# QuentinFuxa/WhisperLiveKit

Hardware: AMD Instinct MI355X
Metric: audio seconds transcribed per second (1/RTF), Whisper-base EN simul_whisper AlignAtt, 0.5 s chunks (higher is better)
Workload: dtype f32; 1 GPU; base.en simul_whisper, 1 stream(s) over 1 GPU(s) (1 per GPU), 30 s 16 kHz speech-like stream, 0.5 s chunks, beam 1, frame_threshold 25, seeded random weights, synthetic vocabulary; model=base.en, streams_total=1

## Files before the change

whisperlivekit_amd/csrc/api.hip:

```cpp
#include <cmath>
#include <cstdio>
#include <cstdlib>
#include <atomic>
#include <chrono>
#include <cstring>
#include <map>
#include <memory>
#include <mutex>
#include <string>
#include <vector>

#include "../../include/wlk_hip.h"
#include "common.h"
#include "internal.h"

namespace wlk {

namespace {
struct UtilStream {
    std::mutex mu;
    hipStream_t stream = nullptr;
};
UtilStream g_util[64];
UtilStream& util_of_current_device() {
// ... 249 lines not shown
        for (int l = 0; l < L; ++l) {
            int n = 0;
            for (int h = 0; h < H; ++h)
                if (rank[(size_t)l * H + h] >= 0) heads[(size_t)l * H + n++] = h;
        }
        copy_sync(m->layer_heads, heads.data(), heads.size() * sizeof(int), hipMemcpyHostToDevice);
        m->align_pairs.assign(pairs, pairs + 2 * n_pairs);
        m->n_align = n_pairs;
        return WLK_OK;
    });
}

int wlk_model_finalize(wlk_model* m) {
    if (!m) return fail(WLK_ERR_ARG, "model is NULL");
    return guarded([&]() {
        WLK_HIP(hipSetDevice(m->device));
        const int nm = m->D.n_mels;
        std::vector<float> f((size_t)nm * kNFreq);
        copy_sync(f.data(), m->w("mel.filters"), f.size() * sizeof(float), hipMemcpyDeviceToHost);
        std::vector<int> lo(nm), hi(nm);
        for (int i = 0; i < nm; ++i) {
            int a = kNFreq, b = 0;
            for (int k = 0; k < kNFreq; ++k)
                if (f[(size_t)i * kNFreq + k] != 0.f) {
                    a = std::min(a, k);
                    b = k + 1;
                }
            if (b == 0) a = 0;
            lo[i] = a;
            hi[i] = b;
        }
        copy_sync(m->filt_lo, lo.data(), nm * sizeof(int), hipMemcpyHostToDevice);
        copy_sync(m->filt_hi, hi.data(), nm * sizeof(int), hipMemcpyHostToDevice);
        m->enc_layers.clear();
        m->dec_layers.clear();
        for (int i = 0; i < m->D.n_audio_layer; ++i) m->enc_layers.push_back(layer_weights(m, "enc", i, false));
        for (int i = 0; i < m->D.n_text_layer; ++i) m->dec_layers.push_back(layer_weights(m, "dec", i, true));
        {
            const size_t d = m->D.n_text_state, da = m->D.n_audio_state, Ld = m->D.n_text_layer;
            if (!m->xkv_all_w) m->xkv_all_w = dev_alloc<float>(Ld * 2 * d * da);
            if (!m->xkv_all_b) m->xkv_all_b = dev_alloc<float>(Ld * 2 * d);
            for (size_t i = 0; i < Ld; ++i) {
                copy_sync(m->xkv_all_w + i * 2 * d * da, m->dec_layers[i].xkvw, 2 * d * da * sizeof(float),
                                  hipMemcpyDeviceToDevice);
                copy_sync(m->xkv_all_b + i * 2 * d, m->dec_layers[i].xkvb, 2 * d * sizeof(float),
                                  hipMemcpyDeviceToDevice);
            }
        }
        {
            for (unsigned short* p : m->x3_owned) (void)hipFree(p);
            m->x3_owned.clear();
            m->xkv_all_w3 = nullptr;
            const int da = m->D.n_audio_state, T = m->D.n_audio_ctx;
            LaunchCtx c;
            c.stream = nullptr;
            hipStream_t st;
            WLK_HIP(hipStreamCreateWithFlags(&st, hipStreamNonBlocking));
            struct StreamGuard {
                hipStream_t s;
                ~StreamGuard() { (void)hipStreamDestroy(s); }
            } st_guard{st};
            c.stream = st;
            auto pack = [&](const float* w, int n_rows, int k = 0) -> unsigned short* {
                if (k == 0) k = da;
                unsigned short* p3 = dev_alloc<unsigned short>(x3_w_elems(n_rows, k));
                m->x3_owned.push_back(p3);
                launch_x3_pack_w(c, w, k, p3, n_rows, k);
                return p3;
            };
            static const bool narrow = [] { const char* e = getenv("WLK_X3_NARROW"); return !(e && e[0] == '0'); }();
            for (auto& L : m->enc_layers) {
                L.qkvw3 = gemm_x3_wide_applicable(T, 3 * da, da, da) ? pack(L.qkvw, 3 * da) : nullptr;
                L.fc1w3 = gemm_x3_wide_applicable(T, 4 * da, da, da) ? pack(L.fc1w, 4 * da) : nullptr;
                L.outw3 = narrow && gemm_x3_wide_applicable(T, da, da, da) ? pack(L.outw, da) : nullptr;
                L.fc2w3 = narrow && gemm_x3_wide_applicable(T, da, 4 * da, 4 * da) ? pack(L.fc2w, da, 4 * da) : nullptr;
            }
            const int n_xkv = m->D.n_text_layer * 2 * m->D.n_text_state;
            if (gemm_x3_wide_applicable(T, n_xkv, da, da)) m->xkv_all_w3 = pack(m->xkv_all_w, n_xkv);
            WLK_HIP(hipStreamSynchronize(st));
        }
        m->w_tok_emb = m->w("dec.tok_emb");
        m->w_dec_pos = m->w("dec.pos");
        m->w_ln_w = m->w("dec.ln.w");
        m->w_ln_b = m->w("dec.ln.b");
        m->finalized = true;
        return WLK_OK;
    });
}

int wlk_model_destroy(wlk_model* m) {
    if (!m) return WLK_OK;
    wlk_engine_destroy_for_model(m);
    (void)hipSetDevice(m->device);
    if (m->owns_arena) (void)hipFree(m->arena);
    if (m->xkv_all_w) (void)hipFree(m->xkv_all_w);
    if (m->xkv_all_b) (void)hipFree(m->xkv_all_b);
    for (unsigned short* p : m->x3_owned) (void)hipFree(p);
    (void)hipFree(m->twiddle);
    (void)hipFree(m->filt_lo);
    (void)hipFree(m->filt_hi);
    (void)hipFree(m->head_rank);
    (void)hipFree(m->layer_heads);
    (void)hipFree(m->layer_ranks);
    (void)hipFree(m->all_ranks);
    if (m->cif_w) (void)hipFree(m->cif_w);
    delete m;
    return WLK_OK;
}

int wlk_session_create(wlk_model* m, int beam, int max_audio_samples, wlk_session** out) {
    if (!m || !out) return fail(WLK_ERR_ARG, "NULL argument");
    if (!m->finalized) return fail(WLK_ERR_STATE, "model not finalized");
    if (beam < 1 || beam > 7) return fail(WLK_ERR_ARG, "beam must be in [1, 7]");
    if (max_audio_samples < kHop) return fail(WLK_ERR_ARG, "max_audio_samples too small");
    return guarded([&]() {
        WLK_HIP(hipSetDevice(m->device));
        auto s = std::make_unique<wlk_session>();
        s->m = m;
        s->beam = beam;
        s->audio_cap = max_audio_samples;
        WLK_HIP(hipStreamCreateWithFlags(&s->stream, hipStreamNonBlocking));
        if (const char* e = std::getenv("WLK_NO_GRAPH")) s->use_graph = !(e[0] == '1');
        hipStream_t st = s->stream;
        const wlk_dims& D = m->D;
        const size_t d = D.n_audio_state, T = D.n_audio_ctx, ctx = D.n_text_ctx, V = D.n_vocab;
        s->audio[0] = dev_alloc_zero<float>(s->audio_cap, st);
        s->audio[1] = dev_alloc_zero<float>(s->audio_cap, st);
        s->frame_cap = s->audio_cap / kHop + 4;
        s->logmel = dev_alloc<float>((size_t)s->frame_cap * D.n_mels);
        s->frame_max = dev_alloc<float>(s->frame_cap);
        s->logmel_alt = dev_alloc<float>((size_t)s->frame_cap * D.n_mels);
        s->frame_max_alt = dev_alloc<float>(s->frame_cap);
        if (const char* e = std::getenv("WLK_MEL_INCREMENTAL")) s->mel_incremental = !(e[0] == '0');
        s->mel_t = dev_alloc_zero<float>((size_t)(kMelFrames + 2) * D.n_mels, st);
        s->x1p = dev_alloc_zero<float>((size_t)(kMelFrames + 1) * d, st);
        s->ex = dev_alloc<float>(T * d);
        s->eh = dev_alloc<float>(T * d);
        s->eqkv = dev_alloc<float>(T * 3 * d);
        s->eatt = dev_alloc<float>(T * d);
        s->emlp = dev_alloc<float>(T * 4 * d);
        s->enc_out = dev_alloc<float>(T * d);
        {
            bool any_x3 = m->xkv_all_w3 != nullptr, qkv_x3 = false;
            bool fc2_x3 = false;
            for (const auto& L : m->enc_layers) {
                any_x3 |= L.qkvw3 || L.fc1w3 || L.outw3;
                qkv_x3 |= L.qkvw3 != nullptr;
                fc2_x3 |= L.fc2w3 != nullptr;
            }
            if (fc2_x3) s->emlp3 = dev_alloc<unsigned short>(T * 3 * 4 * d);
            const bool attn_x3 = qkv_x3 && enc_attention_x3_enabled() && d == (size_t)D.n_audio_head * 64 && T >= 64 && (2 * d) % 128 == 0;
            if (any_x3) s->eh3 = dev_alloc<unsigned short>(T * 3 * d);
            if (attn_x3) s->eqkv3 = dev_alloc_zero<unsigned short>(x3_attn_image_elems((int)T, (int)d), st);
            if (m->xkv_all_w3) s->enc_out3 = dev_alloc<unsigned short>(T * 3 * d);
        }
        s->cross_kv = dev_alloc<float>((size_t)D.n_text_layer * T * 2 * d);

        s->max_rows = beam * (int)ctx;
        const size_t R = s->max_rows;
        s->step_in = dev_alloc<int>(3 * R + 4);
        s->tokens_dev = s->step_in;
        s->dx = dev_alloc<float>(R * d);
        s->dh = dev_alloc<float>(R * d);
        s->dqkv = dev_alloc<float>(R * 3 * d);
        s->datt = dev_alloc<float>(R * d);
        s->dq = dev_alloc<float>(R * d);
        s->dmlp = dev_alloc<float>(R * 4 * d);
        const size_t cache = (size_t)D.n_text_layer * beam * ctx * d;
        s->kcache[0] = dev_alloc<float>(cache);
        s->vcache[0] = dev_alloc<float>(cache);
        s->hsel = dev_alloc<float>((size_t)2 * beam * d);
        s->logits_last = dev_alloc<float>((size_t)2 * beam * V);
        s->logits_sot = s->logits_last + (size_t)beam * V;
        s->ring_row = s->step_in + R;
        s->beam_of_row = s->step_in + 2 * R;
        s->d_offset = s->step_in + 3 * R;
        s->ring_rows = (int)ctx + kAlignWindow;
        if (m->n_align > 0) s->ring = dev_alloc<float>((size_t)m->n_align * beam * s->ring_rows * T);
        s->xsplit = dev_alloc<float>(cross_split_scratch_floats(8, D.n_text_head, (int)T));
        s->fsplit = dev_alloc<float>(flash_split_scratch_floats(s->max_rows, D.n_text_head, wlk_session::kFlashSplitsMax));
        s->z = dev_alloc<float>((size_t)beam * std::max(m->n_align, 1) * T + (size_t)beam * 128);
        s->attn_last = dev_alloc_zero<float>((size_t)beam * T, st);
        s->adj_row = dev_alloc<int>(3 * wlk_session::kAdjCap);
        s->src_rows = dev_alloc<int>(8);
        if (beam >= 2 && beam <= 7) s->anc = dev_alloc_zero<unsigned char>((size_t)beam * ctx, st);
        s->top_vals = dev_alloc<float>((size_t)beam * 18);
        s->top_ids = reinterpret_cast<int*>(s->top_vals) + (size_t)beam * 8;
        s->frames = s->top_ids + (size_t)beam * 8;
        WLK_HIP(hipMalloc(&s->topk_scratch, topk_scratch_bytes(beam)));
        s->probs = dev_alloc<float>(beam);
        WLK_HIP(hipHostMalloc(&s->pinned, wlk_session::kPinnedBytes, hipHostMallocDefault));
        WLK_HIP(hipHostMalloc(&s->dec_stage, 65536, hipHostMallocDefault));
        WLK_HIP(hipHostMalloc(&s->audio_stage, wlk_session::kPinnedBytes, hipHostMallocDefault));
        WLK_HIP(hipEventCreateWithFlags(&s->audio_stage_ev, hipEventDisableTiming));
        WLK_HIP(hipEventCreateWithFlags(&s->dec_stage_ev, hipEventDisableTiming));
        if (beam == 1) {
            void* hp = nullptr;
            WLK_HIP(hipHostMalloc(&hp, 4096, hipHostMallocMapped | hipHostMallocCoherent));
            std::memset(hp, 0, 4096);
            s->step_host = static_cast<StepBlock*>(hp);
            s->result_host = reinterpret_cast<StepResult*>(static_cast<char*>(hp) + 2048);
            void* dp = nullptr;
            WLK_HIP(hipHostGetDevicePointer(&dp, hp, 0));
            s->step_host_dev = static_cast<StepBlock*>(dp);
            s->result_host_dev = reinterpret_cast<StepResult*>(static_cast<char*>(dp) + 2048);
            s->step_dev = reinterpret_cast<StepBlock*>(dev_alloc<int>(sizeof(StepBlock) / 4));
        }
        if (m->cif_w) wlk_cif_session_prepare(s.get());
        WLK_HIP(hipStreamSynchronize(st));
        *out = s.release();
        return WLK_OK;
    });
}

int wlk_session_destroy(wlk_session* s) {
    if (!s) return WLK_OK;
    if (s->step_count && getenv("WLK_STEP_TIMING"))
        fprintf(stderr, "[wlk] one-replay steps: %llu, mean %.1f us per step (graph launch call %.1f us)\n",
                (unsigned long long)s->step_count, s->step_ns / 1e3 / s->step_count, s->step_launch_ns / 1e3 / s->step_count);
    (void)wlk_engine_detach(s);
    (void)hipSetDevice(s->m->device);
    (void)hipStreamSynchronize(s->stream);
    float* fl[] = {s->audio[0], s->audio[1], s->logmel, s->frame_max, s->logmel_alt, s->frame_max_alt, s->mel_t, s->x1p, s->ex, s->eh, s->eqkv,
                   s->eatt, s->emlp, s->enc_out, s->cross_kv, s->dx, s->dh, s->dqkv, s->datt, s->dq, s->dmlp,
                   s->kcache[0], s->kcache[1], s->vcache[0], s->vcache[1], s->hsel, s->logits_last,
                   s->ring, s->z, s->attn_last, s->qk_debug, s->xsplit, s->fsplit, s->top_vals, s->probs};
    for (float* p : fl)
        if (p) (void)hipFree(p);
    int* il[] = {s->step_in, s->adj_row, s->src_rows};
    for (int* p : il)
        if (p) (void)hipFree(p);
    for (auto& e : s->step_exec)
        if (e) (void)hipGraphExecDestroy(e);
    for (auto& e : s->bstep_exec)
        if (e) (void)hipGraphExecDestroy(e);
    if (s->anc) (void)hipFree(s->anc);
    if (s->topk_scratch) (void)hipFree(s->topk_scratch);
    if (s->pcm16_dev) (void)hipFree(s->pcm16_dev);
    if (s->eh3) (void)hipFree(s->eh3);
    if (s->eqkv3) (void)hipFree(s->eqkv3);
    if (s->enc_out3) (void)hipFree(s->enc_out3);
    if (s->emlp3) (void)hipFree(s->emlp3);
    if (s->wa_buf) (void)hipFree(s->wa_buf);
    if (s->pinned) (void)hipHostFree(s->pinned);
    if (s->dec_stage) (void)hipHostFree(s->dec_stage);
    if (s->audio_stage) (void)hipHostFree(s->audio_stage);
    if (s->rules_mask) (void)hipFree(s->rules_mask);
    if (s->pick_out) (void)hipFree(s->pick_out);
    if (s->audio_stage_ev) (void)hipEventDestroy(s->audio_stage_ev);
    if (s->dec_stage_ev) (void)hipEventDestroy(s->dec_stage_ev);
    if (s->step_host) (void)hipHostFree(s->step_host);
    if (s->step_dev) (void)hipFree(s->step_dev);
    if (s->step_align_dev) (void)hipFree(s->step_align_dev);
    wlk_cif_session_free(s);
    for (auto& e : s->fstep_exec)
        if (e) (void)hipGraphExecDestroy(e);
    for (auto& r : s->prof.recs) {
        (void)hipEventDestroy(r.a);
        (void)hipEventDestroy(r.b);
    }
    for (auto e : s->prof.pool) (void)hipEventDestroy(e);
    (void)hipStreamDestroy(s->stream);
    delete s;
    return WLK_OK;
}

int wlk_session_set_debug(wlk_session* s, int on) {
    if (!s) return fail(WLK_ERR_ARG, "session is NULL");
    return guarded([&]() {
        WLK_HIP(hipSetDevice(s->m->device));
        s->debug = on != 0;
        if (s->debug && !s->qk_debug) {
            const wlk_dims& D = s->m->D;
            s->qk_debug = dev_alloc<float>((size_t)D.n_text_layer * s->max_rows * D.n_text_head * D.n_audio_ctx);
        }
        return WLK_OK;
    });
}

static bool drain_staging() {
    static const bool on = [] {
        const char* e = getenv("WLK_DRAIN_STAGING");
        return e && e[0] == '1';
    }();
    return on;
}

int wlk_audio_append(wlk_session* s, const float* pcm_host, int n) {
    if (!s || (n > 0 && !pcm_host) || n < 0) return fail(WLK_ERR_ARG, "bad audio chunk");
    if (s->audio_len + n > s->audio_cap)
        return fail(WLK_ERR_CAPACITY, "audio buffer capacity exceeded (" + std::to_string(s->audio_len + n) + " > " +
                                          std::to_string(s->audio_cap) + " samples)");
    if (n == 0) return WLK_OK;
    return guarded([&]() {
        WLK_HIP(hipSetDevice(s->m->device));
        float* dst = s->audio[s->audio_cur] + s->audio_len;
        size_t done = 0;
        while (done < (size_t)n) {
            const size_t chunk = std::min((size_t)n - done, wlk_session::kPinnedBytes / sizeof(float));
            if (s->audio_stage_used) WLK_HIP(hipEventSynchronize(s->audio_stage_ev));
            std::memcpy(s->audio_stage, pcm_host + done, chunk * sizeof(float));
            WLK_HIP(hipMemcpyAsync(dst + done, s->audio_stage, chunk * sizeof(float), hipMemcpyHostToDevice, s->stream));
            WLK_HIP(hipEventRecord(s->audio_stage_ev, s->stream));
            s->audio_stage_used = true;
            done += chunk;
        }
        if (drain_staging()) WLK_HIP(hipStreamSynchronize(s->stream));
        s->audio_len += n;
        s->encoded = false;
        return WLK_OK;
    });
}

int wlk_audio_append_pcm16(wlk_session* s, const int16_t* pcm_host, int n) {
    if (!s || (n > 0 && !pcm_host) || n < 0) return fail(WLK_ERR_ARG, "bad audio chunk");
    if (s->audio_len + n > s->audio_cap)
        return fail(WLK_ERR_CAPACITY, "audio buffer capacity exceeded (" + std::to_string(s->audio_len + n) + " > " +
                                          std::to_string(s->audio_cap) + " samples)");
    if (n == 0) return WLK_OK;
    return guarded([&]() {
        WLK_HIP(hipSetDevice(s->m->device));
        constexpr size_t kMax = wlk_session::kPinnedBytes / sizeof(int16_t);
        if (!s->pcm16_dev) WLK_HIP(hipMalloc(reinterpret_cast<void**>(&s->pcm16_dev), kMax * sizeof(int16_t)));
        float* dst = s->audio[s->audio_cur] + s->audio_len;
        const LaunchCtx c = s->ctx();
        size_t done = 0;
        while (done < (size_t)n) {
            const size_t chunk = std::min((size_t)n - done, kMax);
            if (s->audio_stage_used) WLK_HIP(hipEventSynchronize(s->audio_stage_ev));
            std::memcpy(s->audio_stage, pcm_host + done, chunk * sizeof(int16_t));
            WLK_HIP(hipMemcpyAsync(s->pcm16_dev, s->audio_stage, chunk * sizeof(int16_t), hipMemcpyHostToDevice, s->stream));
            launch_pcm16_to_float(c, s->pcm16_dev, dst + done, (int)chunk);
            WLK_HIP(hipEventRecord(s->audio_stage_ev, s->stream));
            s->audio_stage_used = true;
            done += chunk;
        }
        if (drain_staging()) WLK_HIP(hipStreamSynchronize(s->stream));
        s->audio_len += n;
        s->encoded = false;
        return WLK_OK;
    });
}

int wlk_audio_append_zeros(wlk_session* s, int n) {
    if (!s || n < 0) return fail(WLK_ERR_ARG, "bad zero run");
    if (s->audio_len + n > s->audio_cap) return fail(WLK_ERR_CAPACITY, "audio buffer capacity exceeded");
    if (n == 0) return WLK_OK;
    return guarded([&]() {
        WLK_HIP(hipSetDevice(s->m->device));
        WLK_HIP(hipMemsetAsync(s->audio[s->audio_cur] + s->audio_len, 0, (size_t)n * sizeof(float), s->stream));
        s->audio_len += n;
        s->encoded = false;
        return WLK_OK;
    });
}

int wlk_audio_drop_front(wlk_session* s, int n) {
    if (!s || n < 0 || n > s->audio_len) return fail(WLK_ERR_ARG, "bad eviction length");
    if (n == 0) return WLK_OK;
    return guarded([&]() {
        WLK_HIP(hipSetDevice(s->m->device));
        const int keep = s->audio_len - n;
        if (keep > 0)
            WLK_HIP(hipMemcpyAsync(s->audio[s->audio_cur ^ 1], s->audio[s->audio_cur] + n, (size_t)keep * sizeof(float),
                                   hipMemcpyDeviceToDevice, s->stream));
        s->audio_cur ^= 1;
        s->audio_len = keep;
        s->encoded = false;
        const int shift = n / kHop;
        if (s->mel_incremental && n % kHop == 0 && s->mel_cached_samples > n && shift < s->mel_cached_frames) {
            const int rows = s->mel_cached_frames - shift;
            const int nm = s->m->D.n_mels;
            WLK_HIP(hipMemcpyAsync(s->logmel_alt, s->logmel + (size_t)shift * nm, (size_t)rows * nm * sizeof(float),
                                   hipMemcpyDeviceToDevice, s->stream));
            WLK_HIP(hipMemcpyAsync(s->frame_max_alt, s->frame_max + shift, (size_t)rows * sizeof(float),
                                   hipMemcpyDeviceToDevice, s->stream));
            std::swap(s->logmel, s->logmel_alt);
            std::swap(s->frame_max, s->frame_max_alt);
            s->mel_cached_samples -= n;
            s->mel_cached_frames = rows;
            s->mel_dirty_head = 2;
        } else {
            s->mel_cached_samples = 0;
        }
        return WLK_OK;
    });
}

int wlk_audio_clear(wlk_session* s) {
    if (!s) return fail(WLK_ERR_ARG, "session is NULL");
    s->audio_len = 0;
    s->encoded = false;
    s->mel_cached_samples = 0;
    return WLK_OK;
}

int wlk_audio_len(wlk_session* s, int* n) {
    if (!s || !n) return fail(WLK_ERR_ARG, "NULL argument");
    *n = s->audio_len;
    return WLK_OK;
}

static void transformer_mlp(const LaunchCtx& c, const LayerW& L, float* x, float* h, float* mlp, int rows, int d,
                            const char* t_ln, const char* t_fc1, const char* t_fc2) {
    GemmArgs g;
    g.lda = d; g.W = L.fc1w; g.bias = L.fc1b; g.C = mlp; g.ldc = 4 * d; g.M = rows; g.N = 4 * d; g.K = d;
    g.flags = kGemmGelu;
    if (gemv_applicable(rows, d)) {
        g.A = x; g.ln_gamma = L.ln2w; g.ln_beta = L.ln2b;
        launch_gemv(c, g, "dec_ln2_fc1");
    } else {
        launch_layernorm(c, x, d, L.ln2w, L.ln2b, h, d, rows, d, t_ln);
        g.A = h;
        launch_gemm(c, g, t_fc1);
    }
    GemmArgs g2;
    g2.A = mlp; g2.lda = 4 * d; g2.W = L.fc2w; g2.bias = L.fc2b; g2.C = x; g2.ldc = d; g2.M = rows; g2.N = d;
    g2.K = 4 * d; g2.flags = kGemmResidual; g2.R = x; g2.ldr = d;
    launch_linear(c, g2, t_fc2);
}

extern "C++" std::string wlk_encode_precheck(const wlk_session* s, const wlk_model* m) {
    if (!s) return "encode: session is NULL";
    if (s->m != m) return "encode: the session belongs to another model";
    const int N = s->audio_len;
    const int n_total = (N + kPadSamples) / kHop;
    int n_active = N > 0 ? (N + kNFft / 2 + kHop - 1) / kHop : 0;
    if (n_active > n_total) n_active = n_total;
    if (n_active > s->frame_cap) return "audio longer than the session's frame capacity";
    return std::string();
}

extern "C++" void wlk_encode_group(const std::vector<wlk_session*>& group, const LaunchCtx& c,
                                   std::vector<int>& content_out, bool mel_given) {
    const int B = (int)group.size();
    if (B < 1 || B > kMaxBatch) throw std::invalid_argument("encode: bad group size");
    wlk_model* m = group[0]->m;
    const wlk_dims& D = m->D;
    const int d = D.n_audio_state, T = D.n_audio_ctx;
    content_out.assign(B, 0);
    for (int i = 0; i < B; ++i) {
        wlk_session* s = group[i];
        if (s->m != m) throw std::invalid_argument("encode: sessions of different models in one group");
        if (mel_given) {
            content_out[i] = D.n_audio_ctx;
            continue;
        }
        const int N = s->audio_len;
        const int n_total = (N + kPadSamples) / kHop;
        int n_active = N > 0 ? (N + kNFft / 2 + kHop - 1) / kHop : 0;
        if (n_active > n_total) n_active = n_total;
        if (n_active > s->frame_cap) throw std::length_error("audio longer than the session's frame capacity");
        content_out[i] = (n_total - kMelFrames) / 2;
        MelArgs ma;
        ma.audio = s->audio[s->audio_cur]; ma.n_samples = N;
        ma.window = m->w("mel.window"); ma.twiddle = m->twiddle; ma.filters = m->w("mel.filters");
        ma.filt_lo = m->filt_lo; ma.filt_hi = m->filt_hi; ma.n_mels = D.n_mels;
        ma.logmel = s->logmel; ma.frame_max = s->frame_max; ma.mel_t = s->mel_t;
        ma.n_active = n_active; ma.n_total = n_total;
        if (s->mel_incremental && s->mel_cached_samples > 0 && s->mel_cached_samples <= N && s->mel_cached_frames <= n_active) {
            int first = s->mel_cached_samples >= kNFft / 2 ? (s->mel_cached_samples - kNFft / 2) / kHop + 1 : 0;
            first = std::min(first, s->mel_cached_frames);
            ma.first = first;
            ma.head = std::min(s->mel_dirty_head, first);
        }
        launch_mel(c, ma);
        s->mel_cached_samples = N;
        s->mel_cached_frames = n_active;
        s->mel_dirty_head = 0;
    }
    auto table = [&](auto in, auto out, auto res) {
        PtrTable z{};
        for (int i = 0; i < B; ++i) {
            z.in[i] = in(group[i]);
            z.out[i] = out(group[i]);
            z.res[i] = res(group[i]);
        }
        return z;
    };
    auto none = [](wlk_session*) -> const float* { return nullptr; };
    auto gemm = [&](GemmArgs g, const PtrTable& z, const char* tag) {
        const bool stackable = !gemm_takes_kwave(g.M, g.N, g.K) && (long)((g.N + 63) / 64) * ((g.M + 63) / 64) >= 64;
        if (stackable) {
            g.batch = B;
            g.z = z;
            launch_gemm(c, g, tag);
        } else {
            for (int i = 0; i < B; ++i) {
                g.A = z.in[i]; g.C = z.out[i]; g.R = z.res[i];
                launch_gemm(c, g, tag);
            }
        }
    };
    {
        GemmArgs g;
        g.lda = D.n_mels; g.W = m->w("enc.conv1.w"); g.bias = m->w("enc.conv1.b");
        g.ldc = d; g.M = kMelFrames; g.N = d; g.K = 3 * D.n_mels; g.flags = kGemmGelu;
        gemm(g, table([](wlk_session* s) { return (const float*)s->mel_t; }, [&](wlk_session* s) { return s->x1p + d; }, none),
             "enc_conv1");
    }
    {
        const float* pos = m->w("enc.pos");
        GemmArgs g;
        g.lda = 2 * d; g.W = m->w("enc.conv2.w"); g.bias = m->w("enc.conv2.b");
        g.ldc = d; g.M = T; g.N = d; g.K = 3 * d; g.flags = kGemmGelu | kGemmResidual; g.ldr = d;
        gemm(g, table([](wlk_session* s) { return (const float*)s->x1p; }, [](wlk_session* s) { return s->ex; },
                      [&](wlk_session*) { return pos; }), "enc_conv2");
    }
    const float scale = std::pow((float)kHeadDim, -0.25f);
    const PtrTable z_ex_eh = table([](wlk_session* s) { return (const float*)s->ex; }, [](wlk_session* s) { return s->eh; }, none);
    const PtrTable z_eh_qkv = table([](wlk_session* s) { return (const float*)s->eh; }, [](wlk_session* s) { return s->eqkv; }, none);
    const PtrTable z_qkv_att = table([](wlk_session* s) { return (const float*)s->eqkv; }, [](wlk_session* s) { return s->eatt; }, none);
    const PtrTable z_att_ex = table([](wlk_session* s) { return (const float*)s->eatt; }, [](wlk_session* s) { return s->ex; },
                                    [](wlk_session* s) { return (const float*)s->ex; });
    const PtrTable z_eh_mlp = table([](wlk_session* s) { return (const float*)s->eh; }, [](wlk_session* s) { return s->emlp; }, none);
    const PtrTable z_mlp_ex = table([](wlk_session* s) { return (const float*)s->emlp; }, [](wlk_session* s) { return s->ex; },
                                    [](wlk_session* s) { return (const float*)s->ex; });
    const PtrTable z_ex_eh3 = table([](wlk_session* s) { return (const float*)s->ex; },
                                    [](wlk_session* s) { return reinterpret_cast<float*>(s->eh3); }, none);
    const PtrTable z_eh3_qkv = table([](wlk_session* s) { return reinterpret_cast<const float*>(s->eh3); },
                                     [](wlk_session* s) { return s->eqkv; }, none);
    const PtrTable z_eh3_mlp = table([](wlk_session* s) { return reinterpret_cast<const float*>(s->eh3); },
                                     [](wlk_session* s) { return s->emlp; }, none);
    const PtrTable z_eh3_qkv3 = table([](wlk_session* s) { return reinterpret_cast<const float*>(s->eh3); },
                                      [](wlk_session* s) { return reinterpret_cast<float*>(s->eqkv3); }, none);
    const PtrTable z_qkv3_att = table([](wlk_session* s) { return reinterpret_cast<const float*>(s->eqkv3); },
                                      [](wlk_session* s) { return s->eatt; }, none);
    const PtrTable z_qkv3_eh3 = table([](wlk_session* s) { return reinterpret_cast<const float*>(s->eqkv3); },
                                      [](wlk_session* s) { return reinterpret_cast<float*>(s->eh3); }, none);
    const PtrTable z_eh3_ex_res = table([](wlk_session* s) { return reinterpret_cast<const float*>(s->eh3); }, [](wlk_session* s) { return s->ex; },
                                        [](wlk_session* s) { return (const float*)s->ex; });
    const PtrTable z_eh3_mlp3 = table([](wlk_session* s) { return reinterpret_cast<const float*>(s->eh3); },
                                      [](wlk_session* s) { return reinterpret_cast<float*>(s->emlp3); }, none);
    const PtrTable z_mlp3_ex_res = table([](wlk_session* s) { return reinterpret_cast<const float*>(s->emlp3); }, [](wlk_session* s) { return s->ex; },
                                         [](wlk_session* s) { return (const float*)s->ex; });
    const bool attn_x3 = enc_attention_x3_enabled() && d == D.n_audio_head * 64 && T >= 64 && (2 * d) % 128 == 0;
    auto gemm_x3 = [&](const GemmArgs& g, const unsigned short* w3, const PtrTable& z, const char* tag) {
        X3GemmArgs x;
        x.lda = g.lda; x.W3 = w3; x.bias = g.bias; x.ldc = g.ldc; x.ldr = g.ldr; x.M = g.M; x.N = g.N; x.K = g.K;
        x.flags = g.flags; x.scale = g.scale; x.scale_cols = g.scale_cols; x.scale_period = g.scale_period;
        x.batch = B;
        x.z = z;
        launch_gemm_x3(c, x, tag);
    };
    for (int i = 0; i < D.n_audio_layer; ++i) {
        const LayerW& L = m->enc_layers[i];
        GemmArgs g;
        g.lda = d; g.W = L.qkvw; g.bias = L.qkvb; g.ldc = 3 * d; g.M = T; g.N = 3 * d;
        g.K = d; g.flags = kGemmScaleCols; g.scale = scale; g.scale_cols = 2 * d;
        bool att_is_x3 = false;
        if (L.qkvw3 && attn_x3) {
            launch_layernorm_x3_batched(c, z_ex_eh3, B, d, L.ln1w, L.ln1b, d, T, d, "enc_ln1");
            X3GemmArgs x;
            x.lda = d; x.W3 = L.qkvw3; x.bias = g.bias; x.M = T; x.N = 3 * d; x.K = d; x.flags = g.flags; x.scale = g.scale;
            x.scale_cols = g.scale_cols; x.batch = B; x.z = z_eh3_qkv3;
            x.x3_out = true; x.ldc3 = 2 * d; x.vt_col0 = 2 * d; x.vt_off = x3_attn_vt_off(T, d); x.vt_ld = x3_attn_vt_ld(T);
            launch_gemm_x3(c, x, "enc_qkv_x3");
            att_is_x3 = L.outw3 != nullptr;
            launch_encoder_attention_x3(c, nullptr, 2L * d, x3_attn_vt_off(T, d), x3_attn_vt_ld(T), nullptr, d, T, d, D.n_audio_head,
                                        att_is_x3 ? &z_qkv3_eh3 : &z_qkv3_att, B, att_is_x3);
        } else {
            if (L.qkvw3) {
                launch_layernorm_x3_batched(c, z_ex_eh3, B, d, L.ln1w, L.ln1b, d, T, d, "enc_ln1");
                gemm_x3(g, L.qkvw3, z_eh3_qkv, "enc_qkv_x3");
            } else {
                launch_layernorm_batched(c, z_ex_eh, B, d, L.ln1w, L.ln1b, d, T, d, "enc_ln1");
                gemm(g, z_eh_qkv, "enc_qkv");
            }
            launch_encoder_attention_batched(c, z_qkv_att, B, T, d, D.n_audio_head);
        }
        GemmArgs o;
        o.lda = d; o.W = L.outw; o.bias = L.outb; o.ldc = d; o.M = T; o.N = d; o.K = d;
        o.flags = kGemmResidual; o.ldr = d;
        if (L.outw3) {
            if (!att_is_x3)
                for (int i = 0; i < B; ++i) launch_x3_pack(c, group[i]->eatt, d, group[i]->eh3, d, T, d);
            gemm_x3(o, L.outw3, z_eh3_ex_res, "enc_out_x3");
        } else {
            gemm(o, z_att_ex, "enc_out");
        }
        GemmArgs f1;
        f1.lda = d; f1.W = L.fc1w; f1.bias = L.fc1b; f1.ldc = 4 * d; f1.M = T; f1.N = 4 * d; f1.K = d; f1.flags = kGemmGelu;
        const bool mlp_x3 = L.fc1w3 && L.fc2w3 && (4 * d) % 128 == 0;
        if (mlp_x3) {
            launch_layernorm_x3_batched(c, z_ex_eh3, B, d, L.ln2w, L.ln2b, d, T, d, "enc_ln2");
            X3GemmArgs x;
            x.lda = d; x.W3 = L.fc1w3; x.bias = f1.bias; x.M = T; x.N = 4 * d; x.K = d; x.flags = kGemmGelu; x.batch = B; x.z = z_eh3_mlp3;
            x.x3_out = true; x.ldc3 = 4 * d; x.vt_col0 = 4 * d; x.vt_off = 0; x.vt_ld = (T + 31) / 32 * 32;
            launch_gemm_x3(c, x, "enc_fc1_x3");
        } else if (L.fc1w3) {
            launch_layernorm_x3_batched(c, z_ex_eh3, B, d, L.ln2w, L.ln2b, d, T, d, "enc_ln2");
            gemm_x3(f1, L.fc1w3, z_eh3_mlp, "enc_fc1_x3");
        } else {
            launch_layernorm_batched(c, z_ex_eh, B, d, L.ln2w, L.ln2b, d, T, d, "enc_ln2");
            gemm(f1, z_eh_mlp, "enc_fc1");
        }
        GemmArgs f2;
        f2.lda = 4 * d; f2.W = L.fc2w; f2.bias = L.fc2b; f2.ldc = d; f2.M = T; f2.N = d; f2.K = 4 * d;
        f2.flags = kGemmResidual; f2.ldr = d;
        if (L.fc2w3) {
            if (!mlp_x3)
                for (int i = 0; i < B; ++i) launch_x3_pack(c, group[i]->emlp, 4 * d, group[i]->emlp3, 4 * d, T, 4 * d);
            gemm_x3(f2, L.fc2w3, z_mlp3_ex_res, "enc_fc2_x3");
        } else {
            gemm(f2, z_mlp_ex, "enc_fc2");
        }
    }
    {
        GemmArgs g;
        g.lda = d; g.W = m->xkv_all_w; g.bias = m->xkv_all_b;
        g.ldc = (long)D.n_text_layer * 2 * d; g.M = T; g.N = D.n_text_layer * 2 * d; g.K = d;
        g.flags = kGemmScaleCols; g.scale = scale; g.scale_cols = d; g.scale_period = 2 * d;
        if (m->xkv_all_w3) {
            launch_layernorm_x3_batched(c, table([](wlk_session* s) { return (const float*)s->ex; },
                                                 [](wlk_session* s) { return reinterpret_cast<float*>(s->enc_out3); }, none),
                                        B, d, m->w("enc.ln_post.w"), m->w("enc.ln_post.b"), d, T, d, "enc_ln_post");
            gemm_x3(g, m->xkv_all_w3,
                    table([](wlk_session* s) { return reinterpret_cast<const float*>(s->enc_out3); }, [](wlk_session* s) { return s->cross_kv; }, none),
                    "dec_cross_kv_x3");
        } else {
            launch_layernorm_batched(c, table([](wlk_session* s) { return (const float*)s->ex; }, [](wlk_session* s) { return s->enc_out; }, none),
                                     B, d, m->w("enc.ln_post.w"), m->w("enc.ln_post.b"), d, T, d, "enc_ln_post");
            gemm(g, table([](wlk_session* s) { return (const float*)s->enc_out; }, [](wlk_session* s) { return s->cross_kv; }, none),
                 "dec_cross_kv");
        }
        for (int i = 0; i < B; ++i) group[i]->enc_out_is_x3 = m->xkv_all_w3 != nullptr;
    }
    if (m->cif_w) wlk_cif_enqueue(group, c, content_out);
    else
        for (int i = 0; i < B; ++i) group[i]->cif_T = -1;
    for (int i = 0; i < B; ++i) {
        wlk_session* s = group[i];
        s->encoded = true;
        s->content_len = content_out[i];
        s->self_len = 0;
        s->n_steps = 0;
    }
}

int wlk_encode(wlk_session* s, int32_t* content_mel_len) {
    if (!s) return fail(WLK_ERR_ARG, "session is NULL");
    return guarded([&]() {
        WLK_HIP(hipSetDevice(s->m->device));
        int content = 0;
        struct Busy {
            wlk_session* s;
            explicit Busy(wlk_session* ss) : s(ss) { wlk_engine_loop_enter(s); }
            ~Busy() { wlk_engine_loop_exit(s); }
        } busy(s);
        if (wlk_engine_batches_encodes(s)) {
            if (int rc = wlk_engine_encode(s, &content)) return rc;
        } else {
            std::vector<int> out;
            wlk_encode_group({s}, s->ctx(), out);
            content = out[0];
        }
        if (content_mel_len) *content_mel_len = content;
        return WLK_OK;
    });
}

int wlk_session::flash_splits() {
    static const int n = [] {
        const char* e = getenv("WLK_FLASH_SPLITS");
        const int v = e ? atoi(e) : 6;
        return v < 1 ? 1 : (v > kFlashSplitsMax ? kFlashSplitsMax : v);
    }();
    return n;
}

constexpr size_t kAncStageOffset = 65536 - 64;

static void enqueue_decode(wlk_session* s, const LaunchCtx& c, int n_rows, int n_tok, bool first, int sot_index,
                           bool step_block = false, const AlignArgs* side_align = nullptr, int side_blocks = 0, int side_zf = 0,
                           bool ancestry = false) {
    wlk_model* m = s->m;
    const wlk_dims& D = m->D;
    const int ctx_len = D.n_text_ctx;
    const int R = n_rows * n_tok;
    const int d = D.n_text_state, T = D.n_audio_ctx, H = D.n_text_head, V = D.n_vocab;
    if (!step_block)
        WLK_HIP(hipMemcpyAsync(s->step_in, s->dec_stage, (size_t)(3 * s->max_rows + 1) * sizeof(int), hipMemcpyHostToDevice,
                               s->stream));
    const bool fused = gemv_applicable(R, d) && n_tok == 1;
    if (ancestry) {
        if (!fused || step_block || !s->anc) throw std::logic_error("decode: the ancestry step needs the fused beam step");
        WLK_HIP(hipMemcpyAsync(s->src_rows, static_cast<char*>(s->dec_stage) + kAncStageOffset, 8 * sizeof(int),
                               hipMemcpyHostToDevice, s->stream));
        launch_anc_update(c, s->anc, s->src_rows, s->d_offset, n_rows, ctx_len);
    }

    if (step_block)
        launch_embed_step(c, s->step_host_dev, s->step_dev, s->tokens_dev, s->ring_row, s->beam_of_row, s->d_offset,
                          m->w_tok_emb, m->w_dec_pos, s->dx, d);
    else
        launch_embed(c, s->tokens_dev, m->w_tok_emb, m->w_dec_pos, s->dx, n_rows, n_tok, s->d_offset, d);
    const float scale = std::pow((float)kHeadDim, -0.25f);
    const size_t cache_layer = (size_t)s->beam * ctx_len * d;
    bool scores_dumped = false;
    for (int i = 0; i < D.n_text_layer; ++i) {
        const LayerW& L = m->dec_layers[i];
        float* kc = s->kcache[s->kv_cur] + i * cache_layer;
        float* vc = s->vcache[s->kv_cur] + i * cache_layer;
        GemmArgs g;
        g.W = L.qkvw; g.bias = L.qkvb; g.C = s->dqkv; g.ldc = 3 * d; g.M = R; g.N = 3 * d;
        g.K = d; g.flags = kGemmScaleCols; g.scale = scale; g.scale_cols = 2 * d; g.lda = d;
        if (fused) {
            g.A = s->dx; g.ln_gamma = L.ln1w; g.ln_beta = L.ln1b;
            g.kcache = kc; g.vcache = vc; g.kv_pos = s->d_offset; g.kv_d = d; g.kv_ctx = ctx_len;
            launch_gemv(c, g, "dec_ln1_qkv_kv");
        } else {
            launch_layernorm(c, s->dx, d, L.ln1w, L.ln1b, s->dh, d, R, d, "dec_ln1");
            g.A = s->dh;
            if (!gemv_applicable(R, d) && gemm_takes_kwave(R, 3 * d, d)) {
                g.kcache = kc; g.vcache = vc; g.kv_pos = s->d_offset; g.kv_d = d; g.kv_ctx = ctx_len; g.kv_ntok = n_tok;
                launch_gemm(c, g, "dec_qkv");
            } else {
                launch_linear(c, g, "dec_qkv");
                launch_kv_append(c, s->dqkv, kc, vc, n_rows, n_tok, s->d_offset, d, ctx_len);
            }
        }
        if (ancestry)
            launch_decoder_self_attention_anc(c, s->dqkv, kc, vc, s->anc, s->datt, n_rows, s->d_offset, d, H, ctx_len);
        else
            launch_decoder_self_attention(c, s->dqkv, kc, vc, s->datt, n_rows, n_tok, s->d_offset, d, H, ctx_len);
        GemmArgs o;
        o.A = s->datt; o.lda = d; o.W = L.outw; o.bias = L.outb; o.C = s->dx; o.ldc = d; o.M = R; o.N = d; o.K = d;
        o.flags = kGemmResidual; o.R = s->dx; o.ldr = d;
        launch_linear(c, o, "dec_out");

        GemmArgs q;
        q.lda = d; q.W = L.xqw; q.bias = L.xqb; q.C = s->dq; q.ldc = d; q.M = R; q.N = d; q.K = d;
// ... 576 lines not shown
        s->step_ns += (uint64_t)std::chrono::duration_cast<std::chrono::nanoseconds>(std::chrono::steady_clock::now() - t_enter).count();
        s->step_count += 1;
        top_logprobs2[0] = r->top_vals[0]; top_logprobs2[1] = r->top_vals[1];
        top_ids2[0] = r->top_ids[0]; top_ids2[1] = r->top_ids[1];
        *frame = r->frame;
        return WLK_OK;
    });
}

int wlk_kv_reorder(wlk_session* s, const int32_t* source_rows, int n_rows) {
    if (!s || !source_rows || n_rows != s->beam) return fail(WLK_ERR_ARG, "bad reorder request");
    if (s->anc_live)
        return fail(WLK_ERR_STATE, "wlk_kv_reorder after an ancestry beam step: the cache rows are not the hypotheses");
    bool identity = true;
    for (int i = 0; i < n_rows; ++i) {
        if (source_rows[i] < 0 || source_rows[i] >= n_rows) return fail(WLK_ERR_ARG, "source row out of range");
        identity &= source_rows[i] == i;
    }
    if (identity || s->self_len == 0) return WLK_OK;
    return guarded([&]() {
        const wlk_dims& D = s->m->D;
        WLK_HIP(hipSetDevice(s->m->device));
        const LaunchCtx c = s->ctx();
        const size_t cache = (size_t)D.n_text_layer * s->beam * D.n_text_ctx * D.n_text_state;
        if (!s->kcache[1]) {
            s->kcache[1] = dev_alloc<float>(cache);
            s->vcache[1] = dev_alloc<float>(cache);
        }
        WLK_HIP(hipStreamSynchronize(s->stream));
        std::memcpy(s->pinned, source_rows, n_rows * sizeof(int));
        WLK_HIP(hipMemcpyAsync(s->src_rows, s->pinned, n_rows * sizeof(int), hipMemcpyHostToDevice, s->stream));
        const int cur = s->kv_cur;
        launch_kv_gather(c, s->kcache[cur], s->kcache[cur ^ 1], s->src_rows, n_rows, s->self_len, D.n_text_state,
                         D.n_text_ctx, D.n_text_layer);
        launch_kv_gather(c, s->vcache[cur], s->vcache[cur ^ 1], s->src_rows, n_rows, s->self_len, D.n_text_state,
                         D.n_text_ctx, D.n_text_layer);
        s->kv_cur ^= 1;
        return WLK_OK;
    });
}

extern "C++" int wlk_beam_step(wlk_session* s, const int64_t* tokens, const int32_t* source_rows) {
    if (!s || !tokens || !source_rows) return fail(WLK_ERR_ARG, "NULL argument");
    wlk_model* m = s->m;
    const wlk_dims& D = m->D;
    const int B = s->beam;
    if (!s->anc || B < 2 || B > 7 || s->debug || s->prof_on || !s->use_graph || s->n_steps < 1 || !s->encoded ||
        !gemv_applicable(B, D.n_text_state) || D.n_text_ctx > 512 || D.n_text_state != D.n_text_head * kHeadDim ||
        (size_t)(s->max_rows * 3 + 4) * sizeof(int) > kAncStageOffset)
        return 1;
    if (s->self_len + 1 > D.n_text_ctx) return fail(WLK_ERR_CAPACITY, "text context exceeded");
    for (int b = 0; b < B; ++b) {
        if (tokens[b] < 0 || tokens[b] >= D.n_vocab) return fail(WLK_ERR_ARG, "token id out of range");
        if (source_rows[b] < 0 || source_rows[b] >= B) return fail(WLK_ERR_ARG, "source row out of range");
    }
    return guarded([&]() {
        WLK_HIP(hipSetDevice(m->device));
        const LaunchCtx c = s->ctx();
        if (s->dec_stage_used) WLK_HIP(hipEventSynchronize(s->dec_stage_ev));
        if (drain_staging()) WLK_HIP(hipStreamSynchronize(s->stream));
        int* stage = static_cast<int*>(s->dec_stage);
        const int MR = s->max_rows;
        const int slot_row = D.n_text_ctx + ((s->n_steps - 1) % kAlignWindow);
        for (int b = 0; b < B; ++b) {
            stage[b] = (int)tokens[b];
            stage[MR + b] = slot_row;
            stage[2 * MR + b] = b;
        }
        stage[3 * MR] = s->self_len;
        int* ctl = reinterpret_cast<int*>(static_cast<char*>(s->dec_stage) + kAncStageOffset);
        for (int b = 0; b < 7; ++b) ctl[b] = b < B ? source_rows[b] : 0;
        ctl[7] = s->anc_live ? 0 : 1;
        hipGraphExec_t& exec = s->bstep_exec[s->kv_cur];
        if (!exec) capture_step_graph(s->stream, exec, [&] { enqueue_decode(s, c, B, 1, false, 0, false, nullptr, 0, 0, true); });
        WLK_HIP(hipGraphLaunch(exec, s->stream));
        WLK_HIP(hipEventRecord(s->dec_stage_ev, s->stream));
        s->dec_stage_used = true;
        s->have_sot = false;
        s->anc_live = true;
        s->anc_steps += 1;
        s->self_len += 1;
        s->n_steps += 1;
        s->last_rows = B;
        s->last_ntok = 1;
        return WLK_OK;
    });
}

int wlk_diag_beam_step(wlk_session* s, const int64_t* tokens, const int32_t* source_rows, int n_rows) {
    if (!s || n_rows != s->beam) return fail(WLK_ERR_ARG, "n_rows must equal the session's beam size");
    const int rc = wlk_beam_step(s, tokens, source_rows);
    return rc == 1 ? fail(WLK_ERR_STATE, "the session does not qualify for the ancestry step") : rc;
}

int wlk_decode_ancestry(wlk_session* s, const int64_t* tokens, const int32_t* source_rows, int n_rows) {
    if (!s || !tokens || !source_rows) return fail(WLK_ERR_ARG, "NULL argument");
    if (n_rows != s->beam) return fail(WLK_ERR_ARG, "n_rows must equal the session's beam size");
    if (!s->encoded) return fail(WLK_ERR_STATE, "wlk_decode_ancestry before wlk_encode");
    if (s->n_steps == 0) return fail(WLK_ERR_STATE, "wlk_decode_ancestry before the prefill (wlk_decode with first=1)");
    const int rc = wlk_beam_step(s, tokens, source_rows);
    if (rc != 1) return rc;
    if (s->anc_live) return fail(WLK_ERR_STATE, "wlk_decode_ancestry: the session stopped qualifying for the ancestry step inside an infer");
    if (int rc2 = wlk_kv_reorder(s, source_rows, n_rows)) return rc2;
    return wlk_decode(s, tokens, n_rows, 1, 0, 0);
}

int wlk_session_beam_stats(wlk_session* s, uint64_t* ancestry_steps) {
    if (!s || !ancestry_steps) return fail(WLK_ERR_ARG, "NULL argument");
    *ancestry_steps = s->anc_steps;
    return WLK_OK;
}

int wlk_sync(wlk_session* s) {
    if (!s) return fail(WLK_ERR_ARG, "session is NULL");
    return guarded([&]() {
        WLK_HIP(hipSetDevice(s->m->device));
        WLK_HIP(hipStreamSynchronize(s->stream));
        return WLK_OK;
    });
}

static int copy_out(wlk_session* s, const float* dev, uint64_t n, float* host, uint64_t cap, uint64_t* n_written) {
    if (n_written) *n_written = n;
    if (n > cap) return fail(WLK_ERR_CAPACITY, "export buffer too small: need " + std::to_string(n) + " floats");
    WLK_HIP(hipStreamSynchronize(s->stream));
    copy_sync(host, dev, n * sizeof(float), hipMemcpyDeviceToHost);
    return WLK_OK;
}

int wlk_export(wlk_session* s, const char* what, float* host, uint64_t capacity, uint64_t* n_written) {
    if (!s || !what || !host) return fail(WLK_ERR_ARG, "NULL argument");
    return guarded([&]() {
        const wlk_dims& D = s->m->D;
        WLK_HIP(hipSetDevice(s->m->device));
        const std::string w(what);
        const uint64_t T = D.n_audio_ctx, d = D.n_text_state;
        if (w == "mel") {
            const uint64_t n = (uint64_t)D.n_mels * kMelFrames;
            if (n_written) *n_written = n;
            if (n > capacity) return fail(WLK_ERR_CAPACITY, "export buffer too small");
            std::vector<float> tm(n);
            WLK_HIP(hipStreamSynchronize(s->stream));
            copy_sync(tm.data(), s->mel_t + D.n_mels, n * sizeof(float), hipMemcpyDeviceToHost);
            for (int t = 0; t < kMelFrames; ++t)
                for (int mm = 0; mm < D.n_mels; ++mm) host[(size_t)mm * kMelFrames + t] = tm[(size_t)t * D.n_mels + mm];
            return WLK_OK;
        }
        if (w == "enc") {
            if (s->enc_out_is_x3) {
                launch_x3_unpack(s->ctx(), s->enc_out3, d, s->enc_out, d, (int)T, (int)d);
            }
            return copy_out(s, s->enc_out, T * d, host, capacity, n_written);
        }
        if (w == "logits_last") return copy_out(s, s->logits_last, (uint64_t)s->beam * D.n_vocab, host, capacity, n_written);
        if (w == "logits_sot") return copy_out(s, s->logits_sot, (uint64_t)s->beam * D.n_vocab, host, capacity, n_written);
        if (w == "attn_last") return copy_out(s, s->attn_last, (uint64_t)s->beam * T, host, capacity, n_written);
        if (w == "dec_x") return copy_out(s, s->dx, (uint64_t)s->last_rows * s->last_ntok * d, host, capacity, n_written);
        const auto colon = w.find(':');
        if (colon != std::string::npos) {
            const std::string kind = w.substr(0, colon);
            const int idx = std::atoi(w.c_str() + colon + 1);
            if (kind == "cross_qk") {
                if (!s->qk_debug) return fail(WLK_ERR_STATE, "cross_qk export needs a debug session");
                if (idx < 0 || idx >= D.n_text_layer) return fail(WLK_ERR_ARG, "layer out of range");
                const uint64_t rows = (uint64_t)s->last_rows * s->last_ntok;
                return copy_out(s, s->qk_debug + (size_t)idx * s->max_rows * D.n_text_head * T,
                                rows * D.n_text_head * T, host, capacity, n_written);
            }
            if (kind == "self_k" || kind == "self_v") {
                if (idx < 0 || idx >= D.n_text_layer) return fail(WLK_ERR_ARG, "layer out of range");
                const float* base = (kind == "self_k" ? s->kcache : s->vcache)[s->kv_cur] +
                                    (size_t)idx * s->beam * D.n_text_ctx * d;
                const uint64_t n = (uint64_t)s->beam * s->self_len * d;
                if (n_written) *n_written = n;
                if (n > capacity) return fail(WLK_ERR_CAPACITY, "export buffer too small");
                WLK_HIP(hipStreamSynchronize(s->stream));
                for (int b = 0; b < s->beam; ++b)
                    copy_sync(host + (size_t)b * s->self_len * d, base + (size_t)b * D.n_text_ctx * d,
                                      (size_t)s->self_len * d * sizeof(float), hipMemcpyDeviceToHost);
                return WLK_OK;
            }
            if (kind == "xattn_w") {
                if (idx < 0 || idx >= s->m->n_align) return fail(WLK_ERR_ARG, "alignment rank out of range");
                const int pre = s->n_steps <= kAlignWindow ? s->prefill_rows : 0;
                const int ns = std::min(s->n_steps - 1, kAlignWindow);
                const uint64_t n = (uint64_t)(pre + ns) * T;
                if (n_written) *n_written = n;
                if (n > capacity) return fail(WLK_ERR_CAPACITY, "export buffer too small");
                const float* base = s->ring + (size_t)idx * s->beam * s->ring_rows * T;
                WLK_HIP(hipStreamSynchronize(s->stream));
                if (pre) copy_sync(host, base, (size_t)pre * T * sizeof(float), hipMemcpyDeviceToHost);
                if (ns)
                    copy_sync(host + (size_t)pre * T, base + (size_t)D.n_text_ctx * T, (size_t)ns * T * sizeof(float),
                                      hipMemcpyDeviceToHost);
                return WLK_OK;
            }
        }
        return fail(WLK_ERR_ARG, "unknown export '" + w + "'");
    });
}


int wlk_melspec_create(int device, int n_fft, int win_length, int hop, int n_mels, const float* filters,
                       const float* window, float preemph, float log_guard, int max_samples, wlk_melspec** out) {
    if (!filters || !window || !out) return fail(WLK_ERR_ARG, "NULL argument");
    if (n_fft < 16 || n_fft > 512 || win_length < 1 || win_length > n_fft || hop < 1 || n_mels < 1 || n_mels > 256 ||
        max_samples < n_fft)
        return fail(WLK_ERR_ARG, "unsupported mel-spectrogram configuration");
    return guarded([&]() {
        WLK_HIP(hipSetDevice(device));
        auto m = std::make_unique<wlk_melspec>();
        m->device = device; m->n_fft = n_fft; m->win_length = win_length; m->hop = hop; m->n_mels = n_mels;
        m->preemph = preemph; m->log_guard = log_guard; m->cap = max_samples;
        const int nf = n_fft / 2 + 1;
        WLK_HIP(hipStreamCreateWithFlags(&m->stream, hipStreamNonBlocking));
        m->window = dev_alloc<float>(win_length);
        m->filters = dev_alloc<float>((size_t)n_mels * nf);
        m->twiddle = dev_alloc<double>(n_fft);
        m->lo = dev_alloc<int>(n_mels);
        m->hi = dev_alloc<int>(n_mels);
        m->audio = dev_alloc<float>(max_samples);
        m->out = dev_alloc<float>((size_t)(max_samples / hop + 2) * n_mels);
        std::vector<double> tw(n_fft);
        for (int i = 0; i < n_fft; ++i) tw[i] = std::cos(2.0 * M_PI * (double)i / (double)n_fft);
        std::vector<int> lo(n_mels), hi(n_mels);
        for (int i = 0; i < n_mels; ++i) {
            int a = nf, b = 0;
            for (int k = 0; k < nf; ++k)
                if (filters[(size_t)i * nf + k] != 0.f) { a = std::min(a, k); b = k + 1; }
            if (b == 0) a = 0;
            lo[i] = a; hi[i] = b;
        }
        copy_sync(m->window, window, win_length * sizeof(float), hipMemcpyHostToDevice);
        copy_sync(m->filters, filters, (size_t)n_mels * nf * sizeof(float), hipMemcpyHostToDevice);
        copy_sync(m->twiddle, tw.data(), n_fft * sizeof(double), hipMemcpyHostToDevice);
        copy_sync(m->lo, lo.data(), n_mels * sizeof(int), hipMemcpyHostToDevice);
        copy_sync(m->hi, hi.data(), n_mels * sizeof(int), hipMemcpyHostToDevice);
        *out = m.release();
        return WLK_OK;
    });
}

int wlk_melspec_run(wlk_melspec* m, const float* pcm_host, int n, float* out_host, int capacity_frames, int* n_frames) {
    if (!m || !pcm_host || !out_host || !n_frames) return fail(WLK_ERR_ARG, "NULL argument");
    if (n < 1 || n > m->cap) return fail(WLK_ERR_CAPACITY, "chunk does not fit the extractor's buffer");
    return guarded([&]() {
        std::lock_guard<std::mutex> lock(m->mu);
        WLK_HIP(hipSetDevice(m->device));
        const int frames = n / m->hop + 1;
        *n_frames = frames;
        if (frames > capacity_frames) return fail(WLK_ERR_CAPACITY, "output buffer too small");
        WLK_HIP(hipMemcpyAsync(m->audio, pcm_host, (size_t)n * sizeof(float), hipMemcpyHostToDevice, m->stream));
        MelSpecArgs a;
        a.audio = m->audio; a.n_samples = n; a.window = m->window; a.twiddle = m->twiddle; a.filters = m->filters;
        a.filt_lo = m->lo; a.filt_hi = m->hi; a.out = m->out; a.n_fft = m->n_fft; a.win_length = m->win_length;
        a.hop = m->hop; a.n_mels = m->n_mels; a.preemph = m->preemph; a.log_guard = m->log_guard;
        LaunchCtx c{m->stream, nullptr};
        launch_melspec(c, a, frames);
        WLK_HIP(hipMemcpyAsync(out_host, m->out, (size_t)frames * m->n_mels * sizeof(float), hipMemcpyDeviceToHost, m->stream));
        WLK_HIP(hipStreamSynchronize(m->stream));
        return WLK_OK;
    });
}

int wlk_melspec_destroy(wlk_melspec* m) {
    if (!m) return WLK_OK;
    (void)hipSetDevice(m->device);
    float* fl[] = {m->window, m->filters, m->audio, m->out};
    for (float* p : fl)
        if (p) (void)hipFree(p);
    if (m->twiddle) (void)hipFree(m->twiddle);
    if (m->lo) (void)hipFree(m->lo);
    if (m->hi) (void)hipFree(m->hi);
    if (m->stream) (void)hipStreamDestroy(m->stream);
    delete m;
    return WLK_OK;
}

int wlk_prof_begin(wlk_session* s) {
    if (!s) return fail(WLK_ERR_ARG, "session is NULL");
    for (auto& r : s->prof.recs) {
        s->prof.pool.push_back(r.a);
        s->prof.pool.push_back(r.b);
    }
    s->prof.recs.clear();
    s->prof_on = true;
    return WLK_OK;
}

int wlk_session_step_stats(wlk_session* s, uint64_t* steps, uint64_t* wall_ns, uint64_t* launch_ns) {
    if (!s || !steps || !wall_ns || !launch_ns) return fail(WLK_ERR_ARG, "NULL argument");
    *steps = s->step_count;
    *wall_ns = s->step_ns;
    *launch_ns = s->step_launch_ns;
    return WLK_OK;
}

int wlk_prof_end(wlk_session* s, int cap, const char** names, float* total_ms, int32_t* launches, double* flops,
                 double* bytes, int32_t* n_out) {
    if (!s || !n_out) return fail(WLK_ERR_ARG, "NULL argument");
    return guarded([&]() {
        WLK_HIP(hipSetDevice(s->m->device));
        WLK_HIP(hipStreamSynchronize(s->stream));
        s->prof_on = false;
        std::vector<const char*> order;
        std::map<std::string, std::pair<double, int>> acc;
// ... 34 lines not shown
```

whisperlivekit_amd/csrc/common.h:

```cpp
#pragma once
#include <hip/hip_runtime.h>

#include <cstdint>
#include <stdexcept>
#include <mutex>
#include <string>

namespace wlk {

constexpr int kNFft = 400;
constexpr int kHop = 160;
constexpr int kNFreq = 201;
constexpr int kMelFrames = 3000;
constexpr int kPadSamples = 480000;
constexpr int kHeadDim = 64;
constexpr int kAlignWindow = 16;

struct HipError : std::runtime_error {
    using std::runtime_error::runtime_error;
};

inline void hip_check(hipError_t e, const char* what, const char* file, int line) {
    if (e != hipSuccess) {
        throw HipError(std::string(what) + " failed: " + hipGetErrorString(e) + " (" + file + ":" +
                       std::to_string(line) + ")");
    }
}
#define WLK_HIP(expr) ::wlk::hip_check((expr), #expr, __FILE__, __LINE__)

void set_last_error(const std::string& msg);

struct Profiler;
void copy_sync(void* dst, const void* src, size_t bytes, hipMemcpyKind kind);
void memset_sync(void* dst, int value, size_t bytes);

struct LaunchCtx {
    hipStream_t stream = nullptr;
    Profiler* prof = nullptr;
};
void prof_before(const LaunchCtx& ctx, const char* name, double flops, double bytes);
void prof_after(const LaunchCtx& ctx);

struct KernelScope {
    const LaunchCtx& ctx;
    KernelScope(const LaunchCtx& c, const char* name, double flops = 0.0, double bytes = 0.0) : ctx(c) {
        if (ctx.prof) prof_before(ctx, name, flops, bytes);
    }
    ~KernelScope() {
        if (ctx.prof) prof_after(ctx);
    }
};

template <typename F>
void capture_step_graph(hipStream_t stream, hipGraphExec_t& exec, F&& enqueue) {
    if (exec) throw std::logic_error("capture_step_graph: the executable graph is already recorded");
    hipGraph_t graph = nullptr;
    WLK_HIP(hipStreamBeginCapture(stream, hipStreamCaptureModeThreadLocal));
    try {
        enqueue();
    } catch (...) {
        (void)hipStreamEndCapture(stream, &graph);
        if (graph) (void)hipGraphDestroy(graph);
        throw;
    }
    hipError_t e = hipStreamEndCapture(stream, &graph);
    if (e == hipSuccess) e = hipGraphInstantiate(&exec, graph, nullptr, nullptr, 0);
    if (graph) (void)hipGraphDestroy(graph);
    if (e != hipSuccess) exec = nullptr;
    hip_check(e, "recording a step graph", __FILE__, __LINE__);
}

struct StepRow {
    float* kcache;
    float* vcache;
    const float* cross_kv;
    float* ring;
    int token;
    int offset;
    int ring_row;
    int prefill_rows, n_single, newest_row, content_len;
    int pad;
};

constexpr int kStepMaxAdj = 160;
struct StepBlock {
    StepRow row;
    int n_adj;
    unsigned seq;
    int pad[2];
    int adj_row[kStepMaxAdj];
    int adj_ids[kStepMaxAdj];
    float adj_deltas[kStepMaxAdj];
};
struct StepResult {
    float top_vals[2];
    int top_ids[2];
    int frame;
    unsigned flag_topk, flag_align;
    int pad;
};
struct StepHostOut {
    StepResult* result = nullptr;
    const int* n_adj = nullptr;
    const unsigned* seq = nullptr;
};
constexpr int kEngineFusedAdj = 1024;
struct EngineBlock {
    int n_adj;
    unsigned seq;
    int pad[2];
    StepRow rows[8];
    int adj_row[kEngineFusedAdj];
    int adj_ids[kEngineFusedAdj];
    float adj_deltas[kEngineFusedAdj];
};
void launch_embed_rows_step(const LaunchCtx& ctx, const EngineBlock* host_block, EngineBlock* dev_block, const float* tok_emb,
                            const float* pos_emb, float* x, int n_rows, int d);
void launch_embed_step(const LaunchCtx& ctx, const StepBlock* host_block, StepBlock* dev_block, int* tokens_dev,
                       int* ring_row, int* beam_of_row, int* d_offset, const float* tok_emb, const float* pos_emb, float* x,
                       int d);

constexpr int kMaxBatch = 8;
struct PtrTable {
    const float* in[kMaxBatch];
    float* out[kMaxBatch];
    const float* res[kMaxBatch];
};
template <typename T>
__device__ __forceinline__ T table_at(T const (&t)[kMaxBatch], unsigned z) {
    T v = t[0];
#pragma unroll
    for (int i = 1; i < kMaxBatch; ++i) v = (z == (unsigned)i) ? t[i] : v;
    return v;
}

enum GemmFlags : int {
    kGemmGelu = 1,
    kGemmResidual = 2,
    kGemmScaleCols = 4,
    kGemmRelu = 8,
    kGemmSwish = 16,
};
struct AlignArgs;
struct GemmArgs {
    const float* A = nullptr;
    long lda = 0;
    const float* W = nullptr;
    const float* bias = nullptr;
    float* C = nullptr;
    long ldc = 0;
    const float* R = nullptr;
    long ldr = 0;
    int M = 0, N = 0, K = 0;
    int flags = 0;
    float scale = 1.f;
    int scale_cols = 0;
    int scale_period = 0;
    int batch = 0;
    long long* dbg_clock = nullptr;
    const float* ln_gamma = nullptr;
    const float* ln_beta = nullptr;
    float* kcache = nullptr;
    float* vcache = nullptr;
    const int* kv_pos = nullptr;
    int kv_d = 0, kv_ctx = 0;
    int kv_ntok = 1;
    const StepRow* kv_rows = nullptr;
    long kv_layer_off = 0;
    const float* mg_pm = nullptr;
    const float* mg_pl = nullptr;
    const float* mg_po = nullptr;
    const float* mg_scores = nullptr;
    const int* mg_head_rank = nullptr;
    const int* mg_side_heads = nullptr;
    float* mg_ring = nullptr;
    const int* mg_ring_row = nullptr;
    const int* mg_beam_of_row = nullptr;
    int mg_heads = 0, mg_T = 0, mg_ring_rows = 0, mg_n_beam = 1, mg_side_blocks = 0;
    PtrTable z;
    const AlignArgs* side_align = nullptr;
    int side_blocks = 0, side_zf = 0;
    bool force_kwave = false;
    int force_kernel = 0;
    bool gemm_plain_loop = false;
};
#define WLK_PIN_S(x) asm volatile("" ::"s"(x))
#define WLK_PIN_GEMM_ARGS(g)                                                                                                \
    do {                                                                                                                    \
        asm volatile("" ::"s"((g).A), "s"((g).lda), "s"((g).W), "s"((g).bias), "s"((g).C), "s"((g).ldc), "s"((g).R),        \
                     "s"((g).ldr), "s"((g).M), "s"((g).N), "s"((g).K), "s"((g).flags), "s"((g).scale), "s"((g).scale_cols), \
                     "s"((g).scale_period), "s"((g).batch), "s"((g).dbg_clock));                                            \
        __builtin_amdgcn_sched_barrier(0);     \
    } while (0)
void launch_gemm(const LaunchCtx& ctx, const GemmArgs& g, const char* tag);
void launch_gemm_kp(const LaunchCtx& ctx, const GemmArgs& g, const char* tag);
bool gemm_kp_takes_kpipe(int M, int N, int K);
bool gemm_takes_kwave(int M, int N, int K);
bool gemm_takes_ksplit(int M, int N, int K);
void launch_gemv(const LaunchCtx& ctx, const GemmArgs& g, const char* tag);
inline int gemv_row_bucket(int M) { return M <= 1 ? 1 : M <= 2 ? 2 : M <= 4 ? 4 : 8; }
inline bool gemv_applicable(int M, int K) {
    return M <= 8 && (long)gemv_row_bucket(M) * K * 4 <= 64 * 1024 && K % 4 == 0;
}
struct GemvPlan {
    enum Kernel { kRefused, kStaged, kSingleRow, kSingleRowMergeLds };
    Kernel kernel = kRefused;
    int width = 0;
    int rpw = 0;
    bool ln = false, mg = false, full = false;
    const char* refusal = nullptr;
};
GemvPlan gemv_plan(const GemmArgs& g);
bool gemv1_folds_merge(int K);
void refresh_env_switches();
inline void launch_linear(const LaunchCtx& ctx, const GemmArgs& g, const char* tag) {
    if (gemv_applicable(g.M, g.K)) launch_gemv(ctx, g, tag);
    else launch_gemm(ctx, g, tag);
}

struct X3GemmArgs {
    const unsigned short* A3 = nullptr;
    long lda = 0;
    const unsigned short* W3 = nullptr;
    const float* bias = nullptr;
    float* C = nullptr;
    long ldc = 0;
    const float* R = nullptr;
    long ldr = 0;
    int M = 0, N = 0, K = 0;
    int flags = 0;
    float scale = 1.f;
    int scale_cols = 0;
    int scale_period = 0;
    int batch = 0;
    int walk_banded = 0;
    int walk_colmajor = 0;
    int walk_slots = 0;
    unsigned short* C3 = nullptr;
    long ldc3 = 0;
    int vt_col0 = 0;
    long vt_off = 0;
    long vt_ld = 0;
    bool x3_out = false;
    PtrTable z;
};
bool gemm_x3_wide_applicable(int M, int N, int K, long lda);
void launch_gemm_x3(const LaunchCtx& ctx, const X3GemmArgs& g, const char* tag);
void x3_gemm_check(const X3GemmArgs& g);
struct X3GemmPlan {
    int bm = 96;
    int tiles_m = 0, tiles_n = 0;
    int banded = 0, colmajor = 0, persist = 1;
    int slots = 0;
    int blocks = 0;
};
X3GemmPlan x3_gemm_plan(int M, int N, int batch, int cus);
size_t x3_w_elems(int n, int k);
void launch_x3_pack_w(const LaunchCtx& ctx, const float* src, long ld_src, unsigned short* dst, int n, int k);
void launch_x3_pack(const LaunchCtx& ctx, const float* src, long ld_src, unsigned short* dst, long ld_dst, int rows, int cols);
void x3_pack_check(long ld_src, long ld_dst, int cols);
void launch_x3_unpack(const LaunchCtx& ctx, const unsigned short* src, long ld_src, float* dst, long ld_dst, int rows, int cols);

inline long x3_attn_vt_ld(int T) { return ((long)T + 31) / 32 * 32; }
inline long x3_attn_vt_off(int T, int d) { return (long)T * 3 * 2 * d; }
inline size_t x3_attn_image_elems(int T, int d) { return (size_t)x3_attn_vt_off(T, d) + (size_t)d * 3 * x3_attn_vt_ld(T); }
bool enc_attention_x3_enabled();
void launch_encoder_attention_x3(const LaunchCtx& ctx, const unsigned short* qk3, long ldqk, long vt_off, long vt_ld, float* out,
                                 long ldo, int T, int d, int n_head, const PtrTable* z, int batch, bool x3_out = false);
void enc_attention_x3_check(long ldqk, long vt_ld, long ldo, int T, int d, int n_head, bool x3_out);
void launch_x3_pack_qkv(const LaunchCtx& ctx, const float* qkv, unsigned short* out, int T, int d, long vt_off, long vt_ld);

void layernorm_check(int d, long ldx, long ldy3, bool x3, int batch);
void launch_layernorm(const LaunchCtx& ctx, const float* x, long ldx, const float* gamma, const float* beta,
                      float* y, long ldy, int rows, int d, const char* tag);
void launch_layernorm_batched(const LaunchCtx& ctx, const PtrTable& z, int batch, long ldx, const float* gamma,
                              const float* beta, long ldy, int rows, int d, const char* tag);
void launch_layernorm_x3(const LaunchCtx& ctx, const float* x, long ldx, const float* gamma, const float* beta,
                         unsigned short* y3, long ldy3, int rows, int d, const char* tag);
void launch_layernorm_x3_batched(const LaunchCtx& ctx, const PtrTable& z, int batch, long ldx, const float* gamma,
                                 const float* beta, long ldy3, int rows, int d, const char* tag);

struct MelArgs {
    const float* audio;
    int n_samples;
    const float* window;
    const double* twiddle;
    const float* filters;
    const int* filt_lo;
    const int* filt_hi;
    int n_mels;
    float* logmel;
    float* frame_max;
    float* mel_t;
    int n_active;
    int n_total;
    int head = 0;
    int first = 0;
    int n_padded = 0x7fffffff;
};
void launch_mel(const LaunchCtx& ctx, const MelArgs& a);
void launch_mel_full(const LaunchCtx& ctx, const MelArgs& a, float* max_scratch, float* out);
void launch_pcm16_to_float(const LaunchCtx& ctx, const short* in, float* out, int n);

struct MelSpecArgs {
    const float* audio;
    int n_samples;
    const float* window;
    const double* twiddle;
    const float* filters;
    const int* filt_lo;
    const int* filt_hi;
    float* out;
    int n_fft, win_length, hop, n_mels;
    float preemph, log_guard;
};
void launch_melspec(const LaunchCtx& ctx, const MelSpecArgs& a, int n_frames);
}
struct wlk_melspec {
    int device = 0, n_fft = 0, win_length = 0, hop = 0, n_mels = 0, cap = 0;
    float preemph = 0.f, log_guard = 0.f;
    float *window = nullptr, *filters = nullptr, *audio = nullptr, *out = nullptr;
    double* twiddle = nullptr;
    int *lo = nullptr, *hi = nullptr;
    hipStream_t stream = nullptr;
    std::mutex mu;
};
namespace wlk {

struct FlashArgs {
    const float* q = nullptr; long ldq = 0;
    const float* k = nullptr; const float* v = nullptr; long ldkv = 0;
    float* out = nullptr; long ldo = 0;
    int Tq = 0, Tk = 0, n_head = 0;
    int batch = 0;
    long z_k_off = 0, z_v_off = 0;
    int k_splits = 1;
    int ring_rows = 0;
    const StepRow* tile_rows = nullptr;
    long tile_kv_off = 0, tile_v_off = 0;
    const int* head_rank = nullptr;
    float* ring = nullptr;
    const int* ring_row = nullptr;
    const int* beam_of_row = nullptr;
    int n_beam = 1;
    float* part_o = nullptr;
    float* part_m = nullptr;
    float* part_l = nullptr;
    PtrTable z;
};
#define WLK_PIN_FLASH_ARGS(a)                                                                                              \
    do {                                                                                                                   \
        asm volatile("" ::"s"((a).q), "s"((a).ldq), "s"((a).k), "s"((a).v), "s"((a).ldkv), "s"((a).out), "s"((a).ldo),      \
                     "s"((a).Tq), "s"((a).Tk), "s"((a).n_head), "s"((a).batch), "s"((a).z_k_off), "s"((a).z_v_off),         \
                     "s"((a).k_splits), "s"((a).ring_rows), "s"((a).tile_rows));                                            \
        __builtin_amdgcn_sched_barrier(0);                                                                                 \
    } while (0)
size_t flash_split_scratch_floats(int rows, int n_head, int k_splits);
void launch_encoder_attention(const LaunchCtx& ctx, const float* qkv, float* out, int T, int d, int n_head);
void launch_encoder_attention_batched(const LaunchCtx& ctx, const PtrTable& z, int batch, int T, int d, int n_head);
void launch_prefill_cross_attention(const LaunchCtx& ctx, const FlashArgs& a);
void launch_ring_softmax(const LaunchCtx& ctx, float* ring, const int* ring_row, const int* beam_of_row,
                         const int* ranks_dev, int n_ranks, int rows, int ring_rows, int n_beam, int T);

void launch_embed(const LaunchCtx& ctx, const int* tokens, const float* tok_emb, const float* pos_emb,
                  float* x, int n_rows, int n_tok, const int* offset_dev, int d);
void launch_embed_rows(const LaunchCtx& ctx, const StepRow* rows, const float* tok_emb, const float* pos_emb, float* x,
                       int n_rows, int d);
void launch_decoder_self_attention_rows(const LaunchCtx& ctx, const float* qkv, const StepRow* rows, long layer_off,
                                        float* out, int n_rows, int d, int n_head, int ctx_len);
void launch_kv_append(const LaunchCtx& ctx, const float* qkv, float* kc, float* vc, int n_rows, int n_tok,
                      const int* offset_dev, int d, int ctx_len);
void launch_kv_append_rows(const LaunchCtx& ctx, const float* qkv, const StepRow* rows, long layer_off, int n_rows, int d);
void launch_decoder_self_attention_anc(const LaunchCtx& ctx, const float* qkv, const float* kc, const float* vc,
                                       const unsigned char* anc, float* out, int n_rows, const int* offset, int d,
                                       int n_head, int ctx_len);
void launch_anc_update(const LaunchCtx& ctx, unsigned char* anc, const int* ctl, const int* offset, int n_rows, int ctx_len);
void launch_anc_update_block(const LaunchCtx& ctx, unsigned char* anc, const int* block, int n_rows, int ctx_len);
void launch_decoder_self_attention(const LaunchCtx& ctx, const float* qkv, const float* kc, const float* vc,
                                   float* out, int n_rows, int n_tok, const int* offset_dev, int d, int n_head,
                                   int ctx_len);
struct CrossAttnArgs {
    const float* q;
    const float* k;
    const float* v;
    long ldkv;
    float* out;
    int rows, d, n_head, T;
    const int* head_rank;
    float* ring;
    const int* ring_row;
    const int* beam_of_row;
    int ring_rows, n_beam;
    float* qk_debug;
    const StepRow* step_rows = nullptr;
    long kv_off = 0;
    const float* xq_x = nullptr;
    const float* xq_w = nullptr;
    const float* xq_b = nullptr;
    const float* xq_gamma = nullptr;
    const float* xq_beta = nullptr;
    float xq_scale = 1.f;
};
void launch_decoder_cross_attention(const LaunchCtx& ctx, const CrossAttnArgs& a);
bool cross_split_folds_query(int d);
void launch_decoder_cross_attention_split(const LaunchCtx& ctx, const CrossAttnArgs& a, float* scores, float* pm,
                                          float* pl, float* po, bool merge = true);
constexpr int kCrossSplitWays = 8;
size_t cross_split_scratch_floats(int rows, int n_head, int T);
void launch_kv_gather(const LaunchCtx& ctx, const float* src, float* dst, const int* source_rows, int n_rows,
                      int len, int d, int ctx_len, int n_layer);

inline int sf_sub_len(int n) { return (n - 1) / 2 + 1; }
void launch_sf_scale_copy(const LaunchCtx& ctx, const float* src, float* dst, long n, float scale);
constexpr int kSfMaxSegments = 8;
struct SfSegments {
    int n = 0;
    int start[kSfMaxSegments] = {0}, len[kSfMaxSegments] = {0};
};
struct SfConvSegs {
    int n = 0, in_total = 0, out_total = 0;
    int in_start[kSfMaxSegments] = {0}, in_len[kSfMaxSegments] = {0}, out_start[kSfMaxSegments] = {0};
};
SfConvSegs sf_conv_segs_next(const SfConvSegs& prev);
void launch_sf_conv0(const LaunchCtx& ctx, const float* in, const float* w, const float* b, float* out, const SfConvSegs& sg, int F,
                     int C);
void launch_sf_dwconv2d(const LaunchCtx& ctx, const float* in, const float* w, const float* b, float* out, const SfConvSegs& sg,
                        int Fi, int C);
void launch_sf_assemble(const LaunchCtx& ctx, const float* ctx_rows, const float* chunk_rows, float* x, const SfSegments& rows,
                        const SfSegments& chunks, int d, float scale);
struct SfAttnArgs {
    const float* q = nullptr; const float* k = nullptr; const float* v = nullptr;
    long ldq = 0, ldk = 0, ldv = 0;
    float* out = nullptr; long ldo = 0;
    int T = 0, n_head = 0, dh = 0;
    float scale = 1.f;
    const float* pos = nullptr; long ldp = 0; int pos_row0 = 0;
    const float* bias_u = nullptr; const float* bias_v = nullptr;
    int n_seg = 0;
    int seg_start[kSfMaxSegments] = {0}, seg_T[kSfMaxSegments] = {0};
};
constexpr int kSfMaxFrames = 512;
void launch_sf_attention(const LaunchCtx& ctx, const SfAttnArgs& a, int form = 0);
void launch_sf_glu_dwconv(const LaunchCtx& ctx, const float* in, const float* w, const float* b, const float* bn_mean,
                          const float* bn_invstd, const float* bn_w, const float* bn_b, float* out, const SfSegments& rows, int d,
                          int taps);
void launch_sf_head(const LaunchCtx& ctx, const float* x, const float* w1t, const float* b1, const float* w2,
                    const float* b2, float* out, int T, int d, int n_spk);
void launch_sf_transpose(const LaunchCtx& ctx, const float* src, float* dst, int rows, int cols);

constexpr int kSfStateMaxKeys = 4096;
constexpr int kSfStateMaxRows = 1024;
struct SfStateParams {
// ... 71 lines not shown
```

whisperlivekit_amd/csrc/gemm_f32.hip:

```cpp
#include <algorithm>
#include <atomic>
#include <cstdlib>
#include <type_traits>

#include "common.h"
#include "wave_ops.h"
#include "align_body.h"

namespace wlk {

typedef float f32x16 __attribute__((ext_vector_type(16)));
typedef float f32x4 __attribute__((ext_vector_type(4)));
typedef unsigned int u32x4 __attribute__((ext_vector_type(4)));

constexpr int BK = 32, LDS_LD = BK + 4;

__device__ __forceinline__ float gelu_erf(float x) {
    return 0.5f * x * (1.0f + erff(x * 0.70710678118654752440f));
}

template <int NA, int NW>
struct Stage {
    float4 a[NA], w[NW];
};

template <int BM, int BN>
__global__ __launch_bounds__(64 * (BM / 32) * (BN / 32)) void gemm_nt_f32_kernel(GemmArgs g) {
    WLK_PIN_GEMM_ARGS(g);
    constexpr int NT = 64 * (BM / 32) * (BN / 32);
    constexpr int NA = BM * 8 / NT, NW = BN * 8 / NT;
    __shared__ __attribute__((aligned(16))) float As[2][BM * LDS_LD];
    __shared__ __attribute__((aligned(16))) float Ws[2][BN * LDS_LD];

    const int tid = threadIdx.x;
    const int lane = tid & 63;
    const int wave = tid >> 6;
    const int wr = wave / (BN / 32), wc = wave % (BN / 32);
    const bool batched = g.batch > 0;
    const float* const gA = batched ? table_at(g.z.in, blockIdx.y) : g.A;
    float* const gC = batched ? table_at(g.z.out, blockIdx.y) : g.C;
    const float* const gR = batched ? table_at(g.z.res, blockIdx.y) : g.R;
    const int tiles_m = (g.M + BM - 1) / BM, tiles_n = (g.N + BN - 1) / BN;
    int tile_m, tile_n;
    if (tiles_m >= 8) {
        const int band_m = (tiles_m + 3) / 4, band_n = (tiles_n + 1) / 2;
        const int xcd = blockIdx.x & 7, slot = blockIdx.x >> 3;
        tile_m = (xcd >> 1) * band_m + slot / band_n;
        tile_n = (xcd & 1) * band_n + slot % band_n;
        if (slot >= band_m * band_n || tile_m >= tiles_m || tile_n >= tiles_n) return;
    } else {
        tile_m = blockIdx.x / tiles_n;
        tile_n = blockIdx.x - tile_m * tiles_n;
        if (tile_m >= tiles_m) return;
    }
    const int m0 = tile_m * BM;
    const int n0 = tile_n * BN;

    constexpr unsigned kOob = 0x80000000u;
    const __amdgpu_buffer_rsrc_t rsrc_a = __builtin_amdgcn_make_buffer_rsrc(
        const_cast<float*>(gA), 0, (int)((((long)g.M - 1) * g.lda + g.K) * 4), 0x00020000);
    const __amdgpu_buffer_rsrc_t rsrc_w = __builtin_amdgcn_make_buffer_rsrc(
        const_cast<float*>(g.W), 0, (int)((long)g.N * g.K * 4), 0x00020000);
    unsigned a_byte[NA], w_byte[NW];
    int a_lds[NA], w_lds[NW], a_c[NA], w_c[NW];
#pragma unroll
    for (int i = 0; i < NA; ++i) {
        const int idx = tid + NT * i, row = idx >> 3, c4 = idx & 7;
        a_byte[i] = (m0 + row) < g.M ? (unsigned)(((long)(m0 + row) * g.lda + c4 * 4) * 4) : kOob;
        a_lds[i] = row * LDS_LD + c4 * 4;
        a_c[i] = c4 * 4;
    }
#pragma unroll
    for (int i = 0; i < NW; ++i) {
        const int idx = tid + NT * i, row = idx >> 3, c4 = idx & 7;
        w_byte[i] = (n0 + row) < g.N ? (unsigned)(((long)(n0 + row) * g.K + c4 * 4) * 4) : kOob;
        w_lds[i] = row * LDS_LD + c4 * 4;
        w_c[i] = c4 * 4;
    }
    const int nk = (g.K + BK - 1) / BK;

    auto fetch = [&](Stage<NA, NW>& st, int kt) {
        const int k0 = kt * BK;
#pragma unroll
        for (int i = 0; i < NA; ++i) {
            const unsigned off = (k0 + a_c[i]) < g.K ? a_byte[i] + (unsigned)k0 * 4u : kOob;
            const u32x4 v = __builtin_amdgcn_raw_buffer_load_b128(rsrc_a, (int)off, 0, 0);
            st.a[i] = make_float4(__uint_as_float(v.x), __uint_as_float(v.y), __uint_as_float(v.z), __uint_as_float(v.w));
        }
#pragma unroll
        for (int i = 0; i < NW; ++i) {
            const unsigned off = (k0 + w_c[i]) < g.K ? w_byte[i] + (unsigned)k0 * 4u : kOob;
            const u32x4 v = __builtin_amdgcn_raw_buffer_load_b128(rsrc_w, (int)off, 0, 0);
            st.w[i] = make_float4(__uint_as_float(v.x), __uint_as_float(v.y), __uint_as_float(v.z), __uint_as_float(v.w));
        }
    };
    auto stash = [&](const Stage<NA, NW>& st, int buf) {
#pragma unroll
        for (int i = 0; i < NA; ++i) *reinterpret_cast<float4*>(&As[buf][a_lds[i]]) = st.a[i];
#pragma unroll
        for (int i = 0; i < NW; ++i) *reinterpret_cast<float4*>(&Ws[buf][w_lds[i]]) = st.w[i];
    };

    f32x16 acc;
#pragma unroll
    for (int i = 0; i < 16; ++i) acc[i] = 0.f;
    const int a_off = (wr * 32 + (lane & 31)) * LDS_LD + (lane >> 5) * 4;
    const int w_off = (wc * 32 + (lane & 31)) * LDS_LD + (lane >> 5) * 4;
    Stage<NA, NW> s0, s1;
    fetch(s0, 0);
    fetch(s1, 1);
    stash(s0, 0);
    __syncthreads();
    const int nk2 = (nk + 1) & ~1;
    {
#define WLK_MFMA(a, b) acc = __builtin_amdgcn_mfma_f32_32x32x2f32(a, b, acc, 0, 0, 0)
#define WLK_SB() __builtin_amdgcn_sched_barrier(0)
        auto rd_a = [&](int buf, int grp) { return *reinterpret_cast<const float4*>(&As[buf][a_off + grp * 8]); };
        auto rd_w = [&](int buf, int grp) { return *reinterpret_cast<const float4*>(&Ws[buf][w_off + grp * 8]); };
        float4 fa0 = rd_a(0, 0), fb0 = rd_w(0, 0), fa1 = rd_a(0, 1), fb1 = rd_w(0, 1), fa2, fb2, fa3, fb3;
        auto tile = [&](int buf, const Stage<NA, NW>& nxt) {
            WLK_MFMA(fa0.x, fb0.x); WLK_SB();
            fa2 = rd_a(buf, 2); fb2 = rd_w(buf, 2); WLK_SB();
            WLK_MFMA(fa0.y, fb0.y); WLK_MFMA(fa0.z, fb0.z); WLK_MFMA(fa0.w, fb0.w);
            WLK_MFMA(fa1.x, fb1.x); WLK_SB();
            fa3 = rd_a(buf, 3); fb3 = rd_w(buf, 3); WLK_SB();
            WLK_MFMA(fa1.y, fb1.y); WLK_MFMA(fa1.z, fb1.z); WLK_MFMA(fa1.w, fb1.w); WLK_SB();
            stash(nxt, buf ^ 1);
            __syncthreads();
            WLK_MFMA(fa2.x, fb2.x); WLK_SB();
            fa0 = rd_a(buf ^ 1, 0); fb0 = rd_w(buf ^ 1, 0); WLK_SB();
            WLK_MFMA(fa2.y, fb2.y); WLK_MFMA(fa2.z, fb2.z); WLK_MFMA(fa2.w, fb2.w);
            WLK_MFMA(fa3.x, fb3.x); WLK_SB();
            fa1 = rd_a(buf ^ 1, 1); fb1 = rd_w(buf ^ 1, 1); WLK_SB();
            WLK_MFMA(fa3.y, fb3.y); WLK_MFMA(fa3.z, fb3.z); WLK_MFMA(fa3.w, fb3.w); WLK_SB();
        };
        for (int kt = 0; kt < nk2; kt += 2) {
            fetch(s0, kt + 2);
            WLK_SB();
            tile(0, s1);
            fetch(s1, kt + 3);
            WLK_SB();
            tile(1, s0);
        }
#undef WLK_MFMA
#undef WLK_SB
    }

    const int col = n0 + wc * 32 + (lane & 31);
    if (col < g.N) {
        const float b = g.bias ? g.bias[col] : 0.f;
        const bool do_scale = (g.flags & kGemmScaleCols) && (g.scale_period ? col % g.scale_period : col) < g.scale_cols;
        const int row_base = m0 + wr * 32 + 4 * (lane >> 5);
        float res[16];
        if (g.flags & kGemmResidual) {
#pragma unroll
            for (int r = 0; r < 16; ++r) {
                const int row = row_base + (r & 3) + 8 * (r >> 2);
                res[r] = gR[(long)min(row, g.M - 1) * g.ldr + col];
            }
        } else {
#pragma unroll
            for (int r = 0; r < 16; ++r) res[r] = 0.f;
        }
        const bool gelu = (g.flags & kGemmGelu) != 0;
        const bool relu = (g.flags & kGemmRelu) != 0, swish = (g.flags & kGemmSwish) != 0;
#pragma unroll
        for (int r = 0; r < 16; ++r) {
            const int row = row_base + (r & 3) + 8 * (r >> 2);
            float v = acc[r] + b;
            if (do_scale) v *= g.scale;
            if (gelu) v = gelu_erf(v);
            if (relu) v = fmaxf(v, 0.f);
            if (swish) v = v / (1.0f + expf(-v));
            v += res[r];
            if (row < g.M) gC[(long)row * g.ldc + col] = v;
        }
    }
}

template <bool KP, int NBUF = 2>
__global__ __launch_bounds__(256) void gemm_nt_f32_kwave_kernel(GemmArgs g) {
    WLK_PIN_GEMM_ARGS(g);
    constexpr int KW = 4, SLAB = BK * KW, SUB = 32 * LDS_LD;
    __shared__ __attribute__((aligned(16))) float As[NBUF][KW * SUB];
    __shared__ __attribute__((aligned(16))) float Ws[NBUF][KW * SUB];
    const int tid = threadIdx.x, lane = tid & 63, wave = tid >> 6;
    const int tiles_n = (g.N + 31) / 32;
    const int tile_m = blockIdx.x / tiles_n, tile_n = blockIdx.x - tile_m * tiles_n;
    const int m0 = tile_m * 32, n0 = tile_n * 32;

    constexpr unsigned kOob = 0x80000000u;
    const __amdgpu_buffer_rsrc_t rsrc_a = __builtin_amdgcn_make_buffer_rsrc(
        const_cast<float*>(g.A), 0, (int)((((long)g.M - 1) * g.lda + g.K) * 4), 0x00020000);
    const __amdgpu_buffer_rsrc_t rsrc_w = __builtin_amdgcn_make_buffer_rsrc(
        const_cast<float*>(g.W), 0, (int)((long)g.N * g.K * 4), 0x00020000);
    unsigned a_byte[4], w_byte[4];
    int lds_at[4];
    const int c4 = tid & 31, kcol = c4 * 4;
#pragma unroll
    for (int i = 0; i < 4; ++i) {
        const int row = (tid >> 5) + 8 * i;
        a_byte[i] = (m0 + row) < g.M ? (unsigned)(((long)(m0 + row) * g.lda + kcol) * 4) : kOob;
        w_byte[i] = (n0 + row) < g.N ? (unsigned)(((long)(n0 + row) * g.K + kcol) * 4) : kOob;
        lds_at[i] = (c4 >> 3) * SUB + row * LDS_LD + (c4 & 7) * 4;
    }
    struct Slab {
        float4 a[4], w[4];
    };
    auto fetch = [&](Slab& st, int ks) {
// ... 267 lines not shown
        const int col = n0 + 32 * j + (lane & 31);
        eo.bias[j] = g.bias && col < g.N ? g.bias[col] : 0.f;
        eo.mul[j] = scaled && (g.scale_period ? col % g.scale_period : col) < g.scale_cols ? g.scale : 1.0f;
    }
#pragma unroll
    for (int q = 0; q < TM * TN; ++q) {
        const int i = q / TN, j = q % TN;
        const int col = min(n0 + 32 * j + (lane & 31), g.N - 1);
        const int row0 = m0 + 32 * i + 8 * wave + 4 * (lane >> 5);
#pragma unroll
        for (int e = 0; e < 4; ++e) eo.res[q][e] = has_res ? gR[(long)min(row0 + e, g.M - 1) * g.ldr + col] : 0.f;
    }
}

template <int TM, int TN, int LDS_FLOATS>
__device__ __forceinline__ void ksplit_fold_store(const GemmArgs& g, f32x16 (&acc)[TM][TN], const EpilogueOperands<TM, TN>& eo,
                                                  float* lds, int wave, int lane, int m0, int n0, float* gC) {
    constexpr int NT = TM * TN;
    constexpr int RES_FLOATS = NT * 1024, COL_FLOATS = 512;
    constexpr int P_FIT = (LDS_FLOATS - RES_FLOATS - COL_FLOATS) / 4096;
    static_assert(P_FIT >= 1, "no room for the fold");
    constexpr int P = P_FIT < NT ? P_FIT : NT;
    constexpr int PASSES = (NT + P - 1) / P;
    float* resbuf = lds;
    float* colbuf = lds + RES_FLOATS;
    float* red = colbuf + COL_FLOATS;
    const bool gelu = (g.flags & kGemmGelu) != 0, relu = (g.flags & kGemmRelu) != 0, swish = (g.flags & kGemmSwish) != 0;
    static_for<NT>([&](auto Q) {
        constexpr int q = decltype(Q)::value;
        *reinterpret_cast<float4*>(resbuf + (q * 4 + wave) * 256 + lane * 4) =
            make_float4(eo.res[q][0], eo.res[q][1], eo.res[q][2], eo.res[q][3]);
    });
    if (wave == 0 && lane < 32) {
        static_for<TN>([&](auto J) {
            constexpr int j = decltype(J)::value;
            colbuf[j * 32 + lane] = eo.bias[j];
            colbuf[128 + j * 32 + lane] = eo.mul[j];
        });
    }
    static_for<PASSES>([&](auto PP) {
        constexpr int pass = decltype(PP)::value, q_lo = pass * P, q_hi = (q_lo + P < NT ? q_lo + P : NT);
        if constexpr (pass > 0) lds_barrier();
        static_for<q_hi - q_lo>([&](auto T) {
            constexpr int t = decltype(T)::value, q = q_lo + t, i = q / TN, j = q % TN;
            float* dst = red + (t * 4 + wave) * 1024 + lane * 4;
            static_for<4>([&](auto V) {
                constexpr int v = decltype(V)::value;
                *reinterpret_cast<float4*>(dst + v * 256) =
                    make_float4(acc[i][j][4 * v], acc[i][j][4 * v + 1], acc[i][j][4 * v + 2], acc[i][j][4 * v + 3]);
            });
        });
        lds_barrier();
#pragma unroll 1
        for (int q = q_lo; q < q_hi; ++q) {
            const float* p = red + ((q - q_lo) * 4) * 1024 + wave * 256 + lane * 4;
            float4 s4 = *reinterpret_cast<const float4*>(p);
#pragma unroll
            for (int w = 1; w < 4; ++w) {
                const float4 t4 = *reinterpret_cast<const float4*>(p + w * 1024);
                s4.x += t4.x; s4.y += t4.y; s4.z += t4.z; s4.w += t4.w;
            }
            const float4 r4 = *reinterpret_cast<const float4*>(resbuf + (q * 4 + wave) * 256 + lane * 4);
            const int i = q / TN, j = q - i * TN;
            const float b = colbuf[j * 32 + (lane & 31)], mul = colbuf[128 + j * 32 + (lane & 31)];
            const int col = n0 + 32 * j + (lane & 31);
            const int row0 = m0 + 32 * i + 8 * wave + 4 * (lane >> 5);
            if (col < g.N) {
                const float res[4] = {r4.x, r4.y, r4.z, r4.w};
                float v[4] = {(s4.x + b) * mul, (s4.y + b) * mul, (s4.z + b) * mul, (s4.w + b) * mul};
                if (gelu) {
#pragma unroll
                    for (int e = 0; e < 4; ++e) v[e] = gelu_erf(v[e]);
                }
                if (relu) {
#pragma unroll
                    for (int e = 0; e < 4; ++e) v[e] = fmaxf(v[e], 0.f);
                }
                if (swish) {
#pragma unroll
                    for (int e = 0; e < 4; ++e) v[e] = v[e] / (1.0f + expf(-v[e]));
                }
                float* out = gC + (long)row0 * g.ldc + col;
#pragma unroll
                for (int e = 0; e < 4; ++e)
                    if (row0 + e < g.M) out[(long)e * g.ldc] = v[e] + res[e];
            }
        }
    });
}

typedef float f32x4v __attribute__((ext_vector_type(4)));
template <int TM, int TN>
struct KPipeCfg {
    static constexpr int BM = 32 * TM, BN = 32 * TN, KS = 32, NB = 4;
    static constexpr int A_PIECES = BM / 8, W_PIECES = BN / 8;
    static constexpr int PIECES_PER_WAVE = (A_PIECES + W_PIECES) / 4;
    static constexpr int SLAB_FLOATS = (BM + BN) * KS;
    static constexpr int RED_FLOATS = TM * TN * 1024 + 512 + 2 * 4096;
    static constexpr int LDS_FLOATS = (NB * SLAB_FLOATS > RED_FLOATS ? NB * SLAB_FLOATS : RED_FLOATS);
    static constexpr size_t LDS_BYTES = (size_t)LDS_FLOATS * sizeof(float);
};

template <int N>
__device__ __forceinline__ void wait_vmcnt() {
    static_assert(N >= 0 && N < 64, "vmcnt range");
    if constexpr (N == 0) asm volatile("s_waitcnt vmcnt(0)" ::: "memory");
#define WLK_VM(n) else if constexpr (N == n) asm volatile("s_waitcnt vmcnt(" #n ")" ::: "memory");
    WLK_VM(6) WLK_VM(8) WLK_VM(10) WLK_VM(12) WLK_VM(14)
#undef WLK_VM
    else static_assert(N < 0, "add the vmcnt literal");
}

template <int N>
__device__ __forceinline__ void wait_lgkm_tied(f32x4v* f) {
    static_assert(N >= 3 && N <= 7, "operand list");
    if constexpr (N == 3) asm volatile("s_waitcnt lgkmcnt(0)" : "+v"(f[0]), "+v"(f[1]), "+v"(f[2]));
    else if constexpr (N == 4) asm volatile("s_waitcnt lgkmcnt(0)" : "+v"(f[0]), "+v"(f[1]), "+v"(f[2]), "+v"(f[3]));
    else if constexpr (N == 5) asm volatile("s_waitcnt lgkmcnt(0)" : "+v"(f[0]), "+v"(f[1]), "+v"(f[2]), "+v"(f[3]), "+v"(f[4]));
    else if constexpr (N == 6) asm volatile("s_waitcnt lgkmcnt(0)" : "+v"(f[0]), "+v"(f[1]), "+v"(f[2]), "+v"(f[3]), "+v"(f[4]), "+v"(f[5]));
    else
        asm volatile("s_waitcnt lgkmcnt(0)" : "+v"(f[0]), "+v"(f[1]), "+v"(f[2]), "+v"(f[3]), "+v"(f[4]), "+v"(f[5]), "+v"(f[6]));
}

template <int TM, int TN>
__global__ __launch_bounds__(256) void gemm_nt_f32_kpipe_kernel(GemmArgs g) {
    WLK_PIN_GEMM_ARGS(g);
    using Cfg = KPipeCfg<TM, TN>;
    constexpr int BM = Cfg::BM, BN = Cfg::BN, NP = Cfg::PIECES_PER_WAVE, KS = Cfg::KS, NB = Cfg::NB;
    constexpr int DT = NB - 1;
    constexpr int NF = TM + TN;
    static_assert(NF <= 7, "fragment operand list");
    extern __shared__ __attribute__((aligned(1024))) float lds[];
    const long long t_start = g.dbg_clock ? (long long)__builtin_readcyclecounter() : 0;
    const int lane = threadIdx.x & 63;
    const int wave = __builtin_amdgcn_readfirstlane(threadIdx.x >> 6);
    const bool batched = g.batch > 0;
    const float* const gA = batched ? table_at(g.z.in, blockIdx.y) : g.A;
    float* const gC = batched ? table_at(g.z.out, blockIdx.y) : g.C;
    const float* const gR = batched ? table_at(g.z.res, blockIdx.y) : g.R;
    const int tiles_m = (g.M + BM - 1) / BM, tiles_n = (g.N + BN - 1) / BN;
    int tile_m, tile_n;
    if (tiles_m >= 8) {
        const int band_m = (tiles_m + 3) / 4, band_n = (tiles_n + 1) / 2;
        const int xcd = blockIdx.x & 7, slot = blockIdx.x >> 3;
        tile_m = (xcd >> 1) * band_m + slot / band_n;
        tile_n = (xcd & 1) * band_n + slot % band_n;
        if (slot >= band_m * band_n || tile_m >= tiles_m || tile_n >= tiles_n) return;
    } else {
        tile_m = blockIdx.x / tiles_n;
        tile_n = blockIdx.x - tile_m * tiles_n;
        if (tile_m >= tiles_m) return;
    }
    const int m0 = tile_m * BM, n0 = tile_n * BN;

    const float* src[NP];
#pragma unroll
    for (int i = 0; i < NP; ++i) {
        const int j = wave + 4 * i;
        const bool is_a = j < Cfg::A_PIECES;
        const int jj = is_a ? j : j - Cfg::A_PIECES;
        const int row_local = jj * 8 + (lane >> 3);
        const int chunk = (lane & 7) ^ ((row_local >> 1) & 7);
        if (is_a) src[i] = gA + (long)min(m0 + row_local, g.M - 1) * g.lda + chunk * 4;
        else src[i] = g.W + (long)min(n0 + row_local, g.N - 1) * g.K + chunk * 4;
    }
    const int nslab = g.K / KS;
    auto issue_piece = [&](auto I, int slab, int slot) {
        constexpr int i = decltype(I)::value;
        const int j = wave + 4 * i;
        __builtin_amdgcn_global_load_lds((const __attribute__((address_space(1))) void*)(src[i] + (long)min(slab, nslab - 1) * KS),
                                         (__attribute__((address_space(3))) void*)(lds + slot * Cfg::SLAB_FLOATS + j * 256), 16, 0, 0);
    };

    const unsigned lds_base = (unsigned)(size_t)(__attribute__((address_space(3))) float*)lds;
    const int c0 = 2 * wave + (lane >> 5);
    unsigned f_addr[NF];
#pragma unroll
    for (int t = 0; t < TM; ++t) {
        const int r = 32 * t + (lane & 31);
        f_addr[t] = lds_base + (unsigned)(((r >> 3) * 64 + (r & 7) * 8 + (c0 ^ ((r >> 1) & 7))) * 16);
    }
#pragma unroll
    for (int t = 0; t < TN; ++t) {
        const int r = 32 * t + (lane & 31);
        f_addr[TM + t] = lds_base + (unsigned)(Cfg::A_PIECES * 1024 + ((r >> 3) * 64 + (r & 7) * 8 + (c0 ^ ((r >> 1) & 7))) * 16);
    }
    auto read_frags = [&](f32x4v (&f)[NF], int slab) {
        const unsigned off = (unsigned)(slab % NB) * (unsigned)(Cfg::SLAB_FLOATS * 4);
#pragma unroll
        for (int t = 0; t < NF; ++t) asm volatile("ds_read_b128 %0, %1" : "=v"(f[t]) : "v"(f_addr[t] + off));
    };

    f32x16 acc[TM][TN];
#pragma unroll
    for (int i = 0; i < TM; ++i)
#pragma unroll
        for (int j = 0; j < TN; ++j)
#pragma unroll
            for (int r = 0; r < 16; ++r) acc[i][j][r] = 0.f;

    constexpr int NMF = 4 * TM * TN;
    constexpr int HEAD = NMF / 2;
    constexpr int GAP = HEAD / NP >= 1 ? HEAD / NP : 1;
    static_assert(NP <= HEAD, "more DMA pieces than head MFMAs");

    EpilogueOperands<TM, TN> eo;
    ksplit_fetch_epilogue<TM, TN>(g, eo, wave, lane, m0, n0, gR);
    static_for<DT>([&](auto S) {
        constexpr int sl = decltype(S)::value;
        static_for<NP>([&](auto I) { issue_piece(I, sl, sl % NB); });
    });
    wait_vmcnt<(DT - 1) * NP>();
    __builtin_amdgcn_s_barrier();
    f32x4v f0[NF], f1[NF];
    read_frags(f0, 0);
    wait_lgkm_tied<NF>(f0);

    auto trip = [&](f32x4v (&f)[NF], f32x4v (&fn)[NF], int tt) {
        auto mfma_at = [&](auto X) {
            constexpr int x = decltype(X)::value;
            constexpr int c = x / (TM * TN), q = x % (TM * TN), i = q / TN, j = q % TN;
            acc[i][j] = __builtin_amdgcn_mfma_f32_32x32x2f32(f[i][c], f[TM + j][c], acc[i][j], 0, 0, 0);
        };
        static_for<HEAD>([&](auto X) {
            constexpr int x = decltype(X)::value;
            mfma_at(X);
            if constexpr (x % GAP == GAP - 1 && x / GAP < NP) {
                const int slab = tt + DT;
                issue_piece(std::integral_constant<int, x / GAP>{}, slab, slab % NB);
            }
        });
        __builtin_amdgcn_sched_barrier(0);
        wait_vmcnt<(DT - 1) * NP>();
        __builtin_amdgcn_s_barrier();
        read_frags(fn, tt + 1);
        __builtin_amdgcn_sched_barrier(0);
        static_for<NMF - HEAD>([&](auto X) { mfma_at(std::integral_constant<int, HEAD + decltype(X)::value>{}); });
        __builtin_amdgcn_sched_barrier(0);
        wait_lgkm_tied<NF>(fn);
    };
    const long long t_loop = g.dbg_clock ? (long long)__builtin_readcyclecounter() : 0;
    const int ntrip = nslab;
    int tt = 0;
    for (; tt + 1 < ntrip; tt += 2) {
        trip(f0, f1, tt);
        trip(f1, f0, tt + 1);
    }
    if (tt < ntrip) trip(f0, f1, tt);
    wait_vmcnt<0>();
    __syncthreads();
    const long long t_fold = g.dbg_clock ? (long long)__builtin_readcyclecounter() : 0;

    ksplit_fold_store<TM, TN, Cfg::LDS_FLOATS>(g, acc, eo, lds, wave, lane, m0, n0, gC);
    if (g.dbg_clock && threadIdx.x == 0) {
        long long* d = g.dbg_clock + 4 * ((long)blockIdx.y * gridDim.x + blockIdx.x);
        d[0] = t_start; d[1] = t_loop; d[2] = t_fold; d[3] = (long long)__builtin_readcyclecounter();
    }
}

template <int TM, int TN>
static void launch_kpipe(const LaunchCtx& ctx, const GemmArgs& g) {
    using Cfg = KPipeCfg<TM, TN>;
    static_assert(Cfg::LDS_BYTES <= 160 * 1024, "ring does not fit the 160 KiB LDS");
    static std::atomic<uint64_t> configured{0};
    int dev = 0;
    WLK_HIP(hipGetDevice(&dev));
    if (!(configured.load(std::memory_order_acquire) >> (dev & 63) & 1)) {
        WLK_HIP(hipFuncSetAttribute(reinterpret_cast<const void*>(&gemm_nt_f32_kpipe_kernel<TM, TN>),
                                    hipFuncAttributeMaxDynamicSharedMemorySize, (int)Cfg::LDS_BYTES));
        configured.fetch_or(1ull << (dev & 63), std::memory_order_release);
    }
    const int tiles_m = (g.M + Cfg::BM - 1) / Cfg::BM, tiles_n = (g.N + Cfg::BN - 1) / Cfg::BN;
    const int blocks = tiles_m >= 8 ? 8 * ((tiles_m + 3) / 4) * ((tiles_n + 1) / 2) : tiles_m * tiles_n;
    hipLaunchKernelGGL((gemm_nt_f32_kpipe_kernel<TM, TN>), dim3(blocks, std::max(g.batch, 1)), dim3(256), Cfg::LDS_BYTES,
                       ctx.stream, g);
}

static bool dispatch_kpipe(const LaunchCtx& ctx, const GemmArgs& g, int tm, int tn) {
#define WLK_KP(a, b) if (tm == a && tn == b) { launch_kpipe<a, b>(ctx, g); return true; }
    WLK_KP(3, 4) WLK_KP(3, 3) WLK_KP(3, 2) WLK_KP(3, 1) WLK_KP(2, 4) WLK_KP(2, 2) WLK_KP(2, 1) WLK_KP(4, 2)
#undef WLK_KP
    return false;
}

struct KSplitTile { int tm, tn; };
static KSplitTile ksplit_tile(int M, int N, int K, bool forced = false) {
    if (K % 64 != 0 || K < 256 || M < 512) return {0, 0};
    if (!forced && (N > 1536 || K < 512)) return {0, 0};
    static const KSplitTile cand[] = {{3, 4}, {3, 3}, {3, 2}, {3, 1}, {2, 4}, {2, 2}, {2, 1}, {4, 2}};
    KSplitTile best{0, 0};
    double best_cost = 0.0;
    for (const KSplitTile& c : cand) {
        const long tiles = (long)((M + 32 * c.tm - 1) / (32 * c.tm)) * ((N + 32 * c.tn - 1) / (32 * c.tn));
        const double cost = ((tiles + 255) / 256) * (c.tm * c.tn * (K / 8.0) + 48.0 + 2.0 * (c.tm + c.tn) * (K / 64.0));
        if (best.tm == 0 || cost < best_cost) { best = c; best_cost = cost; }
    }
    return best;
}

static long kwave_max_tiles() {
    static const long v = [] {
        const char* e = getenv("WLK_KWAVE_MAX_TILES");
        return e ? atol(e) : 416L;
    }();
    return v;
}

bool gemm_takes_kwave(int M, int N, int K) {
    const long tiles32 = (long)((N + 31) / 32) * ((M + 31) / 32);
    return K >= 256 && tiles32 <= kwave_max_tiles();
}

bool gemm_takes_ksplit(int M, int N, int K) { return ksplit_tile(M, N, K).tm != 0; }

void x3_refresh_env_switches();
void refresh_env_switches() { x3_refresh_env_switches(); }

void launch_gemm(const LaunchCtx& ctx, const GemmArgs& g, const char* tag) {
    if (g.M <= 0 || g.N <= 0) return;
    if (g.K % 4 != 0 || g.lda % 4 != 0) throw std::invalid_argument("gemm: K and lda must be multiples of 4");
    if ((((long)g.M - 1) * g.lda + g.K) * 4 >= (1L << 31) || (long)g.N * g.K * 4 >= (1L << 31))
        throw std::invalid_argument("gemm: operand larger than 2 GiB");
    if (g.ln_gamma) throw std::invalid_argument("gemm: only the GEMV kernels (rows <= 8) take the LayerNorm; launch it separately");
    const double nb = std::max(g.batch, 1);
    KernelScope ks(ctx, tag, nb * 2.0 * g.M * g.N * g.K,
                   4.0 * (nb * (double)g.M * g.K + (double)g.N * g.K + nb * (double)g.M * g.N));
    if (g.batch > kMaxBatch) throw std::invalid_argument("gemm: batch too large");
    const bool want_kwave = g.force_kwave || g.force_kernel == 2;
    const KSplitTile kt = (want_kwave || g.kcache || g.force_kernel == 3) ? KSplitTile{0, 0} : ksplit_tile(g.M, g.N, g.K, g.force_kernel == 4);
    if (g.force_kernel == 4 && !kt.tm) throw std::invalid_argument("gemm: the k-pipe kernel does not take this shape");
    if (kt.tm) {
        if (!dispatch_kpipe(ctx, g, kt.tm, kt.tn)) throw std::logic_error("gemm: k-pipe tile without an instantiation");
        WLK_HIP(hipGetLastError());
        return;
    }
    if (g.batch > 0 && (gemm_takes_kwave(g.M, g.N, g.K) || want_kwave || (long)((g.N + 63) / 64) * ((g.M + 63) / 64) < 64))
        throw std::invalid_argument("gemm: batched launches are only available on the tiled paths");
    const long tiles64 = (long)((g.N + 63) / 64) * ((g.M + 63) / 64);
    const int tiles_n = (g.N + 63) / 64;
    const long tiles32 = (long)((g.N + 31) / 32) * ((g.M + 31) / 32);
    if (g.kcache && !(gemm_takes_kwave(g.M, g.N, g.K) || want_kwave))
        throw std::invalid_argument("gemm: fused KV-cache append is only available on the k-wave path");
    if ((gemm_takes_kwave(g.M, g.N, g.K) && g.force_kernel != 3) || (want_kwave && g.K >= 256)) {
        if (g.M <= 128 && g.force_kernel != 2) {
            const long tiles16 = (long)((g.N + 15) / 16) * ((g.M + 15) / 16);
            hipLaunchKernelGGL(gemm_nt_f32_kwave16_kernel<>, dim3((unsigned)tiles16), dim3(256), 0, ctx.stream, g);
        } else {
            hipLaunchKernelGGL(gemm_nt_f32_kwave_kernel<false>, dim3((unsigned)tiles32), dim3(256), 0, ctx.stream, g);
        }
    } else if (tiles64 >= 64) {
        const int tiles_m = (g.M + 63) / 64;
        const int blocks = tiles_m >= 8 ? 8 * ((tiles_m + 3) / 4) * ((tiles_n + 1) / 2) : tiles_m * tiles_n;
        hipLaunchKernelGGL((gemm_nt_f32_kernel<64, 64>), dim3(blocks, std::max(g.batch, 1)), dim3(256), 0, ctx.stream, g);
    } else {
        const int tiles_m = (g.M + 31) / 32;
        const int blocks = tiles_m >= 8 ? 8 * ((tiles_m + 3) / 4) * ((tiles_n + 1) / 2) : tiles_m * tiles_n;
        hipLaunchKernelGGL((gemm_nt_f32_kernel<32, 64>), dim3(blocks), dim3(128), 0, ctx.stream, g);
    }
    WLK_HIP(hipGetLastError());
}

static bool kp16_rule(int M, int N, int K, long tiles16) {
    if (N <= 512 && K <= 1024) return true;
    if (K > 1024) return M <= 320;
    if (N == 1024) return M <= 320;
    return tiles16 <= 1300;
}
static KSplitTile kp_tile(int M, int N, int K) {
    const int band = M < 900 ? 0 : M < 1800 ? 1 : M < 2800 ? 2 : 3;
    struct Row { int n, k; int t[4][2]; };
    static const Row rows[] = {
        {2048, 512, {{3, 2}, {2, 1}, {2, 2}, {2, 1}}},
        {512, 2048, {{2, 1}, {3, 1}, {3, 2}, {2, 4}}},
        {1536, 512, {{3, 2}, {2, 2}, {2, 2}, {2, 2}}},
        {512, 512, {{2, 1}, {3, 1}, {3, 2}, {2, 4}}},
        {1024, 512, {{3, 1}, {3, 2}, {2, 1}, {2, 1}}},
        {192, 768, {{2, 1}, {2, 1}, {2, 1}, {3, 1}}},
        {192, 512, {{2, 1}, {2, 1}, {2, 1}, {3, 1}}},
    };
    for (const Row& r : rows)
        if (r.n == N && r.k == K) return KSplitTile{r.t[band][0], r.t[band][1]};
    if (N == 256 && K == 256) return M < 4000 ? KSplitTile{2, 1} : M < 9000 ? KSplitTile{2, 2} : KSplitTile{2, 1};
    return ksplit_tile(M, N, K, true);
}
static bool kp_takes_16(int M, int N, int K, int force) {
    if (force == 6) return true;
    if (force == 7 || force == 8) return false;
    const long tiles16 = (long)((N + 15) / 16) * ((M + 15) / 16);
    return kp16_rule(M, N, K, tiles16);
}
bool gemm_kp_takes_kpipe(int M, int N, int K) { return K % 128 == 0 && K >= 256 && M >= 512 && ksplit_tile(M, N, K, true).tm != 0; }
void launch_gemm_kp(const LaunchCtx& ctx, const GemmArgs& g, const char* tag) {
    if (g.M <= 0 || g.N <= 0) return;
    if (g.K % 4 != 0 || g.lda % 4 != 0) throw std::invalid_argument("gemm: K and lda must be multiples of 4");
    if (g.batch > 0 || g.kcache) throw std::invalid_argument("gemm (kp family): plain projections only");
    if (g.ln_gamma) throw std::invalid_argument("gemm (kp family): the LayerNorm is a launch of its own");
    const bool short_k_kwave = g.K % 32 == 0 && g.K >= 128 && g.K < 256;
    if (!short_k_kwave && (g.K % 128 != 0 || g.K < 256)) {
        GemmArgs p = g;
        p.force_kernel = 3;
        launch_gemm(ctx, p, tag);
        return;
    }
    if ((((long)g.M - 1) * g.lda + g.K) * 4 >= (1L << 31) || (long)g.N * g.K * 4 >= (1L << 31))
        throw std::invalid_argument("gemm: operand larger than 2 GiB");
    KernelScope ks(ctx, tag, 2.0 * g.M * g.N * g.K, 4.0 * ((double)g.M * g.K + (double)g.N * g.K + (double)g.M * g.N));
    if (!short_k_kwave && gemm_kp_takes_kpipe(g.M, g.N, g.K)) {
        KSplitTile kt = kp_tile(g.M, g.N, g.K);
        if (g.force_kernel >= 500) kt = KSplitTile{(g.force_kernel - 500) / 10, (g.force_kernel - 500) % 10};
        if (!dispatch_kpipe(ctx, g, kt.tm, kt.tn)) throw std::logic_error("gemm: k-pipe tile without an instantiation");
    } else if ((!short_k_kwave || g.M < 512) && kp_takes_16(g.M, g.N, g.K, g.force_kernel)) {
        const long tiles16 = (long)((g.N + 15) / 16) * ((g.M + 15) / 16);
        hipLaunchKernelGGL((gemm_nt_f32_kwave16_kernel<true>), dim3((unsigned)tiles16), dim3(256), 0, ctx.stream, g);
    } else {
        const long tiles32 = (long)((g.N + 31) / 32) * ((g.M + 31) / 32);
        const bool one_buf = g.force_kernel == 8 || (g.force_kernel != 7 && tiles32 > 512);
        if (one_buf) hipLaunchKernelGGL((gemm_nt_f32_kwave_kernel<true, 1>), dim3((unsigned)tiles32), dim3(256), 0, ctx.stream, g);
        else hipLaunchKernelGGL(gemm_nt_f32_kwave_kernel<true>, dim3((unsigned)tiles32), dim3(256), 0, ctx.stream, g);
    }
    WLK_HIP(hipGetLastError());
}

template <int MR, int RPW>
__global__ __launch_bounds__(256) void gemv_f32_kernel(GemmArgs g) {
    WLK_PIN_GEMM_ARGS(g);
    extern __shared__ __attribute__((aligned(16))) float xs[];
    const int side = g.side_blocks;
    if ((int)blockIdx.x < side) {
        const AlignArgs a = *g.side_align;
        const int fblock = (int)blockIdx.x % g.side_zf, rest = (int)blockIdx.x / g.side_zf;
        align_zscore_body(a, fblock, rest % a.n_align, rest / a.n_align);
        return;
    }
    const int blk = (int)blockIdx.x - side, n_blk = (int)gridDim.x - side;
    const int tid = threadIdx.x;
    const int lane = tid & 63;
    const int wave = tid >> 6;
    const int K4 = g.K >> 2;
    const int n_groups = (g.N + RPW - 1) / RPW;
    const int grp0 = blk * 4 + wave;
    float4 wpre[RPW];
#pragma unroll
    for (int r = 0; r < RPW; ++r) {
        const int n = min(grp0 * RPW + r, g.N - 1);
        const bool ok = grp0 < n_groups && lane < K4;
        const float4 t = *reinterpret_cast<const float4*>(g.W + (long)(ok ? n : 0) * g.K + (ok ? lane : 0) * 4);
        wpre[r] = t;
    }
    constexpr int kLnKeep = 8;
    [[maybe_unused]] float gq[kLnKeep], bq[kLnKeep];
    {
        const float* gp = g.ln_gamma ? g.ln_gamma : g.W;
        const float* bp = g.ln_gamma ? g.ln_beta : g.W;
#pragma unroll
        for (int i = 0; i < kLnKeep; ++i) {
            const int c = lane + 64 * i;
            gq[i] = gp[c < g.K ? c : 0];
            bq[i] = bp[c < g.K ? c : 0];
        }
    }
    const int ep_r = lane / MR, ep_m = lane - ep_r * MR;
    const int ep_n0 = min(grp0 * RPW + (ep_r < RPW ? ep_r : 0), g.N - 1);
    const int ep_mm = ep_m < g.M ? ep_m : 0;
    const float bias0 = (g.bias ? g.bias + ep_n0 : g.W)[0];
    const float res0 = ((g.flags & kGemmResidual) ? g.R + (long)ep_mm * g.ldr + ep_n0 : g.W)[0];
    static_assert(sizeof(StepRow) == 64, "the dummy StepRow read below stays inside the first weight row");
    const StepRow kv_row0 = (g.kv_rows ? g.kv_rows + ep_mm : reinterpret_cast<const StepRow*>(g.W))[0];
    const int kv_pos0 = (g.kcache ? g.kv_pos : reinterpret_cast<const int*>(g.W))[0];
    for (int i = tid; i < MR * K4; i += 256) {
        const int m = i / K4, c = i - m * K4;
        float4 v = make_float4(0.f, 0.f, 0.f, 0.f);
        if (m < g.M) v = *reinterpret_cast<const float4*>(g.A + (long)m * g.lda + c * 4);
        reinterpret_cast<float4*>(xs)[i] = v;
    }
    __syncthreads();
    if (g.ln_gamma) {
        for (int m = wave; m < g.M; m += 4) {
            float* xr = xs + m * g.K;
            float sum = 0.f;
            for (int c = lane; c < g.K; c += 64) sum += xr[c];
            sum = wave_sum(sum);
            const float mean = sum / (float)g.K;
            float sq = 0.f;
            for (int c = lane; c < g.K; c += 64) {
                const float t = xr[c] - mean;
                sq += t * t;
            }
            sq = wave_sum(sq);
            const float rstd = 1.0f / sqrtf(sq / (float)g.K + 1e-5f);
#pragma unroll
            for (int i = 0; i < kLnKeep; ++i) {
                const int c = lane + 64 * i;
                if (c < g.K) xr[c] = (xr[c] - mean) * rstd * gq[i] + bq[i];
            }
            for (int c = lane + 64 * kLnKeep; c < g.K; c += 64) xr[c] = (xr[c] - mean) * rstd * g.ln_gamma[c] + g.ln_beta[c];
        }
// ... 548 lines not shown
```

whisperlivekit_amd/csrc/gemm_x3.hip:

```cpp
#include <atomic>
#include <cstdint>
#include <cstdlib>
#include <type_traits>

#include "common.h"
#include "x3.h"

namespace wlk {

typedef float xf32x16 __attribute__((ext_vector_type(16)));
typedef float xf32x4 __attribute__((ext_vector_type(4)));

__device__ __attribute__((noinline)) float x3_gelu_erf(float x) { return 0.5f * x * (1.0f + erff(x * 0.70710678118654752440f)); }

template <int N, int I = 0, typename F>
__device__ __forceinline__ void x3_static_for(F&& f) {
    if constexpr (I < N) {
        f(std::integral_constant<int, I>{});
        x3_static_for<N, I + 1>(f);
    }
}

__global__ __launch_bounds__(256) void x3_pack_kernel(const float* __restrict__ src, long ld_src, unsigned short* __restrict__ dst,
                                                      long ld_dst, int rows, int cols) {
    const int chunks = cols >> 3;
    const long idx = (long)blockIdx.x * 256 + threadIdx.x;
    if (idx >= (long)rows * chunks) return;
    const int row = (int)(idx / chunks), q = (int)(idx - (long)row * chunks);
    const float4 a = *reinterpret_cast<const float4*>(src + (long)row * ld_src + q * 8);
    const float4 b = *reinterpret_cast<const float4*>(src + (long)row * ld_src + q * 8 + 4);
    const float v[8] = {a.x, a.y, a.z, a.w, b.x, b.y, b.z, b.w};
    x3_store_chunk(dst + (long)row * 3 * ld_dst + (long)q * 24, v);
}

void x3_pack_check(long ld_src, long ld_dst, int cols) {
    if (cols % 8 != 0 || ld_src % 4 != 0 || ld_dst % 8 != 0) throw std::invalid_argument("x3 pack: columns must be whole chunks of 8");
}

void launch_x3_pack(const LaunchCtx& ctx, const float* src, long ld_src, unsigned short* dst, long ld_dst, int rows, int cols) {
    x3_pack_check(ld_src, ld_dst, cols);
    const long n = (long)rows * (cols / 8);
    if (n <= 0) return;
    KernelScope ks(ctx, "x3_pack");
    hipLaunchKernelGGL(x3_pack_kernel, dim3((unsigned)((n + 255) / 256)), dim3(256), 0, ctx.stream, src, ld_src, dst, ld_dst, rows, cols);
    WLK_HIP(hipGetLastError());
}

__global__ __launch_bounds__(256) void x3_unpack_kernel(const unsigned short* __restrict__ src, long ld_src, float* __restrict__ dst,
                                                        long ld_dst, int rows, int cols) {
    const long idx = (long)blockIdx.x * 256 + threadIdx.x;
    if (idx >= (long)rows * cols) return;
    const int row = (int)(idx / cols), k = (int)(idx - (long)row * cols);
    const unsigned short* u = src + (long)row * 3 * ld_src + (long)(k >> 3) * 24 + (k & 7);
    const float h = __uint_as_float((unsigned)u[0] << 16), m = __uint_as_float((unsigned)u[8] << 16), l = __uint_as_float((unsigned)u[16] << 16);
    dst[(long)row * ld_dst + k] = (h + m) + l;
}

void launch_x3_unpack(const LaunchCtx& ctx, const unsigned short* src, long ld_src, float* dst, long ld_dst, int rows, int cols) {
    const long n = (long)rows * cols;
    if (n <= 0) return;
    KernelScope ks(ctx, "x3_unpack");
    hipLaunchKernelGGL(x3_unpack_kernel, dim3((unsigned)((n + 255) / 256)), dim3(256), 0, ctx.stream, src, ld_src, dst, ld_dst, rows, cols);
    WLK_HIP(hipGetLastError());
}

size_t x3_w_elems(int n, int k) { return (size_t)((n + 31) / 32 * 32) * 3 * (size_t)k; }

__global__ __launch_bounds__(256) void x3_pack_w_kernel(const float* __restrict__ src, long ld_src, unsigned short* __restrict__ dst,
                                                        int n, int k) {
    const int nslab = k >> 5;
    const long idx = (long)blockIdx.x * 256 + threadIdx.x;
    const long total = (long)((n + 31) / 32) * nslab * 2 * 64;
    if (idx >= total) return;
    const int l = (int)(idx & 63), s2 = (int)((idx >> 6) & 1);
    const long bt = idx >> 7;
    const int t = (int)(bt % nslab), nb = (int)(bt / nslab);
    const int row = 32 * nb + (l & 31), k0 = 32 * t + 16 * s2 + 8 * (l >> 5);
    float v[8];
#pragma unroll
    for (int e = 0; e < 8; ++e) v[e] = row < n ? src[(long)row * ld_src + k0 + e] : 0.f;
    unsigned h[4], m[4], lo[4];
#pragma unroll
    for (int i = 0; i < 4; ++i) {
        const X3Triple x = x3_split(v[2 * i]), y = x3_split(v[2 * i + 1]);
        h[i] = x3_bits(x.h) | (x3_bits(y.h) << 16);
        m[i] = x3_bits(x.m) | (x3_bits(y.m) << 16);
        lo[i] = x3_bits(x.l) | (x3_bits(y.l) << 16);
    }
    x3_u32x4* d = reinterpret_cast<x3_u32x4*>(reinterpret_cast<char*>(dst) + (((long)nb * nslab + t) * 2 + s2) * 3072 + 16 * l);
    d[0] = x3_u32x4{h[0], h[1], h[2], h[3]};
    d[64] = x3_u32x4{m[0], m[1], m[2], m[3]};
    d[128] = x3_u32x4{lo[0], lo[1], lo[2], lo[3]};
}

void launch_x3_pack_w(const LaunchCtx& ctx, const float* src, long ld_src, unsigned short* dst, int n, int k) {
    if (k % 32 != 0 || n <= 0) throw std::invalid_argument("x3 weight pack: K must be a multiple of 32");
    const long total = (long)((n + 31) / 32) * (k / 32) * 128;
    KernelScope ks(ctx, "x3_pack_w");
    hipLaunchKernelGGL(x3_pack_w_kernel, dim3((unsigned)((total + 255) / 256)), dim3(256), 0, ctx.stream, src, ld_src, dst, n, k);
    WLK_HIP(hipGetLastError());
}

namespace {
constexpr int XW_BM = 96, XW_BN = 128;
constexpr int XW_ROW_BYTES = 192;
constexpr int XW_SLAB_BYTES = XW_BM * XW_ROW_BYTES;
constexpr int XW_LOADERS = 3;
constexpr int XW_NB = 5;
constexpr int XW_DT = XW_NB - 1;
constexpr int XW_WSLAB_BYTES = 6 * 1024;
constexpr int XW_STAGE_PITCH = XW_BN + 4;
constexpr int XW_STAGE_OFF = XW_NB * XW_SLAB_BYTES;
constexpr int XW_WPITCH = 36;
constexpr size_t XW_LDS_BYTES = (size_t)XW_STAGE_OFF + (size_t)4 * XW_BM * XW_WPITCH * 4;
static_assert((size_t)4 * XW_BM * XW_WPITCH >= (size_t)XW_BM * XW_STAGE_PITCH, "the staging region holds either transpose");
}

namespace {
constexpr int XK_CW = 8;
constexpr int XK_WAVES = XK_CW + XW_LOADERS;
constexpr int XK_THREADS = XK_WAVES * 64;
template <int NRB>
__device__ __forceinline__ void xk_read(xf32x4 (&f)[NRB], unsigned addr) {
    asm volatile("ds_read_b128 %0, %1" : "=v"(f[0]) : "v"(addr));
    asm volatile("ds_read_b128 %0, %1 offset:6144" : "=v"(f[1]) : "v"(addr));
    if constexpr (NRB == 3) asm volatile("ds_read_b128 %0, %1 offset:12288" : "=v"(f[2]) : "v"(addr));
}
static_assert(32 * XW_ROW_BYTES == 6144, "row-block stride of the fragment reads");
template <int NRB>
__device__ __forceinline__ void xk_wait(xf32x4 (&a)[NRB], xf32x4 (&b)[NRB], xf32x4 (&c)[NRB]) {
    asm volatile("s_waitcnt lgkmcnt(0)" : "+v"(a[0]), "+v"(a[1]), "+v"(b[0]), "+v"(b[1]), "+v"(c[0]), "+v"(c[1]));
    if constexpr (NRB == 3) asm volatile("" : "+v"(a[2]), "+v"(b[2]), "+v"(c[2]));
}
template <int NPW>
__device__ __forceinline__ void xk_wait_landed() {
    static_assert(NPW == 6 || NPW == 4, "update the vmcnt literals");
    if constexpr (NPW == 6) asm volatile("s_waitcnt vmcnt(18)" ::: "memory");
    else asm volatile("s_waitcnt vmcnt(12)" ::: "memory");
}
static_assert(XW_DT - 1 == 3, "xk_wait_landed's literals are 3 slabs of NPW pieces");
}

template <int BM>
__global__ __launch_bounds__(XK_THREADS) void gemm_x3_wide2_kernel(X3GemmArgs g) {
    constexpr int NRB = BM / 32;
    constexpr int SLAB_BYTES = BM * XW_ROW_BYTES;
    constexpr int NPW = SLAB_BYTES / 1024 / XW_LOADERS;
    constexpr int STAGE_OFF = XW_NB * SLAB_BYTES;
    static_assert(NPW * XW_LOADERS * 1024 == SLAB_BYTES, "a slab is a whole number of 1 KiB pieces per loader");
    asm volatile("" ::"s"(g.A3), "s"(g.lda), "s"(g.W3), "s"(g.bias), "s"(g.C), "s"(g.ldc), "s"(g.R), "s"(g.ldr), "s"(g.M),
                 "s"(g.N), "s"(g.K), "s"(g.flags), "s"(g.scale), "s"(g.scale_cols), "s"(g.scale_period), "s"(g.batch));
    __builtin_amdgcn_sched_barrier(0);
    extern __shared__ __attribute__((aligned(1024))) unsigned char lds[];
    const int lane = threadIdx.x & 63;
    const int wave = __builtin_amdgcn_readfirstlane(threadIdx.x >> 6);
    const bool batched = g.batch > 0;
    const int tiles_m = (g.M + BM - 1) / BM, tiles_n = (g.N + XW_BN - 1) / XW_BN;
    const bool banded = g.walk_banded != 0;
    const int band_m = banded ? (tiles_m + 3) / 4 : tiles_m, band_n = banded ? (tiles_n + 1) / 2 : tiles_n;
    const int per_session = band_m * band_n;
    const int xcd = banded ? (int)(blockIdx.x & 7) : 0;
    const int first = banded ? (int)(blockIdx.x >> 3) : (int)blockIdx.x;
    const int stride = banded ? (int)(gridDim.x >> 3) : (int)gridDim.x;
    const int limit = g.walk_slots;
    const int band_m0 = banded ? (xcd >> 1) * band_m : 0, band_n0 = banded ? (xcd & 1) * band_n : 0;
    auto decode = [&](int slot, int& tm, int& tn, int& b) -> bool {
        b = slot / per_session;
        const int r = slot - b * per_session;
        int rm, cn;
        if (g.walk_colmajor) {
            cn = r / band_m;
            rm = r - cn * band_m;
        } else {
            rm = r / band_n;
            cn = r - rm * band_n;
        }
        tm = band_m0 + rm;
        tn = band_n0 + cn;
        return tm < tiles_m && tn < tiles_n;
    };
    auto advance = [&](int slot) {
        int tm, tn, b;
        while (slot < limit && !decode(slot, tm, tn, b)) slot += stride;
        return slot;
    };
    const int slot0 = advance(first);
    if (slot0 >= limit) return;
    const int nslab = g.K / 32;
    const bool x3_out = g.x3_out;

    auto shared_epilogue = [&](int m0, int n0, int bz) {
        float* const gC = batched ? table_at(g.z.out, (unsigned)bz) : g.C;
        const float* const gR = batched ? table_at(g.z.res, (unsigned)bz) : g.R;
        const float* const stage = reinterpret_cast<const float*>(lds + STAGE_OFF);
        const int colq = lane & 7, rsub = lane >> 3;
        constexpr int ITEMS = 4 * (BM / 8);
        auto bias_of_item = [&](int k) -> xf32x4 {
            const int c = min(n0 + 32 * (min(k, ITEMS - 1) / (BM / 8)) + 4 * colq, g.N - 4);
            return g.bias ? *reinterpret_cast<const xf32x4*>(g.bias + c) : xf32x4{0.f, 0.f, 0.f, 0.f};
        };
        xf32x4 bq = bias_of_item(wave);
        asm volatile("s_waitcnt lgkmcnt(0)" ::: "memory");
        __builtin_amdgcn_s_barrier();
        const bool gelu = (g.flags & kGemmGelu) != 0, has_res = (g.flags & kGemmResidual) != 0;
#pragma unroll 1
        for (int k = wave; k < ITEMS; k += XK_WAVES) {
            const xf32x4 bq_next = bias_of_item(k + XK_WAVES);
            const int wp = k / (BM / 8), it = k - wp * (BM / 8);
            const int row_t = 8 * it + rsub, row = m0 + row_t;
            const int col = n0 + 32 * wp + 4 * colq;
            xf32x4 v = *reinterpret_cast<const xf32x4*>(stage + (wp * BM + row_t) * XW_WPITCH + 4 * colq);
            const xf32x4 res = has_res ? *reinterpret_cast<const xf32x4*>(gR + (long)min(row, g.M - 1) * g.ldr + min(col, g.N - 4))
                                       : xf32x4{0.f, 0.f, 0.f, 0.f};
#pragma unroll
            for (int e = 0; e < 4; ++e) {
                v[e] += bq[e];
                if ((g.flags & kGemmScaleCols) && (g.scale_period ? (col + e) % g.scale_period : col + e) < g.scale_cols) v[e] *= g.scale;
                if (gelu) v[e] = x3_gelu_erf(v[e]);
                v[e] += res[e];
            }
            if (row < g.M && col < g.N) *reinterpret_cast<xf32x4*>(gC + (long)row * g.ldc + col) = v;
            bq = bq_next;
        }
    };

    if (wave >= XK_CW) {
        const int lw = wave - XK_CW;
        const char* src[NPW];
        int row_of[NPW], unit_of[NPW];
#pragma unroll
        for (int i = 0; i < NPW; ++i) {
            const int byte = 1024 * (lw + XW_LOADERS * i) + 16 * lane;
            row_of[i] = byte / XW_ROW_BYTES;
            unit_of[i] = (((byte - row_of[i] * XW_ROW_BYTES) >> 4) ^ ((row_of[i] >> 2) & 3)) * 16;
        }
        auto set_src = [&](int slot) {
            int tm, tn, b;
            decode(slot, tm, tn, b);
            const int m0 = tm * BM;
            const char* const gA = reinterpret_cast<const char*>(batched ? reinterpret_cast<const unsigned short*>(table_at(g.z.in, (unsigned)b)) : g.A3);
#pragma unroll
            for (int i = 0; i < NPW; ++i) src[i] = gA + (long)min(m0 + row_of[i], g.M - 1) * g.lda * 6 + unit_of[i];
        };
        int issue_slot = slot0, s_next = 0, ring = 0;
        bool more = true;
        set_src(issue_slot);
        auto issue_one = [&]() {
            const long adv = (long)s_next * XW_ROW_BYTES;
            unsigned char* const dst = lds + ring * SLAB_BYTES + lw * 1024;
            x3_static_for<NPW>([&](auto I) {
                constexpr int i = decltype(I)::value;
                __builtin_amdgcn_global_load_lds((const __attribute__((address_space(1))) void*)(src[i] + adv),
                                                 (__attribute__((address_space(3))) void*)(dst + i * XW_LOADERS * 1024), 16, 0, 0);
            });
            ring = ring == XW_NB - 1 ? 0 : ring + 1;
            if (more && ++s_next == nslab) {
                const int ns = advance(issue_slot + stride);
                if (ns < limit) {
                    issue_slot = ns;
                    set_src(ns);
                    s_next = 0;
                } else {
                    more = false;
                    s_next = nslab - 1;
                }
            }
        };
#pragma unroll
        for (int i = 0; i < XW_DT; ++i) issue_one();
        xk_wait_landed<NPW>();
        __builtin_amdgcn_s_barrier();
        for (int slot = slot0; slot < limit; slot = advance(slot + stride)) {
            for (int tt = 0; tt < nslab; ++tt) {
                issue_one();
                xk_wait_landed<NPW>();
                __builtin_amdgcn_s_barrier();
            }
            __builtin_amdgcn_s_barrier();
            if (x3_out) {
                __builtin_amdgcn_s_barrier();
                __builtin_amdgcn_s_barrier();
            } else {
                int tm, tn, bz;
                decode(slot, tm, tn, bz);
                shared_epilogue(tm * BM, tn * XW_BN, bz);
            }
        }
        asm volatile("s_waitcnt vmcnt(0)" ::: "memory");
        __builtin_amdgcn_s_barrier();
        return;
    }

    const int cb = wave & 3, half = wave >> 2;
    const unsigned lds_base = (unsigned)(size_t)(__attribute__((address_space(3))) unsigned char*)lds;
    const int r = lane & 31, hi = lane >> 5, swz = (r >> 2) & 3;
    unsigned fa[3];
#pragma unroll
    for (int p = 0; p < 3; ++p) fa[p] = lds_base + (unsigned)(r * XW_ROW_BYTES) + (unsigned)((((2 * half + hi) * 3 + p) ^ swz) * 16);
    xf32x16 acc[NRB];
    auto mfma3 = [&](const xf32x4& w, const xf32x4 (&f)[NRB]) {
#pragma unroll
        for (int i = 0; i < NRB; ++i)
            acc[i] = __builtin_amdgcn_mfma_f32_32x32x16_bf16(__builtin_bit_cast(bf16x8, w), __builtin_bit_cast(bf16x8, f[i]), acc[i], 0, 0, 0);
    };
    const int n_blocks = (g.N + 31) / 32;
    typedef const __attribute__((address_space(1))) xf32x4* wptr_t;
    auto w_base = [&](int slot) -> const char* {
        int tm, tn, bz;
        decode(slot, tm, tn, bz);
        return reinterpret_cast<const char*>(g.W3) + (long)min(4 * tn + cb, n_blocks - 1) * nslab * XW_WSLAB_BYTES + half * (XW_WSLAB_BYTES / 2) + 16 * lane;
    };
    const int col_in_tile = 32 * cb + 4 * hi;
    auto load_bias = [&](int slot, xf32x4 (&b)[4]) {
        int tm, tn, bz;
        decode(slot, tm, tn, bz);
        if (x3_out && half == 0) {
#pragma unroll
            for (int j = 0; j < 4; ++j) {
                const int c = min(tn * XW_BN + col_in_tile + 8 * j, g.N - 4);
                b[j] = g.bias ? *reinterpret_cast<const xf32x4*>(g.bias + c) : xf32x4{0.f, 0.f, 0.f, 0.f};
            }
        }
    };
    xf32x4 wa[3], wb[3];
#pragma unroll
    for (int x = 0; x < 3; ++x) wb[x] = xf32x4{0.f, 0.f, 0.f, 0.f};
    const char* w_cur = w_base(slot0);
#pragma unroll
    for (int x = 0; x < 3; ++x) wa[x] = *(wptr_t)(w_cur + 1024 * x);
    xf32x4 bias_next[4];
#pragma unroll
    for (int j = 0; j < 4; ++j) bias_next[j] = xf32x4{0.f, 0.f, 0.f, 0.f};
// ... 258 lines not shown
```

whisperlivekit_amd/csrc/internal.h:

```cpp
#pragma once
#include <algorithm>
#include <map>
#include <memory>
#include <chrono>
#include <cstdlib>
#include <thread>
#include <mutex>
#include <stdexcept>
#include <string>
#include <vector>

#include "../../include/wlk_hip.h"
#include "common.h"

namespace wlk {

const std::string& get_last_error();

template <typename F>
inline int guarded(F&& f) {
    try {
        return f();
    } catch (const HipError& e) {
        set_last_error(e.what());
// ... 4 lines not shown
    } catch (const std::invalid_argument& e) {
        set_last_error(e.what());
        return WLK_ERR_ARG;
    } catch (const std::exception& e) {
        set_last_error(e.what());
        return WLK_ERR_STATE;
    }
}
inline int fail(int code, const std::string& msg) {
    set_last_error(msg);
    return code;
}


struct Profiler {
    struct Rec {
        const char* name;
        hipEvent_t a, b;
        double flops, bytes;
    };
    std::vector<Rec> recs;
    std::vector<hipEvent_t> pool;
    hipEvent_t pending = nullptr;
    const char* pending_name = nullptr;
    double pending_flops = 0.0, pending_bytes = 0.0;
    hipEvent_t get() {
        if (!pool.empty()) {
            hipEvent_t e = pool.back();
            pool.pop_back();
            return e;
        }
        hipEvent_t e;
        WLK_HIP(hipEventCreate(&e));
        return e;
    }
};

struct TensorSlot {
    std::string name;
    uint64_t offset, numel;
};


struct LayerW {
    const float *ln1w, *ln1b, *qkvw, *qkvb, *outw, *outb, *ln2w, *ln2b, *fc1w, *fc1b, *fc2w, *fc2b;
    const float *lnxw = nullptr, *lnxb = nullptr, *xqw = nullptr, *xqb = nullptr, *xkvw = nullptr, *xkvb = nullptr,
                *xoutw = nullptr, *xoutb = nullptr;
    const unsigned short *qkvw3 = nullptr, *fc1w3 = nullptr;
    const unsigned short *outw3 = nullptr, *fc2w3 = nullptr;
};

template <typename T>
inline T* dev_alloc(size_t n) {
    T* p = nullptr;
    WLK_HIP(hipMalloc(reinterpret_cast<void**>(&p), n * sizeof(T)));
    return p;
}
template <typename T>
inline T* dev_alloc_zero(size_t n, hipStream_t s) {
    T* p = dev_alloc<T>(n);
    WLK_HIP(hipMemsetAsync(p, 0, n * sizeof(T), s));
    return p;
}

}

struct wlk_engine;
struct wlk_session;
struct wlk_model;

struct wlk_prefill_ws {
    int cap_rows = 0;
    int cap_session_rows = 0;
    float *dx = nullptr, *dh = nullptr, *dqkv = nullptr, *datt = nullptr, *dq = nullptr, *dmlp = nullptr, *hsel = nullptr,
          *logits = nullptr, *part = nullptr;
    wlk::StepRow *rows_dev = nullptr, *tiles_dev = nullptr;
    int *ring_row_dev = nullptr, *zeros_dev = nullptr;
    char* pinned = nullptr;
    size_t pinned_bytes = 0;
};
struct wlk_prefill_item {
    wlk_session* s = nullptr;
    const int64_t* tokens = nullptr;
    int n_tok = 0, sot_index = 0;
    int rc = 0;
    std::string err;
};

struct wlk_model {
    wlk_dims D{};
    int device = 0;
    float* arena = nullptr;
    bool owns_arena = false;
    uint64_t arena_floats = 0;
    std::vector<wlk::TensorSlot> slots;
    std::map<std::string, const wlk::TensorSlot*> by_name;
    double* twiddle = nullptr;
    float* xkv_all_w = nullptr;
    float* xkv_all_b = nullptr;
    unsigned short* xkv_all_w3 = nullptr;
    std::vector<unsigned short*> x3_owned;
    int* filt_lo = nullptr;
    int* filt_hi = nullptr;
    int* head_rank = nullptr;
    int* layer_ranks = nullptr;
    int* layer_heads = nullptr;
    int* all_ranks = nullptr;
    std::vector<int> layer_rank_count;
    std::vector<int> align_pairs;
    int n_align = 0;
    bool finalized = false;
    std::vector<wlk::LayerW> enc_layers, dec_layers;
    const float *w_tok_emb = nullptr, *w_dec_pos = nullptr, *w_ln_w = nullptr, *w_ln_b = nullptr;
    wlk_engine* engine = nullptr;
    std::mutex engine_mu;
    float* cif_w = nullptr;
    float cif_b = 0.f;

    const float* w(const std::string& name) const {
        auto it = by_name.find(name);
        if (it == by_name.end()) throw std::invalid_argument("unknown tensor " + name);
        return arena + it->second->offset;
    }
};


struct wlk_session {
    wlk_model* m = nullptr;
    int beam = 1;
    int audio_cap = 0;
    hipStream_t stream = nullptr;
    wlk::Profiler prof;
    bool prof_on = false;
    bool debug = false;
    bool use_graph = true;
    hipGraphExec_t step_exec[2] = {nullptr, nullptr};
    short* pcm16_dev = nullptr;

    float* audio[2] = {nullptr, nullptr};
    int audio_cur = 0;
    int audio_len = 0;

    float *logmel = nullptr, *frame_max = nullptr, *mel_t = nullptr;
    float *logmel_alt = nullptr, *frame_max_alt = nullptr;
    int mel_cached_samples = 0, mel_cached_frames = 0, mel_dirty_head = 0;
    bool mel_incremental = true;
    int frame_cap = 0;
    float *x1p = nullptr, *ex = nullptr, *eh = nullptr, *eqkv = nullptr, *eatt = nullptr, *emlp = nullptr,
          *enc_out = nullptr, *cross_kv = nullptr;
    unsigned short *eh3 = nullptr, *enc_out3 = nullptr;
    unsigned short* emlp3 = nullptr;
    bool enc_out_is_x3 = false;
    unsigned short* eqkv3 = nullptr;
    bool encoded = false;
    int content_len = 0;

    int max_rows = 0;
    int* tokens_dev = nullptr;
    float *dx = nullptr, *dh = nullptr, *dqkv = nullptr, *datt = nullptr, *dq = nullptr, *dmlp = nullptr;
    float* kcache[2] = {nullptr, nullptr};
    float* vcache[2] = {nullptr, nullptr};
    int kv_cur = 0;
    int self_len = 0;
    int n_steps = 0;
    int prefill_rows = 0;
    int last_rows = 0, last_ntok = 0;
    float *hsel = nullptr, *logits_last = nullptr, *logits_sot = nullptr;
    bool have_sot = false;
    int* step_in = nullptr;
    int *ring_row = nullptr, *beam_of_row = nullptr, *d_offset = nullptr;
    float* ring = nullptr;
    int ring_rows = 0;
    float *z = nullptr, *attn_last = nullptr;
    float* qk_debug = nullptr;
    float* xsplit = nullptr;
    float* fsplit = nullptr;
    static constexpr int kFlashSplitsMax = 16;
    static int flash_splits();

    int *adj_row = nullptr, *src_rows = nullptr;
    float* top_vals = nullptr;
    void* topk_scratch = nullptr;
    int *top_ids = nullptr, *frames = nullptr;
    float* probs = nullptr;
    static constexpr int kAdjCap = 4096;
    void* pinned = nullptr;
    static constexpr size_t kPinnedBytes = 1 << 20;
    void* dec_stage = nullptr;
    hipEvent_t dec_stage_ev = nullptr;
    bool dec_stage_used = false;
    void* audio_stage = nullptr;
    hipEvent_t audio_stage_ev = nullptr;
    unsigned char* rules_mask = nullptr;
    int* pick_out = nullptr;
    bool audio_stage_used = false;
    wlk::StepBlock *step_host = nullptr, *step_host_dev = nullptr, *step_dev = nullptr;
    wlk::StepResult *result_host = nullptr, *result_host_dev = nullptr;
    hipGraphExec_t fstep_exec[2] = {nullptr, nullptr};
    wlk::AlignArgs* step_align_dev = nullptr;
    unsigned step_seq = 0;
    uint64_t step_ns = 0, step_launch_ns = 0, step_count = 0;

    unsigned char* anc = nullptr;
    hipGraphExec_t bstep_exec[2] = {nullptr, nullptr};
    bool anc_live = false;
    uint64_t anc_steps = 0;

    wlk::LaunchCtx ctx() { return wlk::LaunchCtx{stream, prof_on ? &prof : nullptr}; }
    bool align_raw_scores = false;
    float* wa_buf = nullptr;
    size_t wa_cap = 0;
    wlk_engine* engine = nullptr;
    float* cif_alpha = nullptr;
    wlk_cif_out *cif_host = nullptr, *cif_host_dev = nullptr;
    unsigned cif_seq = 0;
    int cif_T = -1;
    hipStream_t cif_stream = nullptr;
};


inline wlk::StepRow next_step_row(const wlk_session* s, int token, int content_len) {
    const int ctx_len = s->m->D.n_text_ctx;
    const int after = s->n_steps + 1;
    wlk::StepRow r;
    r.kcache = s->kcache[s->kv_cur];
    r.vcache = s->vcache[s->kv_cur];
    r.cross_kv = s->cross_kv;
    r.ring = s->ring;
    r.token = token;
    r.offset = s->self_len;
    r.ring_row = ctx_len + ((s->n_steps - 1) % wlk::kAlignWindow);
    r.prefill_rows = after <= wlk::kAlignWindow ? s->prefill_rows : 0;
    r.n_single = std::min(after - 1, wlk::kAlignWindow);
    r.newest_row = ctx_len + ((after - 2) % wlk::kAlignWindow);
    r.content_len = content_len;
    r.pad = 0;
    return r;
}

inline void wlk_wait_step_flags(hipStream_t stream, const wlk::StepResult* res, int n, unsigned seq) {
    static const long spin_us = [] {
        const char* e = getenv("WLK_STEP_SPIN_US");
        return e ? atol(e) : 400L;
    }();
    const auto t_start = std::chrono::steady_clock::now();
    auto all_set = [&]() {
        for (int i = 0; i < n; ++i)
            if (__atomic_load_n(&res[i].flag_topk, __ATOMIC_ACQUIRE) != seq || __atomic_load_n(&res[i].flag_align, __ATOMIC_ACQUIRE) != seq)
                return false;
        return true;
    };
    bool spinning = true;
    for (unsigned looks = 0;; ++looks) {
        if (all_set()) return;
        if ((looks & 0x3ff) == 0x3ff) {
            const hipError_t q = hipStreamQuery(stream);
            if (q == hipSuccess) {
                if (all_set()) return;
                throw std::runtime_error("graph step: the replay finished without delivering its result");
            }
            if (q != hipErrorNotReady) WLK_HIP(q);
        }
        if (spinning) {
            __builtin_ia32_pause();
            if ((looks & 0x3f) == 0x3f &&
                std::chrono::steady_clock::now() - t_start > std::chrono::microseconds(spin_us))
                spinning = false;
            continue;
        }
        const auto waited = std::chrono::steady_clock::now() - t_start;
        if (waited > std::chrono::seconds(30)) throw std::runtime_error("graph step: no result after 30 s");
        if (waited > std::chrono::milliseconds(2)) std::this_thread::sleep_for(std::chrono::microseconds(50));
        else std::this_thread::yield();
    }
}

int wlk_step_select(wlk_session* s, int64_t token, const int32_t* adj_ids, const float* adj_deltas, int n_adj,
                    int content_mel_len, float* top_logprobs2, int32_t* top_ids2, int32_t* frame);
int wlk_beam_step(wlk_session* s, const int64_t* tokens, const int32_t* source_rows);
int wlk_select_first(wlk_session* s, int no_speech_token, const int32_t* adj_row, const int32_t* adj_ids,
                     const float* adj_deltas, int n_adj, int k, int content_mel_len, float* no_speech_host,
                     float* top_logprobs_host, int32_t* top_ids_host, int32_t* frames_host);
void wlk_encode_group(const std::vector<wlk_session*>& group, const wlk::LaunchCtx& c, std::vector<int>& content_out,
                      bool mel_given = false);
std::string wlk_encode_precheck(const wlk_session* s, const wlk_model* m);

std::string wlk_prefill_precheck(const wlk_prefill_item& it, const wlk_prefill_ws& ws);
void wlk_prefill_group(const std::vector<wlk_prefill_item*>& items, const wlk::LaunchCtx& c, wlk_prefill_ws& ws);
void wlk_prefill_ws_alloc(const wlk_model* m, wlk_prefill_ws& ws, int max_sessions, int session_rows);
void wlk_prefill_ws_free(wlk_prefill_ws& ws);

void wlk_cif_session_prepare(wlk_session* s);
void wlk_cif_session_free(wlk_session* s);
void wlk_cif_enqueue(const std::vector<wlk_session*>& group, const wlk::LaunchCtx& c, const std::vector<int>& content);

int wlk_engine_prefill(wlk_session* s, const int64_t* tokens, int n_tok, int sot_index);
bool wlk_engine_batches_encodes(const wlk_session* s);
int wlk_engine_encode(wlk_session* s, int* content_mel_len);
namespace wlk { struct DecodeJob; }
void wlk_engine_destroy_for_model(wlk_model* m);
bool wlk_engine_wants(const wlk_session* s);
void wlk_engine_loop_enter(wlk_session* s);
void wlk_engine_loop_exit(wlk_session* s);
int wlk_engine_run_job(wlk_session* s, wlk::DecodeJob* job);
```

whisperlivekit_amd/csrc/layernorm.hip:

```cpp
#include "common.h"
#include "wave_ops.h"
#include "x3.h"

namespace wlk {

constexpr int kLnMaxPerLane = 24;

template <int NPL>
__global__ __launch_bounds__(256) void layernorm_kernel(const float* __restrict__ x, long ldx,
                                                        const float* __restrict__ gamma,
                                                        const float* __restrict__ beta, float* __restrict__ y,
                                                        long ldy, int rows, int d, PtrTable z, int batch) {
    const int lane = threadIdx.x & 63;
    const int row = blockIdx.x * 4 + (threadIdx.x >> 6);
    if (row >= rows) return;
    if (x == nullptr) {
        x = table_at(z.in, blockIdx.y);
        y = table_at(z.out, blockIdx.y);
    }
    const float* xr = x + (long)row * ldx;
    float v[NPL], g[NPL], b[NPL];
#pragma unroll
    for (int i = 0; i < NPL; ++i) {
        const int c = lane + 64 * i;
        const int cc = c < d ? c : 0;
        v[i] = xr[cc];
        g[i] = gamma[cc];
        b[i] = beta[cc];
    }
#pragma unroll
    for (int i = 0; i < NPL; ++i) { pin_loaded(g[i]); pin_loaded(b[i]); }
    __builtin_amdgcn_sched_barrier(0);
    float sum = 0.f;
#pragma unroll
    for (int i = 0; i < NPL; ++i) {
        v[i] = (lane + 64 * i) < d ? v[i] : 0.f;
        sum += v[i];
    }
    sum = wave_sum(sum);
    const float mean = sum / (float)d;
    float sq = 0.f;
#pragma unroll
    for (int i = 0; i < NPL; ++i) {
        const int c = lane + 64 * i;
        const float t = c < d ? v[i] - mean : 0.f;
        sq += t * t;
    }
    sq = wave_sum(sq);
    const float rstd = 1.0f / sqrtf(sq / (float)d + 1e-5f);
    float* yr = y + (long)row * ldy;
#pragma unroll
    for (int i = 0; i < NPL; ++i) {
        const int c = lane + 64 * i;
        if (c < d) yr[c] = (v[i] - mean) * rstd * g[i] + b[i];
    }
}

template <int NPL>
__global__ __launch_bounds__(256) void layernorm_x3_kernel(const float* __restrict__ x, long ldx,
                                                           const float* __restrict__ gamma,
                                                           const float* __restrict__ beta, unsigned short* __restrict__ y3,
                                                           long ldy3, int rows, int d, PtrTable z) {
    constexpr int NCH = (NPL + 7) / 8;
    const int lane = threadIdx.x & 63;
    const int row = blockIdx.x * 4 + (threadIdx.x >> 6);
    if (row >= rows) return;
    if (x == nullptr) {
        x = table_at(z.in, blockIdx.y);
        y3 = reinterpret_cast<unsigned short*>(table_at(z.out, blockIdx.y));
    }
    const float* xr = x + (long)row * ldx;
    const int n_chunks = d >> 3;
    float v[NPL];
    float4 xc[NCH][2], gc[NCH][2], bc[NCH][2];
#pragma unroll
    for (int i = 0; i < NPL; ++i) {
        const int c = lane + 64 * i;
        v[i] = xr[c < d ? c : 0];
    }
#pragma unroll
    for (int j = 0; j < NCH; ++j) {
        const int q = lane + 64 * j;
        const int at = (q < n_chunks ? q : 0) * 8;
        xc[j][0] = *reinterpret_cast<const float4*>(xr + at);
        xc[j][1] = *reinterpret_cast<const float4*>(xr + at + 4);
        gc[j][0] = *reinterpret_cast<const float4*>(gamma + at);
        gc[j][1] = *reinterpret_cast<const float4*>(gamma + at + 4);
        bc[j][0] = *reinterpret_cast<const float4*>(beta + at);
        bc[j][1] = *reinterpret_cast<const float4*>(beta + at + 4);
    }
#pragma unroll
    for (int j = 0; j < NCH; ++j) {
        pin_loaded(xc[j][0]); pin_loaded(xc[j][1]);
        pin_loaded(gc[j][0]); pin_loaded(gc[j][1]);
        pin_loaded(bc[j][0]); pin_loaded(bc[j][1]);
    }
    __builtin_amdgcn_sched_barrier(0);
    float sum = 0.f;
#pragma unroll
    for (int i = 0; i < NPL; ++i) {
        v[i] = (lane + 64 * i) < d ? v[i] : 0.f;
        sum += v[i];
    }
    sum = wave_sum(sum);
    const float mean = sum / (float)d;
    float sq = 0.f;
#pragma unroll
    for (int i = 0; i < NPL; ++i) {
        const float t = (lane + 64 * i) < d ? v[i] - mean : 0.f;
        sq += t * t;
    }
    sq = wave_sum(sq);
    const float rstd = 1.0f / sqrtf(sq / (float)d + 1e-5f);
    unsigned short* yr = y3 + (long)row * 3 * ldy3;
#pragma unroll
    for (int j = 0; j < NCH; ++j) {
        const int q = lane + 64 * j;
        const float o[8] = {(xc[j][0].x - mean) * rstd * gc[j][0].x + bc[j][0].x, (xc[j][0].y - mean) * rstd * gc[j][0].y + bc[j][0].y,
                            (xc[j][0].z - mean) * rstd * gc[j][0].z + bc[j][0].z, (xc[j][0].w - mean) * rstd * gc[j][0].w + bc[j][0].w,
                            (xc[j][1].x - mean) * rstd * gc[j][1].x + bc[j][1].x, (xc[j][1].y - mean) * rstd * gc[j][1].y + bc[j][1].y,
                            (xc[j][1].z - mean) * rstd * gc[j][1].z + bc[j][1].z, (xc[j][1].w - mean) * rstd * gc[j][1].w + bc[j][1].w};
        if (q < n_chunks) x3_store_chunk(yr + (long)q * 24, o);
    }
}

template <typename... Args>
static void launch_ln_x3_by_width(int d, dim3 grid, hipStream_t stream, Args... args) {
    const int npl = (d + 63) / 64;
    if (npl <= 8) hipLaunchKernelGGL(layernorm_x3_kernel<8>, grid, dim3(256), 0, stream, args...);
    else if (npl <= 12) hipLaunchKernelGGL(layernorm_x3_kernel<12>, grid, dim3(256), 0, stream, args...);
    else if (npl <= 16) hipLaunchKernelGGL(layernorm_x3_kernel<16>, grid, dim3(256), 0, stream, args...);
    else if (npl <= 20) hipLaunchKernelGGL(layernorm_x3_kernel<20>, grid, dim3(256), 0, stream, args...);
    else hipLaunchKernelGGL(layernorm_x3_kernel<kLnMaxPerLane>, grid, dim3(256), 0, stream, args...);
}

template <typename... Args>
static void launch_ln_by_width(int d, dim3 grid, hipStream_t stream, Args... args) {
    const int npl = (d + 63) / 64;
    if (npl <= 8) hipLaunchKernelGGL(layernorm_kernel<8>, grid, dim3(256), 0, stream, args...);
    else if (npl <= 12) hipLaunchKernelGGL(layernorm_kernel<12>, grid, dim3(256), 0, stream, args...);
    else if (npl <= 16) hipLaunchKernelGGL(layernorm_kernel<16>, grid, dim3(256), 0, stream, args...);
    else if (npl <= 20) hipLaunchKernelGGL(layernorm_kernel<20>, grid, dim3(256), 0, stream, args...);
    else hipLaunchKernelGGL(layernorm_kernel<kLnMaxPerLane>, grid, dim3(256), 0, stream, args...);
}

void layernorm_check(int d, long ldx, long ldy3, bool x3, int batch) {
    if (d > 64 * kLnMaxPerLane || batch > kMaxBatch) throw std::invalid_argument("layernorm: d or batch too large");
    if (x3 && (d % 8 != 0 || ldx % 4 != 0 || ldy3 % 8 != 0)) throw std::invalid_argument("layernorm (x3): unsupported width");
}

void launch_layernorm(const LaunchCtx& ctx, const float* x, long ldx, const float* gamma, const float* beta,
                      float* y, long ldy, int rows, int d, const char* tag) {
    if (rows <= 0) return;
    layernorm_check(d, ldx, 0, false, 0);
    KernelScope ks(ctx, tag);
    launch_ln_by_width(d, dim3((rows + 3) / 4), ctx.stream, x, ldx, gamma, beta, y, ldy, rows, d, PtrTable{}, 0);
    WLK_HIP(hipGetLastError());
}

void launch_layernorm_batched(const LaunchCtx& ctx, const PtrTable& z, int batch, long ldx, const float* gamma,
                              const float* beta, long ldy, int rows, int d, const char* tag) {
    if (rows <= 0 || batch <= 0) return;
    layernorm_check(d, ldx, 0, false, batch);
    KernelScope ks(ctx, tag);
    launch_ln_by_width(d, dim3((rows + 3) / 4, batch), ctx.stream, (const float*)nullptr, ldx, gamma, beta, (float*)nullptr,
                       ldy, rows, d, z, batch);
    WLK_HIP(hipGetLastError());
}


void launch_layernorm_x3(const LaunchCtx& ctx, const float* x, long ldx, const float* gamma, const float* beta,
                         unsigned short* y3, long ldy3, int rows, int d, const char* tag) {
    if (rows <= 0) return;
    layernorm_check(d, ldx, ldy3, true, 0);
    KernelScope ks(ctx, tag);
    launch_ln_x3_by_width(d, dim3((rows + 3) / 4), ctx.stream, x, ldx, gamma, beta, y3, ldy3, rows, d, PtrTable{});
    WLK_HIP(hipGetLastError());
}

void launch_layernorm_x3_batched(const LaunchCtx& ctx, const PtrTable& z, int batch, long ldx, const float* gamma,
                                 const float* beta, long ldy3, int rows, int d, const char* tag) {
    if (rows <= 0 || batch <= 0) return;
    layernorm_check(d, ldx, ldy3, true, batch);
    KernelScope ks(ctx, tag);
    launch_ln_x3_by_width(d, dim3((rows + 3) / 4, batch), ctx.stream, (const float*)nullptr, ldx, gamma, beta,
                          (unsigned short*)nullptr, ldy3, rows, d, z);
    WLK_HIP(hipGetLastError());
}

}
```

whisperlivekit_amd/csrc/mel.hip:

```cpp
#include "common.h"

namespace wlk {

__global__ __launch_bounds__(256) void mel_frame_kernel(MelArgs a) {
    __shared__ double tw[kNFft];
    __shared__ float xw[kNFft];
    __shared__ float power[kNFreq + 3];
    __shared__ float red[256];

    const int t = (int)blockIdx.x < a.head ? (int)blockIdx.x : a.first + ((int)blockIdx.x - a.head);
    const int tid = threadIdx.x;
    for (int n = tid; n < kNFft; n += 256) {
        tw[n] = a.twiddle[n];
        int j = kHop * t - kNFft / 2 + n;
        if (j < 0) j = -j;
        if (j >= a.n_padded) j = 2 * (a.n_padded - 1) - j;
        const float s = j < a.n_samples ? a.audio[j] : 0.f;
        xw[n] = s * a.window[n];
    }
    __syncthreads();

    if (tid < kNFreq) {
        double re = 0.0, im = 0.0;
        int idx = 0;
#pragma unroll 8
        for (int n = 0; n < kNFft; ++n) {
            const double x = (double)xw[n];
            int sidx = idx + 300;
            if (sidx >= kNFft) sidx -= kNFft;
            re = fma(x, tw[idx], re);
            im = fma(-x, tw[sidx], im);
            idx += tid;
            if (idx >= kNFft) idx -= kNFft;
        }
        const float mag = hypotf((float)re, (float)im);
        power[tid] = mag * mag;
    }
    __syncthreads();

    float lm = -INFINITY;
    if (tid < a.n_mels) {
        const float* f = a.filters + (long)tid * kNFreq;
        float acc = 0.f;
        const int lo = a.filt_lo[tid], hi = a.filt_hi[tid];
        for (int k = lo; k < hi; ++k) acc = fmaf(f[k], power[k], acc);
        lm = log10f(fmaxf(acc, 1e-10f));
        a.logmel[(long)t * a.n_mels + tid] = lm;
    }
    red[tid] = lm;
    __syncthreads();
    for (int s = 128; s >= 1; s >>= 1) {
        if (tid < s) red[tid] = fmaxf(red[tid], red[tid + s]);
        __syncthreads();
    }
    if (tid == 0) a.frame_max[t] = red[0];
}

__global__ __launch_bounds__(256) void mel_finish_kernel(MelArgs a) {
    __shared__ float red[256];
    const int tid = threadIdx.x;
    float m = a.n_total > a.n_active ? -10.0f : -INFINITY;
    for (int i = tid; i < a.n_active; i += 256) m = fmaxf(m, a.frame_max[i]);
    red[tid] = m;
    __syncthreads();
    for (int s = 128; s >= 1; s >>= 1) {
        if (tid < s) red[tid] = fmaxf(red[tid], red[tid + s]);
        __syncthreads();
    }
    const float floor_v = red[0] - 8.0f;
    const long total = (long)kMelFrames * a.n_mels;
    for (long i = (long)blockIdx.x * 256 + tid; i < total; i += (long)gridDim.x * 256) {
        const int t = (int)(i / a.n_mels);
        const float v = t < a.n_active ? a.logmel[i] : -10.0f;
        a.mel_t[i + a.n_mels] = (fmaxf(v, floor_v) + 4.0f) / 4.0f;
    }
}

void launch_mel(const LaunchCtx& ctx, const MelArgs& a) {
    const int n_frames = a.head + (a.n_active - a.first);
    if (n_frames > 0) {
        KernelScope ks(ctx, "mel_frames");
        hipLaunchKernelGGL(mel_frame_kernel, dim3(n_frames), dim3(256), 0, ctx.stream, a);
        WLK_HIP(hipGetLastError());
    }
    {
        KernelScope ks(ctx, "mel_finish");
        hipLaunchKernelGGL(mel_finish_kernel, dim3(240), dim3(256), 0, ctx.stream, a);
        WLK_HIP(hipGetLastError());
    }
}

__global__ __launch_bounds__(256) void mel_full_max_kernel(const float* __restrict__ frame_max, int n_active, int n_total,
                                                           float* __restrict__ out) {
    __shared__ float red[256];
    const int tid = threadIdx.x;
    float m = n_total > n_active ? -10.0f : -INFINITY;
    for (int i = tid; i < n_active; i += 256) m = fmaxf(m, frame_max[i]);
    red[tid] = m;
    __syncthreads();
    for (int s = 128; s >= 1; s >>= 1) {
        if (tid < s) red[tid] = fmaxf(red[tid], red[tid + s]);
        __syncthreads();
    }
    if (tid == 0) out[0] = red[0];
}

__global__ __launch_bounds__(256) void mel_full_finish_kernel(const float* __restrict__ logmel, const float* __restrict__ gmax,
                                                              int n_mels, int n_active, int n_total, float* __restrict__ out) {
    __shared__ float tile[64 * 129];
    const int t0 = blockIdx.x * 64, tid = threadIdx.x;
    const float floor_v = gmax[0] - 8.0f;
    const int ld = n_mels + 1;
    for (int i = tid; i < 64 * n_mels; i += 256) {
        const int r = i / n_mels, c = i - r * n_mels, t = t0 + r;
        tile[r * ld + c] = t < n_active ? logmel[(long)t * n_mels + c] : -10.0f;
    }
    __syncthreads();
    for (int i = tid; i < 64 * n_mels; i += 256) {
        const int c = i >> 6, r = i & 63, t = t0 + r;
        if (t < n_total) out[(long)c * n_total + t] = (fmaxf(tile[r * ld + c], floor_v) + 4.0f) / 4.0f;
    }
}

void launch_mel_full(const LaunchCtx& ctx, const MelArgs& a, float* max_scratch, float* out) {
    if (a.n_mels > 128) throw std::invalid_argument("log-mel: more than 128 mel bins");
    if (a.n_active > 0) {
        KernelScope ks(ctx, "mel_frames");
        hipLaunchKernelGGL(mel_frame_kernel, dim3(a.n_active), dim3(256), 0, ctx.stream, a);
        WLK_HIP(hipGetLastError());
    }
    if (a.n_total > 0) {
        KernelScope ks(ctx, "mel_finish");
        hipLaunchKernelGGL(mel_full_max_kernel, dim3(1), dim3(256), 0, ctx.stream, a.frame_max, a.n_active, a.n_total, max_scratch);
        hipLaunchKernelGGL(mel_full_finish_kernel, dim3((a.n_total + 63) / 64), dim3(256), 0, ctx.stream, a.logmel, max_scratch,
                           a.n_mels, a.n_active, a.n_total, out);
        WLK_HIP(hipGetLastError());
    }
}

__global__ void pcm16_to_float_kernel(const short* __restrict__ in, float* __restrict__ out, int n) {
    const int i = blockIdx.x * blockDim.x + threadIdx.x;
    if (i < n) out[i] = (float)in[i] * (1.0f / 32768.0f);
}

void launch_pcm16_to_float(const LaunchCtx& ctx, const short* in, float* out, int n) {
    if (n <= 0) return;
    KernelScope ks(ctx, "pcm16_to_float", 0.0, 6.0 * n);
    hipLaunchKernelGGL(pcm16_to_float_kernel, dim3((n + 255) / 256), dim3(256), 0, ctx.stream, in, out, n);
    WLK_HIP(hipGetLastError());
}

}
```

Measured before the change: 206.0 audio_s/s.

## Recompute only the changed encoder stem rows across incremental chunks

Keeps the conv stem output and the layer-0 q|k|v image between calls. When new audio only appends frames and the global mel max is unchanged, a device-side row band limits the mel finish, conv1, conv2, layer-0 LN1 and q|k|v GEMMs to the affected rows. The band is written on the GPU by the mel kernel, so no host sync is needed. It saves stem and first-projection work for streaming chunks, at the cost of extra buffers and a correctness dependence on the band bounds. Later layers and attention still run over all rows.

```diff
diff --git a/whisperlivekit_amd/csrc/api.hip b/whisperlivekit_amd/csrc/api.hip
--- a/whisperlivekit_amd/csrc/api.hip
+++ b/whisperlivekit_amd/csrc/api.hip
@@ -425,6 +425,13 @@
             const bool attn_x3 = qkv_x3 && enc_attention_x3_enabled() && d == (size_t)D.n_audio_head * 64 && T >= 64 && (2 * d) % 128 == 0;
             if (any_x3) s->eh3 = dev_alloc<unsigned short>(T * 3 * d);
             if (attn_x3) s->eqkv3 = dev_alloc_zero<unsigned short>(x3_attn_image_elems((int)T, (int)d), st);
+            if (attn_x3 && !m->enc_layers.empty() && m->enc_layers[0].qkvw3 && 2 * T == (size_t)kMelFrames) {
+                s->x0 = dev_alloc<float>(T * d);
+                s->eqkv3_l0 = dev_alloc_zero<unsigned short>(x3_attn_image_elems((int)T, (int)d), st);
+                s->enc_max = dev_alloc_zero<float>(2, st);
+                s->enc_band = dev_alloc_zero<int>(kEncBandInts, st);
+                if (const char* e = std::getenv("WLK_ENC_REUSE")) s->enc_reuse_on = !(e[0] == '0');
+            }
             if (m->xkv_all_w3) s->enc_out3 = dev_alloc<unsigned short>(T * 3 * d);
         }
         s->cross_kv = dev_alloc<float>((size_t)D.n_text_layer * T * 2 * d);
@@ -512,6 +519,10 @@
     if (s->pcm16_dev) (void)hipFree(s->pcm16_dev);
     if (s->eh3) (void)hipFree(s->eh3);
     if (s->eqkv3) (void)hipFree(s->eqkv3);
+    if (s->x0) (void)hipFree(s->x0);
+    if (s->eqkv3_l0) (void)hipFree(s->eqkv3_l0);
+    if (s->enc_max) (void)hipFree(s->enc_max);
+    if (s->enc_band) (void)hipFree(s->enc_band);
     if (s->enc_out3) (void)hipFree(s->enc_out3);
     if (s->emlp3) (void)hipFree(s->emlp3);
     if (s->wa_buf) (void)hipFree(s->wa_buf);
@@ -640,6 +651,7 @@
         s->audio_cur ^= 1;
         s->audio_len = keep;
         s->encoded = false;
+        s->enc_reuse_valid = false;
         const int shift = n / kHop;
         if (s->mel_incremental && n % kHop == 0 && s->mel_cached_samples > n && shift < s->mel_cached_frames) {
             const int rows = s->mel_cached_frames - shift;
@@ -665,6 +677,7 @@
     s->audio_len = 0;
     s->encoded = false;
     s->mel_cached_samples = 0;
+    s->enc_reuse_valid = false;
     return WLK_OK;
 }
 
@@ -715,6 +728,8 @@
     for (int i = 0; i < B; ++i) {
         wlk_session* s = group[i];
         if (s->m != m) throw std::invalid_argument("encode: sessions of different models in one group");
+        const bool was_valid = s->enc_reuse_valid;
+        s->enc_reuse_valid = false;
         if (mel_given) {
             content_out[i] = D.n_audio_ctx;
             continue;
@@ -731,16 +746,38 @@
         ma.filt_lo = m->filt_lo; ma.filt_hi = m->filt_hi; ma.n_mels = D.n_mels;
         ma.logmel = s->logmel; ma.frame_max = s->frame_max; ma.mel_t = s->mel_t;
         ma.n_active = n_active; ma.n_total = n_total;
+        bool incremental = false;
         if (s->mel_incremental && s->mel_cached_samples > 0 && s->mel_cached_samples <= N && s->mel_cached_frames <= n_active) {
             int first = s->mel_cached_samples >= kNFft / 2 ? (s->mel_cached_samples - kNFft / 2) / kHop + 1 : 0;
             first = std::min(first, s->mel_cached_frames);
             ma.first = first;
             ma.head = std::min(s->mel_dirty_head, first);
+            incremental = true;
+        }
+        if (s->enc_band) {
+            ma.band = s->enc_band;
+            ma.band_T = T;
+            ma.prev_max = s->enc_max + s->enc_max_cur;
+            ma.new_max = s->enc_max + (s->enc_max_cur ^ 1);
+            s->enc_max_cur ^= 1;
+            ma.reuse = B == 1 && s->enc_reuse_on && was_valid && incremental && s->mel_dirty_head == 0;
+            const int f_hi = std::min(n_active, kMelFrames), f_lo = std::min(ma.first, f_hi);
+            if (ma.reuse && f_hi > f_lo) {
+                int* bc = ma.band_cand;
+                bc[kBandMel] = f_lo; bc[kBandMel + 1] = f_hi;
+                bc[kBandConv1] = std::max(f_lo - 1, 0); bc[kBandConv1 + 1] = std::min(f_hi + 1, kMelFrames);
+                bc[kBandConv2] = bc[kBandConv1] / 2; bc[kBandConv2 + 1] = std::min(bc[kBandConv1 + 1] / 2 + 1, T);
+                bc[kBandQkv] = bc[kBandConv2]; bc[kBandQkv + 1] = bc[kBandConv2 + 1];
+                const int lo = bc[kBandQkv], hi = bc[kBandQkv + 1];
+                bc[kBandLn1] = std::min(lo / 96 * 96, lo / 64 * 64);
+                bc[kBandLn1 + 1] = std::min(std::max((hi + 95) / 96 * 96, (hi + 63) / 64 * 64), T);
+            }
         }
         launch_mel(c, ma);
         s->mel_cached_samples = N;
         s->mel_cached_frames = n_active;
         s->mel_dirty_head = 0;
+        s->enc_reuse_valid = s->enc_band != nullptr;
     }
     auto table = [&](auto in, auto out, auto res) {
         PtrTable z{};
@@ -752,8 +789,16 @@
         return z;
     };
     auto none = [](wlk_session*) -> const float* { return nullptr; };
+    bool stem_keep = enc_attention_x3_enabled() && d == D.n_audio_head * 64 && T >= 64 && (2 * d) % 128 == 0 &&
+                     !m->enc_layers.empty() && m->enc_layers[0].qkvw3;
+    for (int i = 0; i < B; ++i) stem_keep = stem_keep && group[i]->x0 != nullptr;
+    const int* const band = stem_keep && B == 1 && !mel_given ? group[0]->enc_band : nullptr;
+    if (!stem_keep)
+        for (int i = 0; i < B; ++i) group[i]->enc_reuse_valid = false;
     auto gemm = [&](GemmArgs g, const PtrTable& z, const char* tag) {
         const bool stackable = !gemm_takes_kwave(g.M, g.N, g.K) && (long)((g.N + 63) / 64) * ((g.M + 63) / 64) >= 64;
+        if (gemm_takes_kwave(g.M, g.N, g.K) && !gemm_takes_ksplit(g.M, g.N, g.K))
+            g.row_band = nullptr;
         if (stackable) {
             g.batch = B;
             g.z = z;
@@ -769,6 +814,7 @@
         GemmArgs g;
         g.lda = D.n_mels; g.W = m->w("enc.conv1.w"); g.bias = m->w("enc.conv1.b");
         g.ldc = d; g.M = kMelFrames; g.N = d; g.K = 3 * D.n_mels; g.flags = kGemmGelu;
+        g.row_band = band ? band + kBandConv1 : nullptr;
         gemm(g, table([](wlk_session* s) { return (const float*)s->mel_t; }, [&](wlk_session* s) { return s->x1p + d; }, none),
              "enc_conv1");
     }
@@ -777,7 +823,8 @@
         GemmArgs g;
         g.lda = 2 * d; g.W = m->w("enc.conv2.w"); g.bias = m->w("enc.conv2.b");
         g.ldc = d; g.M = T; g.N = d; g.K = 3 * d; g.flags = kGemmGelu | kGemmResidual; g.ldr = d;
-        gemm(g, table([](wlk_session* s) { return (const float*)s->x1p; }, [](wlk_session* s) { return s->ex; },
+        g.row_band = band ? band + kBandConv2 : nullptr;
+        gemm(g, table([](wlk_session* s) { return (const float*)s->x1p; }, [&](wlk_session* s) { return stem_keep ? s->x0 : s->ex; },
                       [&](wlk_session*) { return pos; }), "enc_conv2");
     }
     const float scale = std::pow((float)kHeadDim, -0.25f);
@@ -807,6 +854,18 @@
                                       [](wlk_session* s) { return reinterpret_cast<float*>(s->emlp3); }, none);
     const PtrTable z_mlp3_ex_res = table([](wlk_session* s) { return reinterpret_cast<const float*>(s->emlp3); }, [](wlk_session* s) { return s->ex; },
                                          [](wlk_session* s) { return (const float*)s->ex; });
+    const PtrTable z_x0_eh3 = table([](wlk_session* s) { return (const float*)s->x0; },
+                                    [](wlk_session* s) { return reinterpret_cast<float*>(s->eh3); }, none);
+    const PtrTable z_eh3_qkv3_l0 = table([](wlk_session* s) { return reinterpret_cast<const float*>(s->eh3); },
+                                         [](wlk_session* s) { return reinterpret_cast<float*>(s->eqkv3_l0); }, none);
+    const PtrTable z_qkv3_l0_att = table([](wlk_session* s) { return reinterpret_cast<const float*>(s->eqkv3_l0); },
+                                         [](wlk_session* s) { return s->eatt; }, none);
+    const PtrTable z_qkv3_l0_eh3 = table([](wlk_session* s) { return reinterpret_cast<const float*>(s->eqkv3_l0); },
+                                         [](wlk_session* s) { return reinterpret_cast<float*>(s->eh3); }, none);
+    const PtrTable z_att_ex_x0 = table([](wlk_session* s) { return (const float*)s->eatt; }, [](wlk_session* s) { return s->ex; },
+                                       [](wlk_session* s) { return (const float*)s->x0; });
+    const PtrTable z_eh3_ex_x0 = table([](wlk_session* s) { return reinterpret_cast<const float*>(s->eh3); }, [](wlk_session* s) { return s->ex; },
+                                       [](wlk_session* s) { return (const float*)s->x0; });
     const bool attn_x3 = enc_attention_x3_enabled() && d == D.n_audio_head * 64 && T >= 64 && (2 * d) % 128 == 0;
     auto gemm_x3 = [&](const GemmArgs& g, const unsigned short* w3, const PtrTable& z, const char* tag) {
         X3GemmArgs x;
@@ -822,16 +881,19 @@
         g.lda = d; g.W = L.qkvw; g.bias = L.qkvb; g.ldc = 3 * d; g.M = T; g.N = 3 * d;
         g.K = d; g.flags = kGemmScaleCols; g.scale = scale; g.scale_cols = 2 * d;
         bool att_is_x3 = false;
+        const bool l0 = i == 0 && stem_keep;
         if (L.qkvw3 && attn_x3) {
-            launch_layernorm_x3_batched(c, z_ex_eh3, B, d, L.ln1w, L.ln1b, d, T, d, "enc_ln1");
+            launch_layernorm_x3_batched(c, l0 ? z_x0_eh3 : z_ex_eh3, B, d, L.ln1w, L.ln1b, d, T, d, "enc_ln1",
+                                        l0 && band ? band + kBandLn1 : nullptr);
             X3GemmArgs x;
             x.lda = d; x.W3 = L.qkvw3; x.bias = g.bias; x.M = T; x.N = 3 * d; x.K = d; x.flags = g.flags; x.scale = g.scale;
-            x.scale_cols = g.scale_cols; x.batch = B; x.z = z_eh3_qkv3;
+            x.scale_cols = g.scale_cols; x.batch = B; x.z = l0 ? z_eh3_qkv3_l0 : z_eh3_qkv3;
+            x.row_band = l0 && band ? band + kBandQkv : nullptr;
             x.x3_out = true; x.ldc3 = 2 * d; x.vt_col0 = 2 * d; x.vt_off = x3_attn_vt_off(T, d); x.vt_ld = x3_attn_vt_ld(T);
             launch_gemm_x3(c, x, "enc_qkv_x3");
             att_is_x3 = L.outw3 != nullptr;
             launch_encoder_attention_x3(c, nullptr, 2L * d, x3_attn_vt_off(T, d), x3_attn_vt_ld(T), nullptr, d, T, d, D.n_audio_head,
-                                        att_is_x3 ? &z_qkv3_eh3 : &z_qkv3_att, B, att_is_x3);
+                                        att_is_x3 ? (l0 ? &z_qkv3_l0_eh3 : &z_qkv3_eh3) : (l0 ? &z_qkv3_l0_att : &z_qkv3_att), B, att_is_x3);
         } else {
             if (L.qkvw3) {
                 launch_layernorm_x3_batched(c, z_ex_eh3, B, d, L.ln1w, L.ln1b, d, T, d, "enc_ln1");
@@ -848,9 +910,9 @@
         if (L.outw3) {
             if (!att_is_x3)
                 for (int i = 0; i < B; ++i) launch_x3_pack(c, group[i]->eatt, d, group[i]->eh3, d, T, d);
-            gemm_x3(o, L.outw3, z_eh3_ex_res, "enc_out_x3");
+            gemm_x3(o, L.outw3, l0 ? z_eh3_ex_x0 : z_eh3_ex_res, "enc_out_x3");
         } else {
-            gemm(o, z_att_ex, "enc_out");
+            gemm(o, l0 ? z_att_ex_x0 : z_att_ex, "enc_out");
         }
         GemmArgs f1;
         f1.lda = d; f1.W = L.fc1w; f1.bias = L.fc1b; f1.ldc = 4 * d; f1.M = T; f1.N = 4 * d; f1.K = d; f1.flags = kGemmGelu;
@@ -1733,6 +1795,21 @@
             }
             return copy_out(s, s->enc_out, T * d, host, capacity, n_written);
         }
+        if (w == "cross_kv") return copy_out(s, s->cross_kv, (uint64_t)D.n_text_layer * T * 2 * d, host, capacity, n_written);
+        if (w == "x0" || w == "qkv0" || w == "enc_band") {
+            if (!s->x0) return fail(WLK_ERR_STATE, "the session keeps no encoder stem (not on the X3 q|k|v + X3 attention route)");
+            if (w == "x0") return copy_out(s, s->x0, T * (uint64_t)D.n_audio_state, host, capacity, n_written);
+            if (w == "qkv0")
+                return copy_out(s, reinterpret_cast<const float*>(s->eqkv3_l0), x3_attn_image_elems((int)T, D.n_audio_state) / 2,
+                                host, capacity, n_written);
+            if (n_written) *n_written = kEncBandInts;
+            if (capacity < (uint64_t)kEncBandInts) return fail(WLK_ERR_CAPACITY, "export buffer too small");
+            int b[kEncBandInts];
+            WLK_HIP(hipStreamSynchronize(s->stream));
+            copy_sync(b, s->enc_band, sizeof(b), hipMemcpyDeviceToHost);
+            for (int i = 0; i < kEncBandInts; ++i) host[i] = (float)b[i];
+            return WLK_OK;
+        }
         if (w == "logits_last") return copy_out(s, s->logits_last, (uint64_t)s->beam * D.n_vocab, host, capacity, n_written);
         if (w == "logits_sot") return copy_out(s, s->logits_sot, (uint64_t)s->beam * D.n_vocab, host, capacity, n_written);
         if (w == "attn_last") return copy_out(s, s->attn_last, (uint64_t)s->beam * T, host, capacity, n_written);
diff --git a/whisperlivekit_amd/csrc/common.h b/whisperlivekit_amd/csrc/common.h
--- a/whisperlivekit_amd/csrc/common.h
+++ b/whisperlivekit_amd/csrc/common.h
@@ -158,6 +158,7 @@
     int scale_period = 0;
     int batch = 0;
     long long* dbg_clock = nullptr;
+    const int* row_band = nullptr;
     const float* ln_gamma = nullptr;
     const float* ln_beta = nullptr;
     float* kcache = nullptr;
@@ -189,7 +190,7 @@
     do {                                                                                                                    \
         asm volatile("" ::"s"((g).A), "s"((g).lda), "s"((g).W), "s"((g).bias), "s"((g).C), "s"((g).ldc), "s"((g).R),        \
                      "s"((g).ldr), "s"((g).M), "s"((g).N), "s"((g).K), "s"((g).flags), "s"((g).scale), "s"((g).scale_cols), \
-                     "s"((g).scale_period), "s"((g).batch), "s"((g).dbg_clock));                                            \
+                     "s"((g).scale_period), "s"((g).batch), "s"((g).dbg_clock), "s"((g).row_band));                                            \
         __builtin_amdgcn_sched_barrier(0);     \
     } while (0)
 void launch_gemm(const LaunchCtx& ctx, const GemmArgs& g, const char* tag);
@@ -242,6 +243,7 @@
     long vt_off = 0;
     long vt_ld = 0;
     bool x3_out = false;
+    const int* row_band = nullptr;
     PtrTable z;
 };
 bool gemm_x3_wide_applicable(int M, int N, int K, long lda);
@@ -278,7 +280,7 @@
 void launch_layernorm_x3(const LaunchCtx& ctx, const float* x, long ldx, const float* gamma, const float* beta,
                          unsigned short* y3, long ldy3, int rows, int d, const char* tag);
 void launch_layernorm_x3_batched(const LaunchCtx& ctx, const PtrTable& z, int batch, long ldx, const float* gamma,
-                                 const float* beta, long ldy3, int rows, int d, const char* tag);
+                                 const float* beta, long ldy3, int rows, int d, const char* tag, const int* row_band = nullptr);
 
 struct MelArgs {
     const float* audio;
@@ -297,7 +299,14 @@
     int head = 0;
     int first = 0;
     int n_padded = 0x7fffffff;
-};
+    const float* prev_max = nullptr;
+    float* new_max = nullptr;
+    int* band = nullptr;
+    int reuse = 0;
+    int band_T = 0;
+    int band_cand[10] = {0, 0, 0, 0, 0, 0, 0, 0, 0, 0};
+};
+enum EncBandStage : int { kBandMel = 0, kBandConv1 = 2, kBandConv2 = 4, kBandLn1 = 6, kBandQkv = 8, kEncBandInts = 10 };
 void launch_mel(const LaunchCtx& ctx, const MelArgs& a);
 void launch_mel_full(const LaunchCtx& ctx, const MelArgs& a, float* max_scratch, float* out);
 void launch_pcm16_to_float(const LaunchCtx& ctx, const short* in, float* out, int n);
diff --git a/whisperlivekit_amd/csrc/gemm_f32.hip b/whisperlivekit_amd/csrc/gemm_f32.hip
--- a/whisperlivekit_amd/csrc/gemm_f32.hip
+++ b/whisperlivekit_amd/csrc/gemm_f32.hip
@@ -55,6 +55,10 @@
     }
     const int m0 = tile_m * BM;
     const int n0 = tile_n * BN;
+    if (g.row_band) {
+        const int lo = g.row_band[0], hi = g.row_band[1];
+        if (m0 >= hi || m0 + BM <= lo) return;
+    }
 
     constexpr unsigned kOob = 0x80000000u;
     const __amdgpu_buffer_rsrc_t rsrc_a = __builtin_amdgcn_make_buffer_rsrc(
@@ -628,6 +632,10 @@
         if (tile_m >= tiles_m) return;
     }
     const int m0 = tile_m * BM, n0 = tile_n * BN;
+    if (g.row_band) {
+        const int lo = g.row_band[0], hi = g.row_band[1];
+        if (m0 >= hi || m0 + BM <= lo) return;
+    }
 
     const float* src[NP];
 #pragma unroll
@@ -818,6 +826,7 @@
     if (g.kcache && !(gemm_takes_kwave(g.M, g.N, g.K) || want_kwave))
         throw std::invalid_argument("gemm: fused KV-cache append is only available on the k-wave path");
     if ((gemm_takes_kwave(g.M, g.N, g.K) && g.force_kernel != 3) || (want_kwave && g.K >= 256)) {
+        if (g.row_band) throw std::invalid_argument("gemm: a row band is only available on the tiled and k-pipe paths");
         if (g.M <= 128 && g.force_kernel != 2) {
             const long tiles16 = (long)((g.N + 15) / 16) * ((g.M + 15) / 16);
             hipLaunchKernelGGL(gemm_nt_f32_kwave16_kernel<>, dim3((unsigned)tiles16), dim3(256), 0, ctx.stream, g);
diff --git a/whisperlivekit_amd/csrc/gemm_x3.hip b/whisperlivekit_amd/csrc/gemm_x3.hip
--- a/whisperlivekit_amd/csrc/gemm_x3.hip
+++ b/whisperlivekit_amd/csrc/gemm_x3.hip
@@ -155,14 +155,20 @@
     const int lane = threadIdx.x & 63;
     const int wave = __builtin_amdgcn_readfirstlane(threadIdx.x >> 6);
     const bool batched = g.batch > 0;
-    const int tiles_m = (g.M + BM - 1) / BM, tiles_n = (g.N + XW_BN - 1) / XW_BN;
-    const bool banded = g.walk_banded != 0;
+    int tm_lo = 0, tiles_m = (g.M + BM - 1) / BM;
+    const int tiles_n = (g.N + XW_BN - 1) / XW_BN;
+    if (g.row_band) {
+        const int lo = max(g.row_band[0], 0), hi = min(g.row_band[1], g.M);
+        tm_lo = lo / BM;
+        tiles_m = hi > lo ? (hi + BM - 1) / BM - tm_lo : 0;
+    }
+    const bool banded = g.walk_banded != 0 && (!g.row_band || tiles_m >= 8);
     const int band_m = banded ? (tiles_m + 3) / 4 : tiles_m, band_n = banded ? (tiles_n + 1) / 2 : tiles_n;
     const int per_session = band_m * band_n;
     const int xcd = banded ? (int)(blockIdx.x & 7) : 0;
     const int first = banded ? (int)(blockIdx.x >> 3) : (int)blockIdx.x;
     const int stride = banded ? (int)(gridDim.x >> 3) : (int)gridDim.x;
-    const int limit = g.walk_slots;
+    const int limit = g.row_band ? per_session * (batched ? g.batch : 1) : g.walk_slots;
     const int band_m0 = banded ? (xcd >> 1) * band_m : 0, band_n0 = banded ? (xcd & 1) * band_n : 0;
     auto decode = [&](int slot, int& tm, int& tn, int& b) -> bool {
         b = slot / per_session;
@@ -175,9 +181,9 @@
             rm = r / band_n;
             cn = r - rm * band_n;
         }
-        tm = band_m0 + rm;
+        tm = tm_lo + band_m0 + rm;
         tn = band_n0 + cn;
-        return tm < tiles_m && tn < tiles_n;
+        return band_m0 + rm < tiles_m && tn < tiles_n;
     };
     auto advance = [&](int slot) {
         int tm, tn, b;
diff --git a/whisperlivekit_amd/csrc/internal.h b/whisperlivekit_amd/csrc/internal.h
--- a/whisperlivekit_amd/csrc/internal.h
+++ b/whisperlivekit_amd/csrc/internal.h
@@ -180,6 +180,12 @@
     unsigned short* emlp3 = nullptr;
     bool enc_out_is_x3 = false;
     unsigned short* eqkv3 = nullptr;
+    float* x0 = nullptr;
+    unsigned short* eqkv3_l0 = nullptr;
+    float* enc_max = nullptr;
+    int* enc_band = nullptr;
+    int enc_max_cur = 0;
+    bool enc_reuse_valid = false, enc_reuse_on = true;
     bool encoded = false;
     int content_len = 0;
 
diff --git a/whisperlivekit_amd/csrc/layernorm.hip b/whisperlivekit_amd/csrc/layernorm.hip
--- a/whisperlivekit_amd/csrc/layernorm.hip
+++ b/whisperlivekit_amd/csrc/layernorm.hip
@@ -60,11 +60,13 @@
 __global__ __launch_bounds__(256) void layernorm_x3_kernel(const float* __restrict__ x, long ldx,
                                                            const float* __restrict__ gamma,
                                                            const float* __restrict__ beta, unsigned short* __restrict__ y3,
-                                                           long ldy3, int rows, int d, PtrTable z) {
+                                                           long ldy3, int rows, int d, PtrTable z,
+                                                           const int* __restrict__ row_band) {
     constexpr int NCH = (NPL + 7) / 8;
     const int lane = threadIdx.x & 63;
     const int row = blockIdx.x * 4 + (threadIdx.x >> 6);
     if (row >= rows) return;
+    if (row_band && (row < row_band[0] || row >= row_band[1])) return;
     if (x == nullptr) {
         x = table_at(z.in, blockIdx.y);
         y3 = reinterpret_cast<unsigned short*>(table_at(z.out, blockIdx.y));
@@ -174,17 +176,18 @@
     if (rows <= 0) return;
     layernorm_check(d, ldx, ldy3, true, 0);
     KernelScope ks(ctx, tag);
-    launch_ln_x3_by_width(d, dim3((rows + 3) / 4), ctx.stream, x, ldx, gamma, beta, y3, ldy3, rows, d, PtrTable{});
+    launch_ln_x3_by_width(d, dim3((rows + 3) / 4), ctx.stream, x, ldx, gamma, beta, y3, ldy3, rows, d, PtrTable{},
+                          (const int*)nullptr);
     WLK_HIP(hipGetLastError());
 }
 
 void launch_layernorm_x3_batched(const LaunchCtx& ctx, const PtrTable& z, int batch, long ldx, const float* gamma,
-                                 const float* beta, long ldy3, int rows, int d, const char* tag) {
+                                 const float* beta, long ldy3, int rows, int d, const char* tag, const int* row_band) {
     if (rows <= 0 || batch <= 0) return;
     layernorm_check(d, ldx, ldy3, true, batch);
     KernelScope ks(ctx, tag);
     launch_ln_x3_by_width(d, dim3((rows + 3) / 4, batch), ctx.stream, (const float*)nullptr, ldx, gamma, beta,
-                          (unsigned short*)nullptr, ldy3, rows, d, z);
+                          (unsigned short*)nullptr, ldy3, rows, d, z, row_band);
     WLK_HIP(hipGetLastError());
 }
 
diff --git a/whisperlivekit_amd/csrc/mel.hip b/whisperlivekit_amd/csrc/mel.hip
--- a/whisperlivekit_amd/csrc/mel.hip
+++ b/whisperlivekit_amd/csrc/mel.hip
@@ -67,9 +67,26 @@
         if (tid < s) red[tid] = fmaxf(red[tid], red[tid + s]);
         __syncthreads();
     }
-    const float floor_v = red[0] - 8.0f;
+    const float gmax = red[0];
+    const float floor_v = gmax - 8.0f;
     const long total = (long)kMelFrames * a.n_mels;
-    for (long i = (long)blockIdx.x * 256 + tid; i < total; i += (long)gridDim.x * 256) {
+    long i_lo = 0, i_hi = total;
+    if (a.band) {
+        const bool narrow = a.reuse && __float_as_uint(gmax) == __float_as_uint(a.prev_max[0]);
+        if (narrow) {
+            i_lo = (long)a.band_cand[kBandMel] * a.n_mels;
+            i_hi = (long)a.band_cand[kBandMel + 1] * a.n_mels;
+        }
+        if (blockIdx.x == 0 && tid < kEncBandInts) {
+            int cand = a.band_cand[0];
+#pragma unroll
+            for (int k = 1; k < kEncBandInts; ++k) cand = tid == k ? a.band_cand[k] : cand;
+            const int full = (tid & 1) ? (tid < kBandConv2 ? kMelFrames : a.band_T) : 0;
+            a.band[tid] = narrow ? cand : full;
+        }
+        if (blockIdx.x == 0 && tid == 0) a.new_max[0] = gmax;
+    }
+    for (long i = i_lo + (long)blockIdx.x * 256 + tid; i < i_hi; i += (long)gridDim.x * 256) {
         const int t = (int)(i / a.n_mels);
         const float v = t < a.n_active ? a.logmel[i] : -10.0f;
         a.mel_t[i + a.n_mels] = (fmaxf(v, floor_v) + 4.0f) / 4.0f;
```

New measurement: 205.9 audio_s/s. No clear change (-0.0%).
